# Jonetz/TreeDetection

Measured on AMD Instinct MI355X. Metric: tiles/sec (1000x1000 RGB+nDSM) predict_tiles model stage, higher is better.
Workload: dtype f32

## Files before the change

include/treedet.h:

```cpp
#ifndef TREEDET_H
#define TREEDET_H

#include <stddef.h>
#include <stdint.h>

#ifdef __cplusplus
extern "C" {
#endif

typedef int td_status;
typedef struct td_engine td_engine;

enum {
    TD_OK = 0,
    TD_ERR_INVALID = -1,
    TD_ERR_HIP = -2,
    TD_ERR_WEIGHTS = -3,
    TD_ERR_CAPACITY = -4,
    TD_ERR_STATE = -5,
    TD_ERR_UNSUPPORTED = -6
};

enum { TD_PRECISION_FP32 = 0, TD_PRECISION_FP16 = 1 };
enum { TD_INPUT_F32_CHW = 0,
       TD_INPUT_U8_HWC = 1 };

typedef struct td_model_desc {
    int32_t num_classes;
    int32_t precision;
    int32_t pre_nms_topk;
    int32_t post_nms_topk;
    int32_t detections_per_image;
    float rpn_nms_thresh;
    float score_thresh;
    float nms_thresh;
    float mask_thresh;
} td_model_desc;

typedef struct td_tensor_desc {
    const char* name;
    const float* data;
    int32_t ndim;
    int64_t shape[4];
} td_tensor_desc;

#define TD_MASK_SIDE 28

typedef struct td_detections {
    float* boxes;
    float* scores;
    int32_t* classes;
    int32_t* count;
    float* mask_probs;
    int32_t* mask_region;
    int64_t* mask_offset;
    uint32_t* mask_bits;
    int64_t mask_words_per_image;
} td_detections;

void td_model_desc_default(td_model_desc* desc);
td_status td_engine_create(const td_model_desc* desc, int device, td_engine** out);
td_status td_engine_load_weights(td_engine* e, const td_tensor_desc* tensors, size_t n);
td_status td_engine_reserve(td_engine* e, int max_batch, int max_hp, int max_wp);
td_status td_engine_forward(td_engine* e, const void* images, int input_format, const int32_t* hw_valid,
                            const int32_t* hw_out, int B, int Hp, int Wp, void* stream, td_detections* out);
#define TD_PHASE_STEM 6
td_status td_engine_forward_phase(td_engine* e, int phase, const void* images, int input_format, const int32_t* hw_valid,
                                  const int32_t* hw_out, int B, int Hp, int Wp, void* stream, td_detections* out);
td_status td_engine_tensor(td_engine* e, const char* name, void** dev_ptr, int64_t dims[4], int* elem_size);
td_status td_engine_read_tensor(td_engine* e, const char* name, void* dst_dev, int64_t bytes, void* stream);
#define TD_PROF_CATEGORIES 9
td_status td_engine_profile_enable(td_engine* e, int enable);
td_status td_engine_profile_read(td_engine* e, double* ms, int64_t* launches, double* flops, double* bytes, int reset);
#define TD_PROF_CLASSES 7
#define TD_CLS_WINO_GEMM 0
#define TD_CLS_WINO_XFORM 1
#define TD_CLS_CONV1X1 2
#define TD_CLS_CONV3X3 3
#define TD_CLS_FC 4
#define TD_CLS_MASK_HEAD 5
#define TD_CLS_TAIL 6
#define TD_PEAK_F32_MFMA_TFLOPS 157.3
#define TD_PEAK_F16_MFMA_TFLOPS 2500.0
#define TD_HBM_ACHIEVABLE_TBS 6.3
td_status td_engine_profile_classes(td_engine* e, double* ms, int64_t* launches, double* exec_flops, double* bytes, double* tmin_ms, int reset);
const char* td_last_error(void);
void td_engine_destroy(td_engine* e);

td_status td_resize_tile_u8(const uint8_t* src, int h, int w, int c, uint8_t* dst, int out_h, int out_w,
                            int dst_pitch_px, void* tmp_dev , void* stream);
td_status td_resize_batch_u8(const uint8_t* const* src_tiles, int n, int h, int w, int c, uint8_t* dst, int out_h,
                             int out_w, int dst_pitch_px, int64_t dst_image_stride_bytes, void* tmp_dev, void* stream);
td_status td_resize_bilinear_f64(const double* src, int c, int h, int w, float* dst, int out_h, int out_w, int dst_pitch_px,
                                 int64_t dst_plane_stride, void* stream);
td_status td_windows_u16_to_input(const uint16_t* raster, int height, int width, int c, const int32_t* windows, int n, int32_t* band1_max,
                                  float* dst, int out_h, int out_w, int dst_pitch_px, int64_t dst_plane_stride, int64_t dst_image_stride,
                                  void* stream);
void td_resize_shape(int h, int w, int short_edge, int max_size, int* out_h, int* out_w);

td_status td_bottleneck_tail_nhwc(const void* x, const void* w2, const float* scale2, const float* bias2, const void* w3,
                                  const float* scale3, const float* bias3, const void* shortcut, void* y, int B, int H, int W,
                                  int mid, int cout, int precision, void* stream);
td_status td_conv2d_nhwc(const void* x, const void* w, const float* scale, const float* bias,
                         const void* residual, int res_shift, void* y, int B, int H, int W, int Cin,
                         int Cout, int KH, int KW, int stride, int pad, int relu, int precision,
                         void* stream);
td_status td_conv2d_head_nhwc(const void* x, const void* w, const float* bias, const void* head_w, const float* head_b,
                              float* head_y, int B, int H, int W, int Cin, int KH, int KW, int pad, int head_n, int precision,
                              void* stream);
td_status td_conv2d_winograd_nhwc(const float* x, const float* w, const float* scale, const float* bias, float* y, int B,
                                  int H, int W, int Cin, int Cout, int relu, void* stream);
td_status td_conv2d_winograd_head_nhwc(const float* x, const float* w, const float* bias, const float* head_w, const float* head_b,
                                       float* head_y, int B, int H, int W, int Cin, int head_n, void* stream);
td_status td_nms(const float* boxes, const float* scores, int n, float iou_thresh, int32_t* keep_idx,
                 int32_t* keep_count, void* stream);
td_status td_roi_align(const void* feat, int H, int W, int C, const float* rois, int R, float spatial_scale,
                       int pooled, void* out, int precision, void* stream);
td_status td_paste_masks(const float* mask_probs, const float* boxes, int n, int out_h, int out_w,
                         float thresh, int32_t* mask_region, int64_t* mask_offset, uint32_t* mask_bits,
                         int64_t mask_words_cap, void* stream);

td_status td_paste_masks_batch(const float* mask_probs, const float* boxes, const int32_t* counts, const int32_t* out_hw,
                               int batch, int dets_per_image, float thresh, int32_t* mask_region, int64_t* mask_offset,
                               uint32_t* mask_bits, int64_t mask_words_per_image, void* stream);

#define TD_CONTOUR_MAX 256
td_status td_trace_contours_dev(const int32_t* mask_region, const int64_t* mask_offset, const uint32_t* mask_bits,
                                int64_t mask_words_per_image, const int32_t* counts, int batch, int dets_per_image,
                                int16_t* points, int points_cap, int32_t* image_points, int32_t* det_info,
                                int32_t* contour_info, void* stream);

int td_find_contours(const uint8_t* img, int h, int w, int32_t* points, int max_points, int32_t* starts,
                     int max_contours);
int td_tile_polygons_json(const int32_t* mask_region, const int64_t* mask_offset, const uint32_t* mask_bits,
                          int64_t mask_words, const float* scores, const int32_t* classes, int n,
                          const double* transform, const char* image_id, char* buf, int64_t cap, int64_t* needed);

int td_tile_prediction_file(int device, const int32_t* mask_region, const int64_t* mask_offset, const uint32_t* mask_bits_dev,
                            uint32_t* rows_host, int64_t mask_words, const float* scores, const int32_t* classes, int n,
                            const double* transform, const char* image_id, const char* path, int64_t* bytes_written);

int td_batch_prediction_files(int device, int n_tiles, int dets_per_image, const int32_t* mask_region, const int64_t* mask_offset,
                              const uint32_t* mask_bits_dev, uint32_t* rows_host, int64_t bits_stride_words, const float* scores,
                              const int32_t* classes, const int32_t* counts, const double* transforms, const char* image_id,
                              const char* const* paths, int threads, int32_t* status, int64_t* bytes_written);

int64_t td_tiff_lzw_decode(const uint8_t* src, int64_t n, uint8_t* dst, int64_t cap);
int64_t td_tiff_packbits_decode(const uint8_t* src, int64_t n, uint8_t* dst, int64_t cap);
int64_t td_tiff_lzw_encode(const uint8_t* src, int64_t n, uint8_t* dst, int64_t cap);
td_status td_tiff_lzw_decode_dev(const uint8_t* comp, const int64_t* block_off, const int64_t* block_nbytes, int nblocks,
                                 uint8_t* blocks_out, int64_t block_cap, int64_t* decoded, int32_t* status, void* stream);
td_status td_tiff_inflate_dev(const uint8_t* comp, const int64_t* block_off, const int64_t* block_nbytes, int nblocks,
                              uint8_t* blocks_out, int64_t block_cap, int64_t* decoded, int32_t* status, void* stream);
td_status td_tiff_inflate_verified_dev(const uint8_t* comp, const int64_t* block_off, const int64_t* block_nbytes, int nblocks,
                                       uint8_t* blocks_out, int64_t block_cap, int64_t* decoded, int32_t* status, int64_t* end_off,
                                       void* stream);
td_status td_tiff_adler32_blocks_dev(const uint8_t* blocks, int64_t block_cap, const int64_t* decoded, const uint8_t* comp,
                                     const int64_t* block_off, const int64_t* block_nbytes, const int64_t* end_off, int nblocks,
                                     int32_t* status, void* stream);
td_status td_adler32_dev(const uint8_t* data_dev, int64_t n, uint32_t* out_dev, void* stream);
int64_t td_tiff_inflate(const uint8_t* src, int64_t n, uint8_t* dst, int64_t cap);
int64_t td_tiff_inflate_verified(const uint8_t* src, int64_t n, uint8_t* dst, int64_t cap);
td_status td_tiff_blocks_to_image_dev(const uint8_t* blocks, int64_t block_cap, int block_w, int block_h, int blocks_across,
                                      int blocks_down, int spp, int predictor, uint8_t* image, int width, int height, void* stream);
td_status td_tiff_blocks_to_image_u16_dev(const uint8_t* blocks, int64_t block_cap, int block_w, int block_h, int blocks_across,
                                          int blocks_down, int spp, int predictor, uint16_t* image, int width, int height, void* stream);
td_status td_tiff_blocks_to_image_f32_dev(const uint8_t* blocks, int64_t block_cap, int block_w, int block_h, int blocks_across,
                                          int blocks_down, int spp, int predictor, float* image, int width, int height, void* stream);
#define TD_JPEG_TABSET_BYTES 8928
td_status td_tiff_jpeg_plan(const uint8_t* tables, int64_t tables_len, const uint8_t* data, const int64_t* block_off,
                            const int64_t* block_nbytes, int nblocks, int photometric, int bands, int block_w, const int32_t* block_rows,
                            int64_t* block_info, int64_t* segs, int64_t seg_cap, void* tabsets, int64_t tabset_cap, int64_t* totals);
td_status td_tiff_jpeg_decode_dev(const uint8_t* comp, const int64_t* block_info, int nblocks, const int64_t* segs, int nseg,
                                  const void* tabsets, int16_t* coef, uint8_t* planes, int64_t coef_count, int32_t* status, uint8_t* image,
                                  int width, int height, int bands, int block_w, int block_h, int blocks_across, void* stream);
int64_t td_jpeg_decode(const uint8_t* src, int64_t n, uint8_t* dst, int64_t cap, int32_t* shape);
int64_t td_read_window(int fd, int64_t file_off, int64_t row_stride, int64_t row_bytes, int64_t rows, uint8_t* dst);
int64_t td_read_windows(int fd, int n, const int64_t* file_off, int64_t row_stride, const int64_t* row_bytes, const int64_t* rows,
                        uint8_t* dst, const int64_t* dst_off, int threads);
int td_tiff_unpredict(void* data, int64_t rows, int64_t cols, int samples, int bytes_per_sample);
int td_tiff_unpredict_float(void* data, int64_t rows, int64_t cols, int samples, int bytes_per_sample);

int td_tile_polygons_json_dev(const int16_t* points, int64_t points_cap, const int32_t* det_info, const int32_t* contour_info,
                              const int32_t* mask_region, const int64_t* mask_offset, const uint32_t* mask_bits,
                              int64_t mask_words, const float* scores, const int32_t* classes, int n,
                              const double* transform, const char* image_id, char* buf, int64_t cap, int64_t* needed);

int td_simplify_ring(const double* xy, int n, double tolerance, double* out_xy, int out_cap);

int td_ring_is_valid(const double* xy, int n);
int td_stitch_tile_json(const char* json, int64_t len, const double* box, double tolerance, int32_t srs_id,
                        uint8_t* blobs, int64_t blob_cap, int64_t* blob_offsets, double* scores, int max_features,
                        int64_t* needed_bytes, int* needed_features);

int td_stitch_tile_files(const char* paths, const int64_t* path_offsets, int n_files, const double* boxes, double tolerance,
                         const int32_t* srs_ids, int threads, uint8_t* blobs, int64_t blob_cap, int64_t* blob_offsets,
                         double* scores, int max_features, int32_t* file_status, int64_t* needed_bytes, int* needed_features);

int td_region_relate(const double* ring_xy, const int64_t* ring_start, const int32_t* ring_poly, int n_rings,
                     const double* query_xy, const int64_t* query_start, int n_queries, uint8_t* flags);

td_status td_crown_stats(const float* raster, int rows, int cols, const double* transform, const int32_t* window,
                         const float* circles, int n, int mode, float radius_scale, float* out, void* stream);

#ifdef __cplusplus
}
#endif
#endif
```

treedetection_amd/_lib.py:

```python
from __future__ import annotations

import ctypes as C
import os
import threading
from typing import Optional

_HERE = os.path.dirname(os.path.abspath(__file__))
LIB_PATH = os.path.join(_HERE, "libtreedet_hip.so")

_lib: Optional[C.CDLL] = None
ERR_INVALID = -1
ERR_CAPACITY = -4
ERR_STATE = -5
ERR_UNSUPPORTED = -6
JPEG_TABSET_BYTES = 8928


class TdError(RuntimeError):
    """A libtreedet_hip call returned a negative status (message from td_last_error)."""


class ModelDesc(C.Structure):
    _fields_ = [("num_classes", C.c_int32), ("precision", C.c_int32), ("pre_nms_topk", C.c_int32),
                ("post_nms_topk", C.c_int32), ("detections_per_image", C.c_int32),
                ("rpn_nms_thresh", C.c_float), ("score_thresh", C.c_float), ("nms_thresh", C.c_float),
                ("mask_thresh", C.c_float)]


class TensorDesc(C.Structure):
    _fields_ = [("name", C.c_char_p), ("data", C.c_void_p), ("ndim", C.c_int32), ("shape", C.c_int64 * 4)]


class Detections(C.Structure):
    _fields_ = [("boxes", C.c_void_p), ("scores", C.c_void_p), ("classes", C.c_void_p), ("count", C.c_void_p),
                ("mask_probs", C.c_void_p), ("mask_region", C.c_void_p), ("mask_offset", C.c_void_p),
                ("mask_bits", C.c_void_p), ("mask_words_per_image", C.c_int64)]


SIGNATURES = {
    "td_model_desc_default": (None, [C.POINTER(ModelDesc)]),
    "td_engine_create": (C.c_int, [C.POINTER(ModelDesc), C.c_int, C.POINTER(C.c_void_p)]),
    "td_engine_load_weights": (C.c_int, [C.c_void_p, C.POINTER(TensorDesc), C.c_size_t]),
    "td_engine_reserve": (C.c_int, [C.c_void_p, C.c_int, C.c_int, C.c_int]),
    "td_engine_forward": (C.c_int, [C.c_void_p, C.c_void_p, C.c_int, C.POINTER(C.c_int32), C.POINTER(C.c_int32),
                                    C.c_int, C.c_int, C.c_int, C.c_void_p, C.POINTER(Detections)]),
    "td_engine_forward_phase": (C.c_int, [C.c_void_p, C.c_int, C.c_void_p, C.c_int, C.POINTER(C.c_int32), C.POINTER(C.c_int32),
                                          C.c_int, C.c_int, C.c_int, C.c_void_p, C.POINTER(Detections)]),
    "td_engine_tensor": (C.c_int, [C.c_void_p, C.c_char_p, C.POINTER(C.c_void_p), C.POINTER(C.c_int64),
                                   C.POINTER(C.c_int)]),
    "td_engine_read_tensor": (C.c_int, [C.c_void_p, C.c_char_p, C.c_void_p, C.c_int64, C.c_void_p]),
    "td_engine_profile_enable": (C.c_int, [C.c_void_p, C.c_int]),
    "td_engine_profile_read": (C.c_int, [C.c_void_p, C.POINTER(C.c_double), C.POINTER(C.c_int64), C.POINTER(C.c_double),
                                         C.POINTER(C.c_double), C.c_int]),
    "td_engine_profile_classes": (C.c_int, [C.c_void_p, C.POINTER(C.c_double), C.POINTER(C.c_int64), C.POINTER(C.c_double),
                                            C.POINTER(C.c_double), C.POINTER(C.c_double), C.c_int]),
    "td_last_error": (C.c_char_p, []),
    "td_engine_destroy": (None, [C.c_void_p]),
    "td_resize_tile_u8": (C.c_int, [C.c_void_p, C.c_int, C.c_int, C.c_int, C.c_void_p, C.c_int, C.c_int, C.c_int,
                                    C.c_void_p, C.c_void_p]),
    "td_resize_batch_u8": (C.c_int, [C.POINTER(C.c_void_p), C.c_int, C.c_int, C.c_int, C.c_int, C.c_void_p, C.c_int, C.c_int,
                                     C.c_int, C.c_int64, C.c_void_p, C.c_void_p]),
    "td_bottleneck_tail_nhwc": (C.c_int, [C.c_void_p] * 9 + [C.c_int] * 6 + [C.c_void_p]),
    "td_resize_bilinear_f64": (C.c_int, [C.c_void_p, C.c_int, C.c_int, C.c_int, C.c_void_p, C.c_int, C.c_int, C.c_int, C.c_int64, C.c_void_p]),
    "td_windows_u16_to_input": (C.c_int, [C.c_void_p, C.c_int, C.c_int, C.c_int, C.c_void_p, C.c_int, C.c_void_p, C.c_void_p, C.c_int, C.c_int,
                                          C.c_int, C.c_int64, C.c_int64, C.c_void_p]),
    "td_resize_shape": (None, [C.c_int, C.c_int, C.c_int, C.c_int, C.POINTER(C.c_int), C.POINTER(C.c_int)]),
    "td_conv2d_nhwc": (C.c_int, [C.c_void_p, C.c_void_p, C.c_void_p, C.c_void_p, C.c_void_p, C.c_int, C.c_void_p]
                       + [C.c_int] * 11 + [C.c_void_p]),
    "td_conv2d_head_nhwc": (C.c_int, [C.c_void_p] * 6 + [C.c_int] * 9 + [C.c_void_p]),
    "td_conv2d_winograd_head_nhwc": (C.c_int, [C.c_void_p] * 6 + [C.c_int] * 5 + [C.c_void_p]),
    "td_conv2d_winograd_nhwc": (C.c_int, [C.c_void_p] * 5 + [C.c_int] * 6 + [C.c_void_p]),
    "td_nms": (C.c_int, [C.c_void_p, C.c_void_p, C.c_int, C.c_float, C.c_void_p, C.c_void_p, C.c_void_p]),
    "td_roi_align": (C.c_int, [C.c_void_p, C.c_int, C.c_int, C.c_int, C.c_void_p, C.c_int, C.c_float, C.c_int,
                               C.c_void_p, C.c_int, C.c_void_p]),
    "td_paste_masks": (C.c_int, [C.c_void_p, C.c_void_p, C.c_int, C.c_int, C.c_int, C.c_float, C.c_void_p,
                                 C.c_void_p, C.c_void_p, C.c_int64, C.c_void_p]),
    "td_paste_masks_batch": (C.c_int, [C.c_void_p, C.c_void_p, C.c_void_p, C.POINTER(C.c_int32), C.c_int, C.c_int, C.c_float,
                                       C.c_void_p, C.c_void_p, C.c_void_p, C.c_int64, C.c_void_p]),
    "td_crown_stats": (C.c_int, [C.c_void_p, C.c_int, C.c_int, C.POINTER(C.c_double), C.POINTER(C.c_int32), C.c_void_p, C.c_int,
                                 C.c_int, C.c_float, C.c_void_p, C.c_void_p]),
    "td_trace_contours_dev": (C.c_int, [C.c_void_p, C.c_void_p, C.c_void_p, C.c_int64, C.c_void_p, C.c_int, C.c_int, C.c_void_p,
                                        C.c_int, C.c_void_p, C.c_void_p, C.c_void_p, C.c_void_p]),
    "td_find_contours": (C.c_int, [C.c_void_p, C.c_int, C.c_int, C.c_void_p, C.c_int, C.c_void_p, C.c_int]),
    "td_batch_prediction_files": (C.c_int, [C.c_int, C.c_int, C.c_int, C.c_void_p, C.c_void_p, C.c_void_p, C.c_void_p, C.c_int64, C.c_void_p,
                                          C.c_void_p, C.c_void_p, C.c_void_p, C.c_char_p, C.POINTER(C.c_char_p), C.c_int, C.c_void_p, C.c_void_p]),
    "td_tiff_lzw_decode": (C.c_int64, [C.c_void_p, C.c_int64, C.c_void_p, C.c_int64]),
    "td_tiff_packbits_decode": (C.c_int64, [C.c_void_p, C.c_int64, C.c_void_p, C.c_int64]),
    "td_tiff_lzw_encode": (C.c_int64, [C.c_void_p, C.c_int64, C.c_void_p, C.c_int64]),
    "td_tiff_inflate": (C.c_int64, [C.c_void_p, C.c_int64, C.c_void_p, C.c_int64]),
    "td_tiff_inflate_dev": (C.c_int, [C.c_void_p, C.c_void_p, C.c_void_p, C.c_int, C.c_void_p, C.c_int64, C.c_void_p, C.c_void_p, C.c_void_p]),
    "td_tiff_inflate_verified": (C.c_int64, [C.c_void_p, C.c_int64, C.c_void_p, C.c_int64]),
    "td_tiff_inflate_verified_dev": (C.c_int, [C.c_void_p, C.c_void_p, C.c_void_p, C.c_int, C.c_void_p, C.c_int64, C.c_void_p, C.c_void_p, C.c_void_p,
                                               C.c_void_p]),
    "td_tiff_adler32_blocks_dev": (C.c_int, [C.c_void_p, C.c_int64, C.c_void_p, C.c_void_p, C.c_void_p, C.c_void_p, C.c_void_p, C.c_int, C.c_void_p,
                                             C.c_void_p]),
    "td_adler32_dev": (C.c_int, [C.c_void_p, C.c_int64, C.c_void_p, C.c_void_p]),
    "td_tiff_lzw_decode_dev": (C.c_int, [C.c_void_p, C.c_void_p, C.c_void_p, C.c_int, C.c_void_p, C.c_int64, C.c_void_p, C.c_void_p, C.c_void_p]),
    "td_tiff_blocks_to_image_dev": (C.c_int, [C.c_void_p, C.c_int64, C.c_int, C.c_int, C.c_int, C.c_int, C.c_int, C.c_int, C.c_void_p, C.c_int, C.c_int, C.c_void_p]),
    "td_tiff_blocks_to_image_u16_dev": (C.c_int, [C.c_void_p, C.c_int64, C.c_int, C.c_int, C.c_int, C.c_int, C.c_int, C.c_int, C.c_void_p, C.c_int,
                                                  C.c_int, C.c_void_p]),
    "td_tiff_blocks_to_image_f32_dev": (C.c_int, [C.c_void_p, C.c_int64, C.c_int, C.c_int, C.c_int, C.c_int, C.c_int, C.c_int, C.c_void_p, C.c_int,
                                                  C.c_int, C.c_void_p]),
    "td_tiff_jpeg_plan": (C.c_int, [C.c_void_p, C.c_int64, C.c_void_p, C.c_void_p, C.c_void_p, C.c_int, C.c_int, C.c_int, C.c_int, C.c_void_p,
                                    C.c_void_p, C.c_void_p, C.c_int64, C.c_void_p, C.c_int64, C.c_void_p]),
    "td_tiff_jpeg_decode_dev": (C.c_int, [C.c_void_p, C.c_void_p, C.c_int, C.c_void_p, C.c_int, C.c_void_p, C.c_void_p, C.c_void_p, C.c_int64,
                                          C.c_void_p, C.c_void_p] + [C.c_int] * 6 + [C.c_void_p]),
    "td_jpeg_decode": (C.c_int64, [C.c_void_p, C.c_int64, C.c_void_p, C.c_int64, C.c_void_p]),
    "td_read_windows": (C.c_int64, [C.c_int, C.c_int, C.c_void_p, C.c_int64, C.c_void_p, C.c_void_p, C.c_void_p, C.c_void_p, C.c_int]),
    "td_tiff_unpredict": (C.c_int, [C.c_void_p, C.c_int64, C.c_int64, C.c_int, C.c_int]),
    "td_tiff_unpredict_float": (C.c_int, [C.c_void_p, C.c_int64, C.c_int64, C.c_int, C.c_int]),
    "td_region_relate": (C.c_int, [C.c_void_p, C.c_void_p, C.c_void_p, C.c_int, C.c_void_p, C.c_void_p, C.c_int, C.c_void_p]),
    "td_simplify_ring": (C.c_int, [C.c_void_p, C.c_int, C.c_double, C.c_void_p, C.c_int]),
    "td_ring_is_valid": (C.c_int, [C.c_void_p, C.c_int]),
    "td_stitch_tile_json": (C.c_int, [C.c_char_p, C.c_int64, C.POINTER(C.c_double), C.c_double, C.c_int32, C.c_void_p,
                                      C.c_int64, C.c_void_p, C.c_void_p, C.c_int, C.POINTER(C.c_int64), C.POINTER(C.c_int)]),
    "td_stitch_tile_files": (C.c_int, [C.c_char_p, C.c_void_p, C.c_int, C.c_void_p, C.c_double, C.c_void_p, C.c_int, C.c_void_p, C.c_int64,
                                       C.c_void_p, C.c_void_p, C.c_int, C.c_void_p, C.POINTER(C.c_int64), C.POINTER(C.c_int)]),
    "td_tile_polygons_json_dev": (C.c_int, [C.c_void_p, C.c_int64, C.c_void_p, C.c_void_p, C.c_void_p, C.c_void_p, C.c_void_p, C.c_int64,
                                            C.c_void_p, C.c_void_p, C.c_int, C.POINTER(C.c_double), C.c_char_p, C.c_void_p, C.c_int64,
                                            C.POINTER(C.c_int64)]),
    "td_read_window": (C.c_int64, [C.c_int, C.c_int64, C.c_int64, C.c_int64, C.c_int64, C.c_void_p]),
    "td_tile_prediction_file": (C.c_int, [C.c_int, C.c_void_p, C.c_void_p, C.c_void_p, C.c_void_p, C.c_int64, C.c_void_p, C.c_void_p,
                                          C.c_int, C.POINTER(C.c_double), C.c_char_p, C.c_char_p, C.POINTER(C.c_int64)]),
    "td_tile_polygons_json": (C.c_int, [C.c_void_p, C.c_void_p, C.c_void_p, C.c_int64, C.c_void_p, C.c_void_p, C.c_int,
                                        C.POINTER(C.c_double), C.c_char_p, C.c_void_p, C.c_int64, C.POINTER(C.c_int64)]),
}


def load() -> C.CDLL:
    global _lib
    if _lib is not None:
        return _lib
    host_only = os.environ.get("TD_HOST_LIB")
    if host_only:
        lib = C.CDLL(host_only, mode=C.RTLD_GLOBAL)
        for name, (res, args) in SIGNATURES.items():
            fn = getattr(lib, name, None)
            if fn is not None:
                fn.restype = res
                fn.argtypes = args
        _lib = lib
        return lib
    if not os.path.exists(LIB_PATH):
        raise TdError(f"{LIB_PATH} not found — build it first: python -c 'import __graft_entry__ as g; g.build()' "
                      f"(or make -C treedetection_amd/csrc). There is no CPU fallback.")
    import torch

    lib = C.CDLL(LIB_PATH, mode=C.RTLD_GLOBAL)
    for name, (res, args) in SIGNATURES.items():
        fn = getattr(lib, name)
        fn.restype = res
        fn.argtypes = args
    _lib = lib
    return lib


def check(status: int, what: str = "") -> None:
    if status < 0:
        msg = load().td_last_error().decode("utf-8", "replace")
        raise TdError(f"{what or 'libtreedet_hip'} failed ({status}): {msg}")


def stream_ptr() -> int:
    import torch

    return int(torch.cuda.current_stream().cuda_stream)


_low_priority_streams: dict = {}
_low_priority_lock = threading.Lock()


def low_priority_stream(device_index: int):
    import torch

    with _low_priority_lock:
        if device_index in _low_priority_streams:
            return _low_priority_streams[device_index]
        lib = load()
        least, greatest, handle = C.c_int(0), C.c_int(0), C.c_void_p()
        with torch.cuda.device(device_index):
            torch.cuda.current_stream()
            err = lib.hipDeviceGetStreamPriorityRange(C.byref(least), C.byref(greatest))
            if err == 0:
                err = lib.hipStreamCreateWithPriority(C.byref(handle), C.c_uint(1), C.c_int(least.value))
            if err != 0 or not handle.value:
                raise TdError(f"hipStreamCreateWithPriority(priority {least.value}) failed: hipError {err}")
            stream = torch.cuda.ExternalStream(handle.value, device=device_index)
        _low_priority_streams[device_index] = stream
        return stream
```

treedetection_amd/csrc/api.cpp:

```cpp
#include "common.h"
#include "detect.h"
#include <cstdarg>
#include <cstdio>
#include <cmath>
#include <cstdlib>
#include <vector>


namespace {
td_status scratch(void** p, size_t bytes) {
    TD_HIP_CHECK(hipMalloc(p, bytes ? bytes : 16));
    return TD_OK;
}
}

extern "C" {

void td_model_desc_default(td_model_desc* d) {
    d->num_classes = 1;
    d->precision = TD_PRECISION_FP32;
    d->pre_nms_topk = 1000;
    d->post_nms_topk = 1000;
    d->detections_per_image = 100;
    d->rpn_nms_thresh = 0.7f;
    d->score_thresh = 0.3f;
    d->nms_thresh = 0.5f;
    d->mask_thresh = 0.5f;
}

static td_status conv2d_api(ConvArgs& a, int precision, void* stream);

td_status td_conv2d_nhwc(const void* x, const void* w, const float* scale, const float* bias,
                         const void* residual, int res_shift, void* y, int B, int H, int W, int Cin,
                         int Cout, int KH, int KW, int stride, int pad, int relu, int precision,
                         void* stream) {
    TD_REQUIRE(x && w && y, "td_conv2d_nhwc: null pointer");
    TD_REQUIRE(stride >= 1 && KH >= 1 && KW >= 1 && B >= 1, "td_conv2d_nhwc: bad geometry");
    ConvArgs a{};
    a.x = x; a.w = w; a.scale = scale; a.bias = bias; a.res = residual; a.y = y;
    a.B = B; a.H = H; a.W = W; a.Cin = Cin; a.Cout = Cout; a.KH = KH; a.KW = KW;
    a.stride = stride; a.pad = pad;
    a.Ho = (H + 2 * pad - KH) / stride + 1;
    a.Wo = (W + 2 * pad - KW) / stride + 1;
    a.res_shift = res_shift; a.relu = relu; a.out_mode = 0;
    a.M = B * a.Ho * a.Wo; a.m_dyn = nullptr; a.m_mul = 1;
    a.out_f32 = (precision & 0x10000) && (precision & 0xff) == TD_PRECISION_FP16 ? 1 : 0;
    a.tile_cfg = ((precision >> 8) & 0xff) - 1;
    a.tile_strict = (precision & 0x20000) ? 1 : 0;
    return conv2d_api(a, precision, stream);
}

td_status td_conv2d_head_nhwc(const void* x, const void* w, const float* bias, const void* head_w, const float* head_b,
                              float* head_y, int B, int H, int W, int Cin, int KH, int KW, int pad, int head_n, int precision,
                              void* stream) {
    TD_REQUIRE(x && w && head_w && head_y, "td_conv2d_head_nhwc: null pointer");
    TD_REQUIRE((precision & 0xff) == TD_PRECISION_FP16, "td_conv2d_head_nhwc: float16 tensors only");
    TD_REQUIRE(KH >= 1 && KW >= 1 && B >= 1 && head_n >= 1 && head_n <= 32, "td_conv2d_head_nhwc: bad geometry");
    ConvArgs a{};
    a.x = x; a.w = w; a.bias = bias;
    a.B = B; a.H = H; a.W = W; a.Cin = Cin; a.Cout = 256; a.KH = KH; a.KW = KW;
    a.stride = 1; a.pad = pad;
    a.Ho = H + 2 * pad - KH + 1;
    a.Wo = W + 2 * pad - KW + 1;
    a.relu = 1; a.M = B * a.Ho * a.Wo; a.m_mul = 1;
    a.tile_cfg = ((precision >> 8) & 0xff) - 1;
    TD_REQUIRE(conv_head_capable(a.tile_cfg, TD_PRECISION_FP16), "td_conv2d_head_nhwc: tile id %d does not own 256 output channels per block", a.tile_cfg);
    a.head_w = head_w; a.head_b = head_b; a.head_y = head_y; a.head_n = head_n;
    a.y = head_y;
    return conv2d_api(a, precision, stream);
}

static td_status conv2d_api(ConvArgs& a, int precision, void* stream) {
    hipStream_t s = static_cast<hipStream_t>(stream);
    ConvArgs with_frag = a;
    with_frag.w_frag = a.w;
    if (!conv_tile(a.tile_cfg) || !conv_tile(a.tile_cfg)->frag || conv_tile_refusal(a.tile_cfg, with_frag, precision & 0xff))
        return conv2d_launch(a, precision & 0xff, s);
    const int es = (precision & 0xff) == TD_PRECISION_FP16 ? 2 : 4;
    const size_t n = (size_t)a.Cout * a.KH * a.KW * a.Cin;
    std::vector<unsigned char> bits(n * es), packed;
    TD_HIP_CHECK(hipStreamSynchronize(s));
    TD_HIP_CHECK(hipMemcpy(bits.data(), a.w, n * es, hipMemcpyDeviceToHost));
    conv_bd_pack(bits.data(), es, a.Cout, a.KH, a.KW, a.Cin, packed);
    void* wf = nullptr;
    td_status st = scratch(&wf, packed.size());
    if (st < 0) return st;
    hipError_t herr = hipMemcpy(wf, packed.data(), packed.size(), hipMemcpyHostToDevice);
    a.w_frag = wf;
    if (herr == hipSuccess) st = conv2d_launch(a, precision & 0xff, s);
    hipError_t herr2 = hipStreamSynchronize(s);
    (void)hipFree(wf);
    if (st < 0) return st;
    TD_HIP_CHECK(herr);
    TD_HIP_CHECK(herr2);
    return TD_OK;
}

static td_status wino_api(const float* x, const float* w, const float* scale, const float* bias, float* y, int B, int H, int W, int Cin,
                          int Cout, int relu, void* stream, const float* head_w, const float* head_b, float* head_y, int head_n);

td_status td_conv2d_winograd_nhwc(const float* x, const float* w, const float* scale, const float* bias, float* y, int B, int H,
                                  int W, int Cin, int Cout, int relu, void* stream) {
    TD_REQUIRE(y, "td_conv2d_winograd_nhwc: bad arguments");
    return wino_api(x, w, scale, bias, y, B, H, W, Cin, Cout, relu, stream, nullptr, nullptr, nullptr, 0);
}

td_status td_conv2d_winograd_head_nhwc(const float* x, const float* w, const float* bias, const float* head_w, const float* head_b,
                                       float* head_y, int B, int H, int W, int Cin, int head_n, void* stream) {
    TD_REQUIRE(head_w && head_y && head_n >= 1 && head_n <= 32, "td_conv2d_winograd_head_nhwc: bad arguments");
    return wino_api(x, w, nullptr, bias, nullptr, B, H, W, Cin, 256, 1, stream, head_w, head_b, head_y, head_n);
}

static td_status wino_api(const float* x, const float* w, const float* scale, const float* bias, float* y, int B, int H, int W, int Cin,
                          int Cout, int relu, void* stream, const float* head_w, const float* head_b, float* head_y, int head_n) {
    TD_REQUIRE(x && w && B >= 1 && H >= 1 && W >= 1, "td_conv2d_winograd_nhwc: bad arguments");
    TD_REQUIRE(Cin % 32 == 0 && Cout % 4 == 0, "td_conv2d_winograd_nhwc: Cin must be a multiple of 32, Cout of 4");
    hipStream_t s = static_cast<hipStream_t>(stream);
    const char* tenv = getenv("TD_WINO_TILE");
    const bool f43 = head_w || (tenv && atoi(tenv) == 4);
    const int P = f43 ? 36 : 16;
    const size_t T = f43 ? (size_t)B * ((H + 3) / 4) * ((W + 3) / 4) : (size_t)B * ((H + 1) / 2) * ((W + 1) / 2);
    std::vector<float> wh((size_t)Cout * 9 * Cin), uh((size_t)P * Cout * Cin);
    TD_HIP_CHECK(hipMemcpy(wh.data(), w, wh.size() * sizeof(float), hipMemcpyDeviceToHost));
    if (f43) wino43_filter_transform(wh.data(), Cout, Cin, uh.data());
    else wino_filter_transform(wh.data(), Cout, Cin, uh.data());
    void *U = nullptr, *V = nullptr, *Mb = nullptr;
    td_status st;
    if ((st = scratch(&U, uh.size() * 4)) < 0 || (st = scratch(&V, P * T * Cin * 4)) < 0 || (st = scratch(&Mb, P * T * Cout * 4)) < 0) {
        (void)hipFree(U); (void)hipFree(V); (void)hipFree(Mb);
        return st;
    }
    TD_HIP_CHECK(hipMemcpy(U, uh.data(), uh.size() * 4, hipMemcpyHostToDevice));
    const char* folde = getenv("TD_WINO_FOLD");
    const bool fold = f43 && !head_w && folde && atoi(folde) != 0;
    if (fold) TD_REQUIRE(wino43_fused_ok(B, H, W, Cin, Cout), "td_conv2d_winograd_nhwc: TD_WINO_FOLD needs Cin %% 128 == 0, Cout %% 64 == 0");
    const char* fenv = getenv("TD_WINO_FUSED");
    const bool fused = !f43 && (!fenv || atoi(fenv) != 0);
    ConvArgs a{};
    a.w = U; a.y = Mb;
    a.Cin = Cin; a.Cout = Cout; a.KH = a.KW = 1; a.stride = 1; a.pad = 0;
    a.M = (int)T; a.m_mul = 1; a.tile_cfg = -1;
    a.w_bs = (long long)Cout * Cin; a.y_bs = (long long)T * Cout;
    if (fused) {
        a.x = x; a.B = B; a.H = H; a.W = W;
        st = wino_gemm_launch(a, s);
    } else {
        st = f43 ? wino43_input_launch(x, B, H, W, Cin, static_cast<float*>(V), nullptr, s)
                 : wino_input_launch(x, B, H, W, Cin, static_cast<float*>(V), nullptr, 1, 0, (int)T, s);
        if (st == TD_OK && fold) {
            st = wino43_fused_launch(static_cast<float*>(V), static_cast<float*>(U), B, H, W, Cin, Cout, scale, bias, relu, y, nullptr, s);
        } else if (st == TD_OK) {
            a.x = V; a.B = 1; a.H = 1; a.W = (int)T; a.Ho = 1; a.Wo = (int)T;
            a.batch_count = P; a.x_bs = (long long)T * Cin;
            st = conv2d_launch(a, TD_PRECISION_FP32, s);
        }
    }
    if (fold) {
    } else if (st == TD_OK && head_w)
        st = wino43_output_head_launch(static_cast<float*>(Mb), B, H, W, Cout, scale, bias, relu, head_w, head_b, head_y, head_n, s);
    else if (st == TD_OK)
        st = f43 ? wino43_output_launch(static_cast<float*>(Mb), B, H, W, Cout, scale, bias, relu, y, nullptr, s)
                 : wino_output_launch(static_cast<float*>(Mb), B, H, W, Cout, scale, bias, relu, y, nullptr, 1, 0, (int)T, s);
    hipError_t herr = hipStreamSynchronize(s);
    (void)hipFree(U); (void)hipFree(V); (void)hipFree(Mb);
    if (st < 0) return st;
    TD_HIP_CHECK(herr);
    return TD_OK;
}

td_status td_resize_tile_u8(const uint8_t* src, int h, int w, int c, uint8_t* dst, int out_h, int out_w,
                            int dst_pitch_px, void* tmp_dev, void* stream) {
    return resize_tile_u8_launch(src, h, w, c, dst, out_h, out_w, dst_pitch_px, tmp_dev, static_cast<hipStream_t>(stream));
}

td_status td_resize_batch_u8(const uint8_t* const* src_tiles, int n, int h, int w, int c, uint8_t* dst, int out_h,
                             int out_w, int dst_pitch_px, int64_t dst_image_stride_bytes, void* tmp_dev, void* stream) {
    return resize_batch_u8_launch(src_tiles, n, h, w, c, dst, out_h, out_w, dst_pitch_px, (size_t)dst_image_stride_bytes,
                                  tmp_dev, static_cast<hipStream_t>(stream));
}

td_status td_bottleneck_tail_nhwc(const void* x, const void* w2, const float* scale2, const float* bias2, const void* w3,
                                  const float* scale3, const float* bias3, const void* shortcut, void* y, int B, int H, int W,
                                  int mid, int cout, int precision, void* stream) {
    TD_REQUIRE(x && w2 && w3 && shortcut && y && B > 0 && H > 0 && W > 0, "td_bottleneck_tail_nhwc: null argument or empty tensor");
    TailArgs a{};
    a.x = x; a.w2 = w2; a.scale2 = scale2; a.bias2 = bias2; a.w3 = w3; a.scale3 = scale3; a.bias3 = bias3; a.res = shortcut; a.y = y;
    a.B = B; a.H = H; a.W = W; a.MID = mid; a.COUT = cout; a.M = B * H * W;
    return bottleneck_tail_launch(a, precision, static_cast<hipStream_t>(stream));
}

td_status td_resize_bilinear_f64(const double* src, int c, int h, int w, float* dst, int out_h, int out_w, int dst_pitch_px,
                                 int64_t dst_plane_stride, void* stream) {
    return resize_bilinear_f64_launch(src, c, h, w, dst, out_h, out_w, dst_pitch_px, (long long)dst_plane_stride, static_cast<hipStream_t>(stream));
}

td_status td_windows_u16_to_input(const uint16_t* raster, int height, int width, int c, const int32_t* windows, int n, int32_t* band1_max,
                                  float* dst, int out_h, int out_w, int dst_pitch_px, int64_t dst_plane_stride, int64_t dst_image_stride,
                                  void* stream) {
    return windows_u16_to_input_launch(raster, height, width, c, windows, n, band1_max, dst, out_h, out_w, dst_pitch_px,
                                       (long long)dst_plane_stride, (long long)dst_image_stride, static_cast<hipStream_t>(stream));
}

void td_resize_shape(int h, int w, int short_edge, int max_size, int* out_h, int* out_w) {
    const double scale = (double)short_edge / (double)(h < w ? h : w);
    double newh, neww;
    if (h < w) { newh = short_edge; neww = scale * w; }
    else { newh = scale * h; neww = short_edge; }
    const double mx = newh > neww ? newh : neww;
    if (mx > max_size) {
        const double s2 = (double)max_size / mx;
        newh *= s2;
        neww *= s2;
    }
    *out_h = (int)(newh + 0.5);
    *out_w = (int)(neww + 0.5);
}

td_status td_nms(const float* boxes, const float* scores, int n, float iou_thresh, int32_t* keep_idx,
                 int32_t* keep_count, void* stream) {
    TD_REQUIRE(boxes && scores && keep_idx && keep_count, "td_nms: null pointer");
    TD_REQUIRE(n >= 0 && n <= 32768, "td_nms: n=%d must be in [0, 32768]", n);
    hipStream_t s = static_cast<hipStream_t>(stream);
    if (n == 0) {
        TD_HIP_CHECK(hipMemsetAsync(keep_count, 0, sizeof(int32_t), s));
        return TD_OK;
    }
    void *sb = nullptr, *ss = nullptr, *si = nullptr, *sc = nullptr, *mk = nullptr, *kp = nullptr;
    td_status st;
    if ((st = scratch(&sb, sizeof(float) * 4 * n)) < 0) return st;
    if ((st = scratch(&ss, sizeof(float) * n)) < 0) return st;
    if ((st = scratch(&si, sizeof(int) * n)) < 0) return st;
    if ((st = scratch(&sc, sizeof(int))) < 0) return st;
    if ((st = scratch(&mk, sizeof(unsigned long long) * n * td_cdiv(n, 64))) < 0) return st;
    if ((st = scratch(&kp, sizeof(int) * n)) < 0) return st;
    if (n > 1024) {
        st = nms_big_launch(boxes, scores, n, iou_thresh, (float*)sb, (float*)ss, (int*)si, (int*)sc, (unsigned long long*)mk, (int*)kp, keep_count, s);
    } else {
        st = sort_boxes_launch(boxes, scores, nullptr, nullptr, 1, n, (float*)sb, (float*)ss, (int*)si, (int*)sc, s);
        if (st >= 0) st = nms_launch((float*)sb, (int*)sc, nullptr, 1, n, iou_thresh, (unsigned long long*)mk, (int*)kp, keep_count, n, s);
    }
    if (st >= 0) st = gather_keep_launch((int*)si, (int*)kp, keep_count, n, keep_idx, s);
    hipError_t herr = hipStreamSynchronize(s);
    (void)hipFree(sb); (void)hipFree(ss); (void)hipFree(si); (void)hipFree(sc); (void)hipFree(mk); (void)hipFree(kp);
    if (st < 0) return st;
    TD_HIP_CHECK(herr);
    return TD_OK;
}

td_status td_roi_align(const void* feat, int H, int W, int C, const float* rois, int R, float spatial_scale,
                       int pooled, void* out, int precision, void* stream) {
    TD_REQUIRE(feat && rois && out, "td_roi_align: null pointer");
    TD_REQUIRE(H >= 1 && W >= 1 && pooled >= 1 && R >= 0, "td_roi_align: bad geometry");
    if (R == 0) return TD_OK;
    return roi_align_single_launch(feat, H, W, C, rois, R, spatial_scale, pooled, out, precision, static_cast<hipStream_t>(stream));
}

td_status td_paste_masks(const float* mask_probs, const float* boxes, int n, int out_h, int out_w, float thresh,
                         int32_t* mask_region, int64_t* mask_offset, uint32_t* mask_bits, int64_t mask_words_cap,
                         void* stream) {
    TD_REQUIRE(mask_probs && boxes && mask_region && mask_offset && mask_bits, "td_paste_masks: null pointer");
    TD_REQUIRE(n >= 0 && n <= 1024 && out_h >= 1 && out_w >= 1, "td_paste_masks: bad shape");
    if (n == 0) return TD_OK;
    hipStream_t s = static_cast<hipStream_t>(stream);
    void* cnt = nullptr;
    td_status st = scratch(&cnt, sizeof(int));
    if (st < 0) return st;
    TD_HIP_CHECK(hipMemcpy(cnt, &n, sizeof(int), hipMemcpyHostToDevice));
    ImgSizes outsz{};
    outsz.h[0] = out_h;
    outsz.w[0] = out_w;
    st = paste_masks_launch(mask_probs, boxes, (int*)cnt, outsz, 1, n, thresh, mask_region,
                            reinterpret_cast<long long*>(mask_offset), mask_bits, mask_words_cap, s);
    hipError_t herr = hipStreamSynchronize(s);
    (void)hipFree(cnt);
    if (st < 0) return st;
    TD_HIP_CHECK(herr);
    return TD_OK;
}

td_status td_paste_masks_batch(const float* mask_probs, const float* boxes, const int32_t* counts, const int32_t* out_hw,
                               int batch, int dets_per_image, float thresh, int32_t* mask_region, int64_t* mask_offset,
                               uint32_t* mask_bits, int64_t mask_words_per_image, void* stream) {
    TD_REQUIRE(mask_probs && boxes && counts && out_hw && mask_region && mask_offset && mask_bits,
               "td_paste_masks_batch: null pointer");
    TD_REQUIRE(batch >= 1 && batch <= TD_MAX_BATCH && dets_per_image >= 1 && dets_per_image <= 1024,
               "td_paste_masks_batch: batch %d (max %d) / detections per image %d (max 1024)", batch, TD_MAX_BATCH, dets_per_image);
    ImgSizes outsz{};
    for (int i = 0; i < batch; ++i) {
        TD_REQUIRE(out_hw[2 * i] >= 1 && out_hw[2 * i + 1] >= 1, "td_paste_masks_batch: bad output size of image %d", i);
        outsz.h[i] = out_hw[2 * i];
        outsz.w[i] = out_hw[2 * i + 1];
        const int64_t need = (int64_t)dets_per_image * ((outsz.w[i] + 2 + 31) / 32) * outsz.h[i];
        TD_REQUIRE(mask_words_per_image >= need, "td_paste_masks_batch: image %d needs %lld mask words, capacity %lld", i,
                   (long long)need, (long long)mask_words_per_image);
    }
    return paste_masks_launch(mask_probs, boxes, counts, outsz, batch, dets_per_image, thresh, mask_region,
                              reinterpret_cast<long long*>(mask_offset), mask_bits, mask_words_per_image,
                              static_cast<hipStream_t>(stream));
}

}
```

treedetection_amd/csrc/common.h:

```cpp
#pragma once
#include <hip/hip_runtime.h>
#include <hip/hip_fp16.h>
#include <cstdint>
#include <cstddef>
#include "../../include/treedet.h"
#include <string>
#include <vector>

void td_set_error(const char* fmt, ...);

int td_polygons_json_text(const int32_t* mask_region, const int64_t* mask_offset, const uint32_t* mask_bits, int64_t mask_words,
                          const float* scores, const int32_t* classes, int n, const double* transform, const char* image_id,
                          std::string& out, const char* who);

#define TD_HIP_CHECK(expr)                                                                         \
    do {                                                                                           \
        hipError_t _e = (expr);                                                                    \
        if (_e != hipSuccess) {                                                                    \
            td_set_error("%s failed: %s (%s:%d)", #expr, hipGetErrorString(_e), __FILE__, __LINE__); \
            return TD_ERR_HIP;                                                                     \
        }                                                                                          \
    } while (0)

#define TD_REQUIRE(cond, ...)            \
    do {                                 \
        if (!(cond)) {                   \
            td_set_error(__VA_ARGS__);   \
            return TD_ERR_INVALID;       \
        }                                \
    } while (0)

#define TD_KERNEL_CHECK() TD_HIP_CHECK(hipGetLastError())

td_status td_decode_ticket(hipStream_t s, int** ticket, int* cus);

static inline int td_cdiv(int a, int b) { return (a + b - 1) / b; }

struct ConvArgs {
    const void* x;
    const void* w;
    const float* scale;
    const float* bias;
    const void* res;
    void* y;
    int B, H, W, Cin, Cout, KH, KW, stride, pad, Ho, Wo;
    int res_shift;
    int relu;
    int out_mode;
    int M;
    const int* m_dyn;
    int m_mul;
    int m_off;
    int out_f32;
    int batch_count;
    long long x_bs, w_bs, y_bs;
    const void* w_frag;
    int tile_cfg;
    int tile_strict;
    const void* head_w;
    const float* head_b;
    float* head_y;
    int head_n;
    int nlev;
    struct Level {
        const void* x;
        const void* w;
        const float* bias;
        void* y;
        float* head_y;
        int H, W, M, tile0;
    } lev[5];
    int ntiles;
};
enum ConvFamily : unsigned char { TILE_IGEMM, TILE_PP8, TILE_PLANE, TILE_BD, TILE_BS, TILE_RETIRED };
enum : unsigned char { TILE_F32 = 1 << TD_PRECISION_FP32, TILE_F16 = 1 << TD_PRECISION_FP16, TILE_ANY = TILE_F32 | TILE_F16 };
struct ConvTile {
    ConvFamily family;
    unsigned char variant;
    unsigned char prec;
    bool head;
    bool frag;
    signed char tune_rank;
    unsigned char max_ksteps;
    short min_cout, max_cout;
};
inline constexpr ConvTile TD_CONV_TILES[] = {
    {TILE_IGEMM,   0, TILE_ANY, false, false,  5, 0,   0,  0},
    {TILE_IGEMM,   0, TILE_ANY, false, false, 10, 0,   0,  0},
    {TILE_IGEMM,   0, TILE_ANY, false, false, 11, 0,   0,  0},
    {TILE_IGEMM,   0, TILE_ANY, false, false, 16, 0,   0,  0},
    {TILE_IGEMM,   0, TILE_ANY, false, false, -1, 0,   0,  0},
    {TILE_IGEMM,   0, TILE_ANY, false, false, -1, 0,   0,  0},
    {TILE_IGEMM,   0, TILE_ANY, false, false, -1, 0,   0,  0},
    {TILE_IGEMM,   0, TILE_ANY, false, false, -1, 0,   0,  0},
    {TILE_IGEMM,   0, TILE_ANY, false, false, -1, 0,   0,  0},
    {TILE_IGEMM,   0, TILE_ANY, true,  false, -1, 0,   0,  0},
    {TILE_IGEMM,   0, TILE_ANY, true,  false,  1, 0,   0,  0},
    {TILE_IGEMM,   0, TILE_ANY, false, false, -1, 0,   0,  0},
    {TILE_IGEMM,   0, TILE_ANY, true,  false, -1, 0,   0,  0},
    {TILE_IGEMM,   0, TILE_ANY, true,  false, -1, 0,   0,  0},
    {TILE_IGEMM,   0, TILE_ANY, false, false, -1, 4,   0,  0},
    {TILE_IGEMM,   0, TILE_ANY, false, false,  6, 4,   0,  0},
    {TILE_IGEMM,   0, TILE_ANY, false, false,  4, 4,   0,  0},
    {TILE_PP8,     0, TILE_F16, true,  false,  2, 0, 128,  0},
    {TILE_PLANE,   0, TILE_F32, false, false, 18, 0,   0,  0},
    {TILE_PLANE,   0, TILE_F32, false, false, 19, 0,   0,  0},
    {TILE_PLANE,   0, TILE_F32, false, false, 20, 0,   0,  0},
    {TILE_RETIRED, 0, 0,        false, false, -1, 0,   0,  0},
    {TILE_RETIRED, 0, 0,        false, false, -1, 0,   0,  0},
    {TILE_BD,      0, TILE_ANY, true,  true,   8, 0,   0,  0},
    {TILE_BD,      1, TILE_ANY, false, true,  12, 0,   0,  0},
    {TILE_BD,      2, TILE_ANY, false, true,  13, 0,   0,  0},
    {TILE_BD,      3, TILE_ANY, false, true,  14, 0,   0,  0},
    {TILE_BD,      4, TILE_ANY, true,  true,   9, 0,   0,  0},
    {TILE_RETIRED, 0, 0,        false, false, -1, 0,   0,  0},
    {TILE_BD,      5, TILE_ANY, true,  true,   3, 0,   0,  0},
    {TILE_BD,      6, TILE_ANY, false, true,   7, 0,   0,  0},
    {TILE_IGEMM,   0, TILE_ANY, false, false, 15, 0,   0, 32},
    {TILE_IGEMM,   0, TILE_ANY, false, false, 17, 0,   0, 32},
    {TILE_BS,      0, TILE_ANY, false, true,   0, 4, 128,  0},
};
static inline const ConvTile* conv_tile(int id) { return id >= 0 && id < (int)(sizeof TD_CONV_TILES / sizeof *TD_CONV_TILES) ? &TD_CONV_TILES[id] : nullptr; }
static inline bool conv_head_capable(int id, int precision) { return precision == TD_PRECISION_FP16 && conv_tile(id) && conv_tile(id)->head; }
const char* conv_tile_refusal(int id, const ConvArgs& a, int precision);
td_status conv2d_launch(const ConvArgs& a, int precision, hipStream_t stream);
td_status conv_pp8_grouped_launch(ConvArgs a, hipStream_t stream);
void conv_bd_pack(const void* w_ohwi, int elem_bytes, int cout, int kh, int kw, int cin, std::vector<unsigned char>& out);
bool conv_bd_ok(const ConvArgs& a, int precision);
td_status conv_bd_launch(const ConvArgs& a, int precision, int variant, hipStream_t stream);
bool conv_bs_ok(const ConvArgs& a, int precision);
td_status conv_bs_launch(const ConvArgs& a, int precision, hipStream_t stream);
td_status wino_gemm_launch(const ConvArgs& a, hipStream_t stream);

struct TailArgs {
    const void* x;
    const void* w2;
    const float* scale2;
    const float* bias2;
    const void* w3;
    const float* scale3;
    const float* bias3;
    const void* res;
    void* y;
    int B, H, W, MID, COUT, M;
};
bool bottleneck_tail_ok(int precision, int mid, int cout);
td_status bottleneck_tail_launch(const TailArgs& a, int precision, hipStream_t stream);

td_status wino_input_launch(const float* x, int B, int H, int W, int C, float* V, const int* m_dyn, int m_mul, long long t0, int Ts,
                            hipStream_t s);
td_status wino_output_launch(const float* Mb, int B, int H, int W, int N, const float* scale, const float* bias, int relu,
                             float* y, const int* m_dyn, int m_mul, long long t0, int Ts, hipStream_t s);
void wino_filter_transform(const float* w_ohwi, int N, int C, float* U);
td_status wino43_input_launch(const float* x, int B, int H, int W, int C, float* V, const int* m_dyn, hipStream_t s);
bool wino43_fused_ok(int B, int H, int W, int C, int N);
td_status wino43_fused_launch(const float* V, const float* U, int B, int H, int W, int C, int N, const float* scale, const float* bias,
                              int relu, float* y, const int* m_dyn, hipStream_t s);
td_status wino43_output_launch(const float* Mb, int B, int H, int W, int N, const float* scale, const float* bias, int relu,
                               float* y, const int* m_dyn, hipStream_t s);
td_status wino43_output_head_launch(const float* Mb, int B, int H, int W, int N, const float* scale, const float* bias, int relu,
                                    const float* head_w, const float* head_b, float* head_y, int head_n, hipStream_t s);
void wino43_filter_transform(const float* w_ohwi, int N, int C, float* U);

struct ImgSizes {
    int h[64];
    int w[64];
};
#define TD_MAX_BATCH 64
td_status stem_launch(const void* images, int input_format, const ImgSizes& valid, int B, int Hp, int Wp,
                      const float* w_kc , const float* scale, const float* bias, void* y,
                      int cout, int precision, hipStream_t stream, const void* w16 = nullptr, const float* bias16 = nullptr);
void stem_mfma_prepare(const float* w_kc, const float* scale, const float* bias, int cout, std::vector<unsigned short>& w16_bits,
                       std::vector<float>& bias16);
td_status maxpool3x3s2_launch(const void* x, void* y, int B, int H, int W, int C, int precision, hipStream_t stream);
td_status subsample2_launch(const void* x, void* y, int B, int H, int W, int C, int precision, hipStream_t stream);
td_status resize_batch_u8_launch(const uint8_t* const* srcs, int n, int h, int w, int c, uint8_t* dst, int out_h,
                                 int out_w, int dst_pitch_px, size_t dst_img_bytes, void* tmp, hipStream_t stream);
td_status resize_bilinear_f64_launch(const double* src, int c, int h, int w, float* dst, int out_h, int out_w, int dst_pitch,
                                     long long dst_plane, hipStream_t stream);
td_status windows_u16_to_input_launch(const uint16_t* raster, int H, int W, int C, const int32_t* windows, int n, int* band1_max, float* dst,
                                      int out_h, int out_w, int dst_pitch, long long dst_plane, long long dst_image, hipStream_t stream);
td_status resize_tile_u8_launch(const uint8_t* src, int h, int w, int c, uint8_t* dst, int out_h, int out_w,
                                int dst_pitch_px, void* tmp, hipStream_t stream);
```

treedetection_amd/csrc/engine.cpp:

```cpp
#include "common.h"
#include "detect.h"

#include <cmath>
#include <cstdio>
#include <cstdlib>
#include <cstring>
#include <algorithm>
#include <functional>
#include <map>
#include <optional>
#include <string>
#include <tuple>
#include <vector>

namespace {

struct HostTensor {
    const float* data = nullptr;
    std::vector<int64_t> shape;
    int64_t numel() const {
        int64_t n = 1;
        for (auto s : shape) n *= s;
        return n;
    }
};

struct ConvLayer {
    int cout = 0, cin = 0, kh = 1, kw = 1;
    void* w = nullptr;
    float* scale = nullptr;
    float* bias = nullptr;
    bool out_f32 = false;
    void* w_frag = nullptr;
    float* wino_u = nullptr;
    float* wino_u43 = nullptr;
};

struct Block {
    ConvLayer c1, c2, c3, sc;
    bool has_sc = false;
    int stride = 1;
};

struct NamedTensor {
    void* p = nullptr;
    int64_t dims[4] = {0, 0, 0, 0};
    int elem = 4;
};

}

struct td_engine {
    td_model_desc desc{};
    int device = 0;
    bool loaded = false;
    std::vector<void*> weight_allocs;
    std::vector<void*> ws_allocs;

    float* stem_w = nullptr;
    float* stem_scale = nullptr;
    float* stem_bias = nullptr;
    unsigned short* stem_w16 = nullptr;
    float* stem_bias16 = nullptr;
    int stem_c = 64;
    std::vector<Block> stages[4];
    ConvLayer lateral[4], fpn_out[4];
    ConvLayer rpn_conv, rpn_head;
    ConvLayer fc1, fc2, pred;
    ConvLayer mask_fcn[4], deconv;
    float* mask_pred_w = nullptr;
    float mask_pred_b = 0.f;
    int fpn_c = 256, fc_dim = 1024;

    int rB = 0, rHp = 0, rWp = 0;
    void *stem_out = nullptr, *pool_out = nullptr;
    void *t1[4] = {}, *t2[4] = {}, *scb[4] = {}, *res[4] = {}, *xtmp[4] = {};
    void *inner[4] = {}, *pfeat[5] = {};
    void* rpn_t = nullptr;
    float* rpn_headbuf[5] = {};
    uint32_t* key_ws = nullptr;
    float *cand_boxes = nullptr, *cand_scores = nullptr;
    int *cand_valid = nullptr, *cand_idx = nullptr;
    unsigned long long* nms_mask = nullptr;
    int *rpn_keep = nullptr, *rpn_keep_count = nullptr;
    float *props = nullptr, *prop_scores = nullptr;
    int* prop_count = nullptr;
    void *pooled7 = nullptr, *fc1_out = nullptr, *fc2_out = nullptr;
    float* pred_out = nullptr;
    float *dboxes = nullptr, *dscores = nullptr;
    int* dflags = nullptr;
    float *sboxes = nullptr, *sscores = nullptr;
    int *sidx = nullptr, *scount = nullptr, *det_keep = nullptr, *det_keep_count = nullptr;
    float* det_boxes_net = nullptr;
    void *pooled14 = nullptr, *mbuf0 = nullptr, *mbuf1 = nullptr, *deconv_out = nullptr;
    float *mask_logits = nullptr, *mask_probs_compact = nullptr;
    int* total_rows = nullptr;
    float *o_boxes = nullptr, *o_scores = nullptr, *o_mask_probs = nullptr;
    int *o_classes = nullptr, *o_count = nullptr;

    std::map<std::string, NamedTensor> named;

    bool autotune = true;
    int backbone_subbatch = 0;
    std::map<std::tuple<int, int, int, int, int>, int> tuned;
    bool winograd = true;
    float *wino_v = nullptr, *wino_m = nullptr;
    size_t wino_elems = 0;
    bool group_levels = true;
    bool fuse_head = true;
    bool fuse_tail = true;
    bool fuse_tail_fp16 = false;
    bool wino_fused = true;
    int wino_slab = 0;
    int wino_minc = 128;
    int wino43_min = 12;
    int wino_fold = 39;
    std::string tune_cache;
    void* tune_evict = nullptr;
    size_t tune_evict_bytes = 0;

    struct FwdCtx {
        const void* images = nullptr;
        int input_format = 0, B = 0, Hp = 0, Wp = 0;
        ImgSizes valid{}, outsz{};
        td_detections out{};
        bool valid_ctx = false;
    } ctx;
    hipEvent_t phase_ev[7] = {};
    bool phase_ev_recorded[7] = {};
    hipEvent_t prev5_ev = nullptr;
    bool prev5_recorded = false;
    bool stem_done = false;

    bool prof = false;
    bool prof_group_open = false;
    struct ProfRec { hipEvent_t a, b; int cat; };
    std::vector<ProfRec> prof_recs;
    std::vector<hipEvent_t> prof_free;
    double prof_ms[TD_PROF_CATEGORIES] = {};
    int64_t prof_launches[TD_PROF_CATEGORIES] = {};
    double prof_flops[TD_PROF_CATEGORIES] = {};
    double prof_bytes[TD_PROF_CATEGORIES] = {};
    bool prof_detail = false;
    double cls_ms[TD_PROF_CLASSES] = {};
    int64_t cls_launches[TD_PROF_CLASSES] = {};
    double cls_flops[TD_PROF_CLASSES] = {};
    double cls_bytes[TD_PROF_CLASSES] = {};
    double cls_tmin_ms[TD_PROF_CLASSES] = {};
    struct ClsRec { hipEvent_t a, b; int cls; };
    std::vector<ClsRec> cls_recs;
};

namespace {

td_status dev_alloc(std::vector<void*>& pool, void** p, size_t bytes) {
    if (bytes == 0) bytes = 16;
    TD_HIP_CHECK(hipMalloc(p, bytes));
    pool.push_back(*p);
    return TD_OK;
}

template <typename T>
td_status upload(td_engine* e, const std::vector<T>& h, T** d) {
    void* p = nullptr;
    td_status st = dev_alloc(e->weight_allocs, &p, h.size() * sizeof(T));
    if (st < 0) return st;
    TD_HIP_CHECK(hipMemcpy(p, h.data(), h.size() * sizeof(T), hipMemcpyHostToDevice));
    *d = static_cast<T*>(p);
    return TD_OK;
}

td_status upload_w(td_engine* e, const std::vector<float>& h, void** d) {
    if (e->desc.precision == TD_PRECISION_FP16) {
        std::vector<_Float16> hh(h.size());
        for (size_t i = 0; i < h.size(); ++i) hh[i] = (_Float16)h[i];
        _Float16* p = nullptr;
        td_status st = upload(e, hh, &p);
        *d = p;
        return st;
    }
    float* p = nullptr;
    td_status st = upload(e, h, &p);
    *d = p;
    return st;
}

td_status upload_frag(td_engine* e, const std::vector<float>& h, ConvLayer& L) {
    L.w_frag = nullptr;
    static const bool off = getenv("TD_BDIRECT") && atoi(getenv("TD_BDIRECT")) == 0;
    const bool f16 = e->desc.precision == TD_PRECISION_FP16;
    const int ke = f16 ? 64 : 32;
    if (off || L.cin % ke != 0 || L.kh * L.kw > 32 || (size_t)L.cout * L.kh * L.kw * L.cin != h.size()) return TD_OK;
    std::vector<unsigned char> packed;
    if (f16) {
        std::vector<unsigned short> bits(h.size());
        for (size_t i = 0; i < h.size(); ++i) bits[i] = __builtin_bit_cast(unsigned short, (_Float16)h[i]);
        conv_bd_pack(bits.data(), 2, L.cout, L.kh, L.kw, L.cin, packed);
    } else {
        conv_bd_pack(h.data(), 4, L.cout, L.kh, L.kw, L.cin, packed);
    }
    unsigned char* d = nullptr;
    td_status st = upload(e, packed, &d);
    L.w_frag = d;
    return st;
}

using TensorMap = std::map<std::string, HostTensor>;

td_status need(const TensorMap& tm, const std::string& name, int ndim, const HostTensor** out) {
    auto it = tm.find(name);
    if (it == tm.end()) {
        td_set_error("load_weights: tensor '%s' missing", name.c_str());
        return TD_ERR_WEIGHTS;
    }
    if ((int)it->second.shape.size() != ndim) {
        td_set_error("load_weights: tensor '%s' has %d dims, expected %d", name.c_str(), (int)it->second.shape.size(), ndim);
        return TD_ERR_WEIGHTS;
    }
    *out = &it->second;
    return TD_OK;
}

std::vector<float> pack_ohwi(const HostTensor& t) {
    const int co = (int)t.shape[0], ci = (int)t.shape[1], kh = (int)t.shape[2], kw = (int)t.shape[3];
    std::vector<float> out((size_t)co * ci * kh * kw);
    for (int o = 0; o < co; ++o)
        for (int c = 0; c < ci; ++c)
            for (int y = 0; y < kh; ++y)
                for (int x = 0; x < kw; ++x)
                    out[(((size_t)o * kh + y) * kw + x) * ci + c] = t.data[(((size_t)o * ci + c) * kh + y) * kw + x];
    return out;
}

td_status bn_fold(const TensorMap& tm, const std::string& p, int c, std::vector<float>& scale, std::vector<float>& bias) {
    const HostTensor *g, *b, *m, *v;
    td_status st;
    if ((st = need(tm, p + ".norm.weight", 1, &g)) < 0) return st;
    if ((st = need(tm, p + ".norm.bias", 1, &b)) < 0) return st;
    if ((st = need(tm, p + ".norm.running_mean", 1, &m)) < 0) return st;
    if ((st = need(tm, p + ".norm.running_var", 1, &v)) < 0) return st;
    if (g->shape[0] != c || b->shape[0] != c || m->shape[0] != c || v->shape[0] != c) {
        td_set_error("load_weights: norm tensors of '%s' do not have %d channels", p.c_str(), c);
        return TD_ERR_WEIGHTS;
    }
    scale.resize(c);
    bias.resize(c);
    for (int i = 0; i < c; ++i) {
        const float r = 1.0f / std::sqrt(v->data[i] + 1e-5f);
        const float s = g->data[i] * r;
        const float ms = m->data[i] * s;
        scale[i] = s;
        bias[i] = b->data[i] - ms;
    }
    return TD_OK;
}

int wino_slab_tiles(const td_engine* e, const ConvLayer& L) {
    (void)L;
    return e->wino_slab > 0 ? e->wino_slab : (1 << 30);
}

// ... 11 lines not shown
}

td_status load_conv_bn(td_engine* e, const TensorMap& tm, const std::string& p, ConvLayer& L) {
    const HostTensor* w;
    td_status st = need(tm, p + ".weight", 4, &w);
    if (st < 0) return st;
    L.cout = (int)w->shape[0];
    L.cin = (int)w->shape[1];
    L.kh = (int)w->shape[2];
    L.kw = (int)w->shape[3];
    const std::vector<float> packed = pack_ohwi(*w);
    if ((st = upload_w(e, packed, &L.w)) < 0) return st;
    if ((st = upload_frag(e, packed, L)) < 0) return st;
    if ((st = upload_wino(e, packed, L)) < 0) return st;
    std::vector<float> s, b;
    if ((st = bn_fold(tm, p, L.cout, s, b)) < 0) return st;
    if ((st = upload(e, s, &L.scale)) < 0) return st;
    return upload(e, b, &L.bias);
}

td_status load_conv_bias(td_engine* e, const TensorMap& tm, const std::string& p, ConvLayer& L) {
    const HostTensor *w, *b;
    td_status st = need(tm, p + ".weight", 4, &w);
    if (st < 0) return st;
    if ((st = need(tm, p + ".bias", 1, &b)) < 0) return st;
    L.cout = (int)w->shape[0];
    L.cin = (int)w->shape[1];
    L.kh = (int)w->shape[2];
    L.kw = (int)w->shape[3];
    if (b->shape[0] != L.cout) {
        td_set_error("load_weights: bias of '%s' has wrong length", p.c_str());
        return TD_ERR_WEIGHTS;
    }
    const std::vector<float> packed = pack_ohwi(*w);
    if ((st = upload_w(e, packed, &L.w)) < 0) return st;
    if ((st = upload_frag(e, packed, L)) < 0) return st;
    if ((st = upload_wino(e, packed, L)) < 0) return st;
    L.scale = nullptr;
    return upload(e, std::vector<float>(b->data, b->data + L.cout), &L.bias);
}

void set_named(td_engine* e, const char* name, void* p, int64_t d0, int64_t d1 = 0, int64_t d2 = 0, int64_t d3 = 0,
               int elem = 4) {
    NamedTensor t;
    t.p = p;
    t.dims[0] = d0; t.dims[1] = d1; t.dims[2] = d2; t.dims[3] = d3;
    t.elem = elem;
    e->named[name] = t;
}

hipEvent_t prof_event(td_engine* e) {
    hipEvent_t ev = nullptr;
    if (!e->prof_free.empty()) {
        ev = e->prof_free.back();
        e->prof_free.pop_back();
    } else {
        (void)hipEventCreate(&ev);
    }
    return ev;
}

struct ProfScope {
    td_engine* e;
    hipStream_t s;
    hipEvent_t a = nullptr;
    int cat;
    bool group;
    ProfScope(td_engine* e_, hipStream_t s_, int cat_, double flops = 0.0, double bytes = 0.0, bool group_ = false)
        : e(e_), s(s_), cat(cat_), group(group_) {
        if (!e->prof) return;
        if (!group) {
            e->prof_flops[cat] += flops;
            e->prof_bytes[cat] += bytes;
            e->prof_launches[cat] += 1;
        }
        if (e->prof_group_open) return;
        a = prof_event(e);
        (void)hipEventRecord(a, s);
        if (group) e->prof_group_open = true;
    }
    ~ProfScope() {
        if (!a) return;
        hipEvent_t b = prof_event(e);
        (void)hipEventRecord(b, s);
        e->prof_recs.push_back({a, b, cat});
        if (group) e->prof_group_open = false;
    }
};

struct ClassScope {
    td_engine* e;
    hipStream_t s;
    hipEvent_t a = nullptr;
    int cls;
    ClassScope(td_engine* e_, hipStream_t s_, int cls_, double exec_flops, double bytes) : e(e_), s(s_), cls(cls_) {
        if (!e->prof) return;
        const double peak = (e->desc.precision == TD_PRECISION_FP16 ? TD_PEAK_F16_MFMA_TFLOPS : TD_PEAK_F32_MFMA_TFLOPS) * 1e12;
        e->cls_launches[cls] += 1;
        e->cls_flops[cls] += exec_flops;
        e->cls_bytes[cls] += bytes;
        e->cls_tmin_ms[cls] += 1e3 * std::max(exec_flops / peak, bytes / (TD_HBM_ACHIEVABLE_TBS * 1e12));
        if (!e->prof_detail) return;
        a = prof_event(e);
        (void)hipEventRecord(a, s);
    }
    ~ClassScope() {
        if (!a) return;
        hipEvent_t b = prof_event(e);
        (void)hipEventRecord(b, s);
        e->cls_recs.push_back({a, b, cls});
    }
};

void load_tune_cache(td_engine* e) {
    if (e->tune_cache.empty()) return;
    if (FILE* f = fopen(e->tune_cache.c_str(), "r")) {
        int pr, a0, a1, a2, a3, a4, cfg;
        while (fscanf(f, "%d %d %d %d %d %d %d", &pr, &a0, &a1, &a2, &a3, &a4, &cfg) == 7) {
            if (pr == e->desc.precision && conv_tile(cfg)) e->tuned[std::make_tuple(a0, a1, a2, a3, a4)] = cfg;
        }
        fclose(f);
    }
}

void free_pool(std::vector<void*>& pool) {
    for (void* p : pool) (void)hipFree(p);
    pool.clear();
}

}

extern "C" {

td_status td_engine_create(const td_model_desc* desc, int device, td_engine** out) {
    TD_REQUIRE(out, "td_engine_create: out is NULL");
    td_model_desc d;
    if (desc) d = *desc; else td_model_desc_default(&d);
    TD_REQUIRE(d.num_classes == 1, "td_engine_create: num_classes=%d (the reference configures exactly 1, config.py:35)", d.num_classes);
    TD_REQUIRE(d.precision == TD_PRECISION_FP32 || d.precision == TD_PRECISION_FP16, "td_engine_create: bad precision %d", d.precision);
    TD_REQUIRE(d.pre_nms_topk >= 1 && d.pre_nms_topk <= RPN_CAND, "td_engine_create: pre_nms_topk must be in [1,%d]", RPN_CAND);
    TD_REQUIRE(d.post_nms_topk >= 1 && d.post_nms_topk <= 1024, "td_engine_create: post_nms_topk must be in [1,1024]");
    TD_REQUIRE(d.detections_per_image >= 1 && d.detections_per_image <= 1024, "td_engine_create: detections_per_image must be in [1,1024]");
    int ndev = 0;
    TD_HIP_CHECK(hipGetDeviceCount(&ndev));
    TD_REQUIRE(device >= 0 && device < ndev, "td_engine_create: device %d of %d", device, ndev);
    TD_HIP_CHECK(hipSetDevice(device));
    td_engine* e = new td_engine();
    if (const char* sbenv = getenv("TD_BACKBONE_SUBBATCH")) e->backbone_subbatch = atoi(sbenv);
    if (const char* tc = getenv("TD_TUNE_CACHE")) e->tune_cache = tc;
    if (const char* wg = getenv("TD_WINOGRAD")) e->winograd = atoi(wg) != 0;
    if (const char* ws = getenv("TD_WINO_SLAB")) e->wino_slab = atoi(ws);
    if (const char* wf = getenv("TD_WINO_FUSED")) e->wino_fused = atoi(wf) != 0;
    if (const char* fh = getenv("TD_FUSE_HEAD")) e->fuse_head = atoi(fh) != 0;
    if (const char* gl = getenv("TD_GROUP_LEVELS")) e->group_levels = atoi(gl) != 0;
    if (const char* ft = getenv("TD_FUSE_TAIL")) { e->fuse_tail = atoi(ft) != 0; e->fuse_tail_fp16 = atoi(ft) == 2; }
    if (const char* w4 = getenv("TD_WINO43_MIN")) e->wino43_min = atoi(w4);
    if (const char* wf2 = getenv("TD_WINO_FOLD")) e->wino_fold = atoi(wf2);
    if (const char* wc = getenv("TD_WINO_MINC")) e->wino_minc = atoi(wc);
    e->desc = d;
    load_tune_cache(e);
    e->device = device;
    *out = e;
    return TD_OK;
}

void td_engine_destroy(td_engine* e) {
    if (!e) return;
    (void)hipSetDevice(e->device);
    free_pool(e->weight_allocs);
    free_pool(e->ws_allocs);
    if (e->tune_evict) (void)hipFree(e->tune_evict);
    for (auto& r : e->prof_recs) { (void)hipEventDestroy(r.a); (void)hipEventDestroy(r.b); }
    for (auto& r : e->cls_recs) { (void)hipEventDestroy(r.a); (void)hipEventDestroy(r.b); }
    for (auto ev : e->prof_free) (void)hipEventDestroy(ev);
    for (auto ev : e->phase_ev) if (ev) (void)hipEventDestroy(ev);
    if (e->prev5_ev) (void)hipEventDestroy(e->prev5_ev);
    delete e;
}

td_status td_engine_load_weights(td_engine* e, const td_tensor_desc* tensors, size_t n) {
    TD_REQUIRE(e && tensors, "td_engine_load_weights: null argument");
    TD_HIP_CHECK(hipSetDevice(e->device));
    TensorMap tm;
    for (size_t i = 0; i < n; ++i) {
        TD_REQUIRE(tensors[i].name && tensors[i].data && tensors[i].ndim >= 1 && tensors[i].ndim <= 4,
                   "td_engine_load_weights: bad tensor descriptor %zu", i);
        HostTensor t;
        t.data = tensors[i].data;
        t.shape.assign(tensors[i].shape, tensors[i].shape + tensors[i].ndim);
        tm[tensors[i].name] = t;
    }
    free_pool(e->weight_allocs);
    e->loaded = false;
    td_status st;
    {
        const HostTensor* w;
        if ((st = need(tm, "backbone.bottom_up.stem.conv1.weight", 4, &w)) < 0) return st;
        if (w->shape[1] != 3 || w->shape[2] != 7 || w->shape[3] != 7) {
            td_set_error("load_weights: stem conv must be [C,3,7,7] (RGB+nDSM tiles still feed 3 channels, prediction.py:166)");
            return TD_ERR_WEIGHTS;
        }
        e->stem_c = (int)w->shape[0];
        std::vector<float> p((size_t)147 * e->stem_c);
        for (int co = 0; co < e->stem_c; ++co)
            for (int c = 0; c < 3; ++c)
                for (int ky = 0; ky < 7; ++ky)
                    for (int kx = 0; kx < 7; ++kx)
                        p[(size_t)((ky * 7 + kx) * 3 + c) * e->stem_c + co] = w->data[(((size_t)co * 3 + c) * 7 + ky) * 7 + kx];
        if ((st = upload(e, p, &e->stem_w)) < 0) return st;
        std::vector<float> s, b;
        if ((st = bn_fold(tm, "backbone.bottom_up.stem.conv1", e->stem_c, s, b)) < 0) return st;
        if ((st = upload(e, s, &e->stem_scale)) < 0) return st;
        if ((st = upload(e, b, &e->stem_bias)) < 0) return st;
        const char* mfma_stem = getenv("TD_STEM_MFMA");
        if (e->desc.precision == TD_PRECISION_FP16 && e->stem_c == 64 && !(mfma_stem && atoi(mfma_stem) == 0)) {
            std::vector<unsigned short> w16;
            std::vector<float> b16;
            stem_mfma_prepare(p.data(), s.data(), b.data(), e->stem_c, w16, b16);
            if ((st = upload(e, w16, &e->stem_w16)) < 0) return st;
            if ((st = upload(e, b16, &e->stem_bias16)) < 0) return st;
        }
    }
    for (int si = 0; si < 4; ++si) {
        e->stages[si].clear();
        for (int bi = 0;; ++bi) {
            const std::string p = "backbone.bottom_up.res" + std::to_string(si + 2) + "." + std::to_string(bi);
            if (tm.find(p + ".conv1.weight") == tm.end()) break;
            Block blk;
            blk.stride = (bi == 0 && si > 0) ? 2 : 1;
            if ((st = load_conv_bn(e, tm, p + ".conv1", blk.c1)) < 0) return st;
            if ((st = load_conv_bn(e, tm, p + ".conv2", blk.c2)) < 0) return st;
            if ((st = load_conv_bn(e, tm, p + ".conv3", blk.c3)) < 0) return st;
            blk.has_sc = tm.find(p + ".shortcut.weight") != tm.end();
            if (blk.has_sc && (st = load_conv_bn(e, tm, p + ".shortcut", blk.sc)) < 0) return st;
            e->stages[si].push_back(blk);
        }
        if (e->stages[si].empty()) {
            td_set_error("load_weights: no blocks found for res%d", si + 2);
            return TD_ERR_WEIGHTS;
        }
    }
    for (int l = 0; l < 4; ++l) {
        if ((st = load_conv_bias(e, tm, "backbone.fpn_lateral" + std::to_string(l + 2), e->lateral[l])) < 0) return st;
        if ((st = load_conv_bias(e, tm, "backbone.fpn_output" + std::to_string(l + 2), e->fpn_out[l])) < 0) return st;
    }
    e->fpn_c = e->lateral[0].cout;
    if ((st = load_conv_bias(e, tm, "proposal_generator.rpn_head.conv", e->rpn_conv)) < 0) return st;
    {
        const HostTensor *wo, *bo, *wd, *bd;
        if ((st = need(tm, "proposal_generator.rpn_head.objectness_logits.weight", 4, &wo)) < 0) return st;
        if ((st = need(tm, "proposal_generator.rpn_head.objectness_logits.bias", 1, &bo)) < 0) return st;
        if ((st = need(tm, "proposal_generator.rpn_head.anchor_deltas.weight", 4, &wd)) < 0) return st;
        if ((st = need(tm, "proposal_generator.rpn_head.anchor_deltas.bias", 1, &bd)) < 0) return st;
        if (wo->shape[0] != RPN_A || wd->shape[0] != 4 * RPN_A || wo->shape[1] != e->fpn_c || wd->shape[1] != e->fpn_c) {
            td_set_error("load_weights: RPN head must have %d anchors per position", RPN_A);
            return TD_ERR_WEIGHTS;
        }
        const int c = e->fpn_c;
        std::vector<float> w((size_t)RPN_HEAD_C * c), b(RPN_HEAD_C);
        std::memcpy(w.data(), wo->data, sizeof(float) * RPN_A * c);
        std::memcpy(w.data() + (size_t)RPN_A * c, wd->data, sizeof(float) * 4 * RPN_A * c);
        std::memcpy(b.data(), bo->data, sizeof(float) * RPN_A);
        std::memcpy(b.data() + RPN_A, bd->data, sizeof(float) * 4 * RPN_A);
        e->rpn_head.cout = RPN_HEAD_C; e->rpn_head.cin = c; e->rpn_head.kh = e->rpn_head.kw = 1;
        e->rpn_head.out_f32 = true;
        if ((st = upload_w(e, w, &e->rpn_head.w)) < 0) return st;
        if ((st = upload_frag(e, w, e->rpn_head)) < 0) return st;
        if ((st = upload(e, b, &e->rpn_head.bias)) < 0) return st;
    }
    {
        const HostTensor *w, *b;
        if ((st = need(tm, "roi_heads.box_head.fc1.weight", 2, &w)) < 0) return st;
        if ((st = need(tm, "roi_heads.box_head.fc1.bias", 1, &b)) < 0) return st;
        const int c = e->fpn_c, o = (int)w->shape[0];
        if (w->shape[1] != (int64_t)c * 49) {
            td_set_error("load_weights: fc1 expects %d inputs", c * 49);
            return TD_ERR_WEIGHTS;
        }
        std::vector<float> p((size_t)o * c * 49);
        for (int r = 0; r < o; ++r)
            for (int ch = 0; ch < c; ++ch)
                for (int q = 0; q < 49; ++q) p[(size_t)r * c * 49 + (size_t)q * c + ch] = w->data[(size_t)r * c * 49 + (size_t)ch * 49 + q];
        e->fc1.cout = o; e->fc1.cin = c * 49; e->fc1.kh = e->fc1.kw = 1;
        e->fc_dim = o;
        if ((st = upload_w(e, p, &e->fc1.w)) < 0) return st;
        if ((st = upload_frag(e, p, e->fc1)) < 0) return st;
        if ((st = upload(e, std::vector<float>(b->data, b->data + o), &e->fc1.bias)) < 0) return st;
    }
    {
        const HostTensor *w, *b;
        if ((st = need(tm, "roi_heads.box_head.fc2.weight", 2, &w)) < 0) return st;
        if ((st = need(tm, "roi_heads.box_head.fc2.bias", 1, &b)) < 0) return st;
        e->fc2.cout = (int)w->shape[0]; e->fc2.cin = (int)w->shape[1]; e->fc2.kh = e->fc2.kw = 1;
        const std::vector<float> w2v(w->data, w->data + w->numel());
        if ((st = upload_w(e, w2v, &e->fc2.w)) < 0) return st;
        if ((st = upload_frag(e, w2v, e->fc2)) < 0) return st;
        if ((st = upload(e, std::vector<float>(b->data, b->data + e->fc2.cout), &e->fc2.bias)) < 0) return st;
    }
    {
        const HostTensor *wc, *bc, *wr, *br;
        if ((st = need(tm, "roi_heads.box_predictor.cls_score.weight", 2, &wc)) < 0) return st;
        if ((st = need(tm, "roi_heads.box_predictor.cls_score.bias", 1, &bc)) < 0) return st;
        if ((st = need(tm, "roi_heads.box_predictor.bbox_pred.weight", 2, &wr)) < 0) return st;
        if ((st = need(tm, "roi_heads.box_predictor.bbox_pred.bias", 1, &br)) < 0) return st;
        if (wc->shape[0] != 2 || wr->shape[0] != 4) {
            td_set_error("load_weights: box predictor must be 1 class (+background), got cls %lld / reg %lld rows",
                         (long long)wc->shape[0], (long long)wr->shape[0]);
            return TD_ERR_WEIGHTS;
        }
        const int k = (int)wc->shape[1];
        std::vector<float> w((size_t)6 * k), b(6);
        std::memcpy(w.data(), wc->data, sizeof(float) * 2 * k);
        std::memcpy(w.data() + (size_t)2 * k, wr->data, sizeof(float) * 4 * k);
        std::memcpy(b.data(), bc->data, sizeof(float) * 2);
        std::memcpy(b.data() + 2, br->data, sizeof(float) * 4);
        e->pred.cout = 6; e->pred.cin = k; e->pred.kh = e->pred.kw = 1;
        e->pred.out_f32 = true;
        if ((st = upload_w(e, w, &e->pred.w)) < 0) return st;
        if ((st = upload_frag(e, w, e->pred)) < 0) return st;
        if ((st = upload(e, b, &e->pred.bias)) < 0) return st;
    }
    for (int i = 0; i < 4; ++i)
        if ((st = load_conv_bias(e, tm, "roi_heads.mask_head.mask_fcn" + std::to_string(i + 1), e->mask_fcn[i])) < 0) return st;
    {
        const HostTensor *w, *b;
        if ((st = need(tm, "roi_heads.mask_head.deconv.weight", 4, &w)) < 0) return st;
        if ((st = need(tm, "roi_heads.mask_head.deconv.bias", 1, &b)) < 0) return st;
        const int ci = (int)w->shape[0], co = (int)w->shape[1];
        if (w->shape[2] != 2 || w->shape[3] != 2) {
            td_set_error("load_weights: mask deconv must be 2x2");
            return TD_ERR_WEIGHTS;
        }
        std::vector<float> p((size_t)4 * co * ci);
        for (int i = 0; i < ci; ++i)
            for (int o = 0; o < co; ++o)
                for (int q = 0; q < 4; ++q) p[((size_t)q * co + o) * ci + i] = w->data[((size_t)i * co + o) * 4 + q];
        e->deconv.cout = 4 * co; e->deconv.cin = ci; e->deconv.kh = e->deconv.kw = 1;
        if ((st = upload_w(e, p, &e->deconv.w)) < 0) return st;
        if ((st = upload(e, std::vector<float>(b->data, b->data + co), &e->deconv.bias)) < 0) return st;
    }
    {
        const HostTensor *w, *b;
        if ((st = need(tm, "roi_heads.mask_head.predictor.weight", 4, &w)) < 0) return st;
        if ((st = need(tm, "roi_heads.mask_head.predictor.bias", 1, &b)) < 0) return st;
        if (w->shape[0] != 1) {
            td_set_error("load_weights: mask predictor must have 1 output channel");
            return TD_ERR_WEIGHTS;
        }
        if ((st = upload(e, std::vector<float>(w->data, w->data + w->shape[1]), &e->mask_pred_w)) < 0) return st;
        e->mask_pred_b = b->data[0];
    }
    e->loaded = true;
    return TD_OK;
}

td_status td_engine_reserve(td_engine* e, int B, int Hp, int Wp) {
    TD_REQUIRE(e, "td_engine_reserve: null engine");
    TD_REQUIRE(e->loaded, "td_engine_reserve: load weights first");
    TD_REQUIRE(B >= 1 && B <= TD_MAX_BATCH, "td_engine_reserve: batch %d not in [1,%d]", B, TD_MAX_BATCH);
    TD_REQUIRE(Hp >= 64 && Wp >= 64 && Hp % 32 == 0 && Wp % 32 == 0, "td_engine_reserve: padded size %dx%d must be multiples of 32 (>= 64)", Hp, Wp);
    if (B <= e->rB && Hp <= e->rHp && Wp <= e->rWp) return TD_OK;
    B = B > e->rB ? B : e->rB;
    Hp = Hp > e->rHp ? Hp : e->rHp;
    Wp = Wp > e->rWp ? Wp : e->rWp;
    TD_HIP_CHECK(hipSetDevice(e->device));
    free_pool(e->ws_allocs);
    e->rB = e->rHp = e->rWp = 0;
    auto A = [&](auto** p, size_t elems) -> td_status {
        void* q = nullptr;
        td_status st = dev_alloc(e->ws_allocs, &q, elems * sizeof(**p));
        *p = static_cast<std::remove_reference_t<decltype(*p)>>(q);
        return st;
    };
    const size_t es = e->desc.precision == TD_PRECISION_FP16 ? 2 : 4;
    auto AA = [&](void** p, size_t elems) -> td_status { return dev_alloc(e->ws_allocs, p, elems * es); };
    td_status st;
    const size_t b = B;
    const int H2 = Hp / 4, W2 = Wp / 4;
    if ((st = AA(&e->stem_out, b * (Hp / 2) * (Wp / 2) * e->stem_c)) < 0) return st;
    if ((st = AA(&e->pool_out, b * H2 * W2 * e->stem_c)) < 0) return st;
    int hs[5], wsz[5];
    for (int l = 0; l < 4; ++l) {
        hs[l] = Hp >> (l + 2);
        wsz[l] = Wp >> (l + 2);
    }
    hs[4] = (hs[3] - 1) / 2 + 1;
    wsz[4] = (wsz[3] - 1) / 2 + 1;
    for (int s = 0; s < 4; ++s) {
        const size_t px = b * hs[s] * wsz[s];
        const int mid = e->stages[s][0].c1.cout, co = e->stages[s][0].c3.cout;
        if ((st = AA(&e->t1[s], px * mid)) < 0) return st;
        if ((st = AA(&e->t2[s], px * mid)) < 0) return st;
        if ((st = AA(&e->scb[s], px * co)) < 0) return st;
        if ((st = AA(&e->res[s], px * co)) < 0) return st;
        if ((st = AA(&e->xtmp[s], px * co)) < 0) return st;
        if ((st = AA(&e->inner[s], px * e->fpn_c)) < 0) return st;
    }
    size_t total_anchors = 0;
    for (int l = 0; l < 5; ++l) {
        const size_t px = b * hs[l] * wsz[l];
        if ((st = AA(&e->pfeat[l], px * e->fpn_c)) < 0) return st;
        if ((st = A(&e->rpn_headbuf[l], px * RPN_HEAD_C)) < 0) return st;
        total_anchors += (size_t)hs[l] * wsz[l] * RPN_A;
    }
    if ((st = AA(&e->rpn_t, b * hs[0] * wsz[0] * e->fpn_c)) < 0) return st;
    if ((st = A(&e->key_ws, rpn_topk_ws_elems((int)b, (int)total_anchors))) < 0) return st;
    const size_t nc = b * RPN_LEVELS * RPN_CAND;
    if ((st = A(&e->cand_boxes, nc * 4)) < 0) return st;
    if ((st = A(&e->cand_scores, nc)) < 0) return st;
    if ((st = A(&e->cand_valid, nc)) < 0) return st;
    if ((st = A(&e->cand_idx, nc)) < 0) return st;
    if ((st = A(&e->nms_mask, nc * (RPN_CAND / 64))) < 0) return st;
    if ((st = A(&e->rpn_keep, nc)) < 0) return st;
    if ((st = A(&e->rpn_keep_count, b * RPN_LEVELS)) < 0) return st;
    const int P = e->desc.post_nms_topk, D = e->desc.detections_per_image;
    if ((st = A(&e->props, b * P * 4)) < 0) return st;
    if ((st = A(&e->prop_scores, b * P)) < 0) return st;
    if ((st = A(&e->prop_count, b)) < 0) return st;
    if ((st = AA(&e->pooled7, b * P * 49 * e->fpn_c)) < 0) return st;
    if ((st = AA(&e->fc1_out, b * P * e->fc_dim)) < 0) return st;
    if ((st = AA(&e->fc2_out, b * P * e->fc_dim)) < 0) return st;
    if ((st = A(&e->pred_out, b * P * 6)) < 0) return st;
    if ((st = A(&e->dboxes, b * P * 4)) < 0) return st;
    if ((st = A(&e->dscores, b * P)) < 0) return st;
    if ((st = A(&e->dflags, b * P)) < 0) return st;
    if ((st = A(&e->sboxes, b * P * 4)) < 0) return st;
    if ((st = A(&e->sscores, b * P)) < 0) return st;
    if ((st = A(&e->sidx, b * P)) < 0) return st;
    if ((st = A(&e->scount, b)) < 0) return st;
    if ((st = A(&e->det_keep, b * D)) < 0) return st;
    if ((st = A(&e->det_keep_count, b)) < 0) return st;
    if ((st = A(&e->det_boxes_net, b * D * 4)) < 0) return st;
    const size_t mrows = b * D;
    if ((st = AA(&e->pooled14, mrows * 196 * e->fpn_c)) < 0) return st;
    if ((st = AA(&e->mbuf0, mrows * 196 * e->fpn_c)) < 0) return st;
    if ((st = AA(&e->mbuf1, mrows * 196 * e->fpn_c)) < 0) return st;
    if ((st = AA(&e->deconv_out, mrows * 784 * (e->deconv.cout / 4))) < 0) return st;
    if ((st = A(&e->mask_logits, mrows * 784)) < 0) return st;
    if ((st = A(&e->mask_probs_compact, mrows * 784)) < 0) return st;
    if ((st = A(&e->total_rows, 4)) < 0) return st;
    if ((st = A(&e->o_boxes, b * D * 4)) < 0) return st;
    if ((st = A(&e->o_scores, b * D)) < 0) return st;
    if ((st = A(&e->o_classes, b * D)) < 0) return st;
    if ((st = A(&e->o_count, b)) < 0) return st;
    if ((st = A(&e->o_mask_probs, mrows * 784)) < 0) return st;
    e->wino_v = e->wino_m = nullptr;
    e->wino_elems = 0;
    if (e->desc.precision == TD_PRECISION_FP32 && e->winograd) {
        auto tiles = [](int h, int w) { return (size_t)((h + 1) / 2) * ((w + 1) / 2); };
        size_t need = 0;
        for (int l = 0; l < 5; ++l) need = std::max(need, b * tiles(hs[l], wsz[l]) * (size_t)e->fpn_c);
        for (int s = 0; s < 4; ++s) need = std::max(need, b * tiles(hs[s], wsz[s]) * (size_t)e->stages[s][0].c2.cout);
        need = std::max(need, mrows * tiles(14, 14) * (size_t)e->fpn_c);
        e->wino_elems = 16 * need;
        if ((st = A(&e->wino_v, e->wino_elems)) < 0) return st;
        if ((st = A(&e->wino_m, e->wino_elems)) < 0) return st;
    }
    e->rB = B;
    e->rHp = Hp;
    e->rWp = Wp;
    return TD_OK;
}

}

namespace {

td_status time_launch(td_engine* e, hipStream_t s, hipEvent_t ea, hipEvent_t eb, const std::function<td_status()>& launch, float* ms_out) {
    td_status st = launch();
    if (st < 0) return st;
    static const bool evict = !(getenv("TD_TUNE_EVICT") && atoi(getenv("TD_TUNE_EVICT")) == 0);
    if (evict && !e->tune_evict) {
        e->tune_evict_bytes = (size_t)64 << 20;
        if (hipMalloc(&e->tune_evict, e->tune_evict_bytes) != hipSuccess) {
            (void)hipGetLastError();
            e->tune_evict = nullptr;
            e->tune_evict_bytes = 0;
        }
    }
    const bool cold = evict && e->tune_evict;
    float ms = 1e30f;
    for (int round = 0, reps = cold ? 1 : 2; round < (cold ? 5 : 2); ++round, reps = cold ? 1 : 8) {
        if (cold) TD_HIP_CHECK(hipMemsetAsync(e->tune_evict, round, e->tune_evict_bytes, s));
        TD_HIP_CHECK(hipEventRecord(ea, s));
        for (int rep = 0; rep < reps; ++rep)
            if ((st = launch()) < 0) return st;
        TD_HIP_CHECK(hipEventRecord(eb, s));
        TD_HIP_CHECK(hipEventSynchronize(eb));
        float t = 0.f;
        TD_HIP_CHECK(hipEventElapsedTime(&t, ea, eb));
        t /= (float)reps;
        if (t < ms) ms = t;
        if (!cold && ms > 0.1f) break;
    }
    *ms_out = ms;
    return TD_OK;
}

td_status tuned_cfg(td_engine* e, const std::tuple<int, int, int, int, int>& key, int prec, const ConvArgs& a, hipStream_t s,
                    const std::function<td_status(int)>& launch_cfg, int* cfg_out) {
    const int ksteps = a.KH * a.KW * a.Cin / (prec == TD_PRECISION_FP16 ? 64 : 32);
    auto candidate = [&](int id) {
        const ConvTile* t = conv_tile(id);
        return t && (!t->max_ksteps || ksteps <= t->max_ksteps) && a.Cout >= t->min_cout && (!t->max_cout || a.Cout <= t->max_cout) &&
               !conv_tile_refusal(id, a, prec);
    };
    static const int forced = getenv("TD_FORCE_CFG") ? atoi(getenv("TD_FORCE_CFG")) : -1;
    if (candidate(forced)) {
        *cfg_out = forced;
        return TD_OK;
    }
    auto it = e->tuned.find(key);
    if (it == e->tuned.end()) {
        load_tune_cache(e);
        it = e->tuned.find(key);
    }
    if (it != e->tuned.end()) {
        *cfg_out = it->second;
        return TD_OK;
    }
    std::vector<int> order;
    for (const ConvTile& t : TD_CONV_TILES)
        if (t.tune_rank >= 0 && candidate((int)(&t - TD_CONV_TILES))) order.push_back((int)(&t - TD_CONV_TILES));
    std::sort(order.begin(), order.end(), [](int x, int y) { return TD_CONV_TILES[x].tune_rank < TD_CONV_TILES[y].tune_rank; });
    float best = 1e30f;
    int best_cfg = -1;
    hipEvent_t ea, eb;
    TD_HIP_CHECK(hipEventCreate(&ea));
    TD_HIP_CHECK(hipEventCreate(&eb));
    td_status st = TD_OK;
    for (int c : order) {
        float ms = 1e30f;
        if ((st = time_launch(e, s, ea, eb, [&]() { return launch_cfg(c); }, &ms)) < 0) break;
        static const float hyst = 1.f - 0.01f * (getenv("TD_TUNE_HYST") ? (float)atof(getenv("TD_TUNE_HYST")) : 2.f);
        if (best_cfg < 0 || ms < best * hyst) { best = ms; best_cfg = c; }
    }
    (void)hipEventDestroy(ea);
    (void)hipEventDestroy(eb);
    if (st < 0) return st;
    e->tuned.emplace(key, best_cfg);
    if (FILE* f = e->tune_cache.empty() ? nullptr : fopen(e->tune_cache.c_str(), "a")) {
        fprintf(f, "%d %d %d %d %d %d %d\n", prec, std::get<0>(key), std::get<1>(key), std::get<2>(key), std::get<3>(key), std::get<4>(key), best_cfg);
        fclose(f);
    }
    *cfg_out = best_cfg;
    return TD_OK;
}

ConvArgs wino_plane_args(const td_engine* e, const ConvLayer& L, const void* x, int B, int H, int W, int n, long long t0,
                         const int* m_dyn, int m_mul) {
    ConvArgs a{};
    a.w = L.wino_u; a.y = e->wino_m;
    a.Cin = L.cin; a.Cout = L.cout; a.KH = a.KW = 1; a.stride = 1; a.pad = 0;
    a.M = n; a.m_dyn = m_dyn; a.m_mul = m_dyn ? m_mul / 4 : 1;
    a.m_off = (int)t0;
    a.w_bs = (long long)L.cout * L.cin; a.y_bs = (long long)n * L.cout;
    if (e->wino_fused) { a.x = x; a.B = B; a.H = H; a.W = W; }
    else { a.x = e->wino_v; a.B = 1; a.H = 1; a.W = n; a.Ho = 1; a.Wo = n; a.batch_count = 16; a.x_bs = (long long)n * L.cin; }
    return a;
}

ConvArgs wino43_plane_args(const td_engine* e, const ConvLayer& L, int B, int H, int W, const int* m_dyn) {
    const int tiles_img = ((H + 3) / 4) * ((W + 3) / 4);
    const long long T = (long long)B * tiles_img;
    ConvArgs a{};
    a.x = e->wino_v; a.w = L.wino_u43; a.y = e->wino_m;
    a.Cin = L.cin; a.Cout = L.cout; a.KH = a.KW = 1; a.stride = 1; a.pad = 0;
    a.B = 1; a.H = 1; a.W = (int)T; a.Ho = 1; a.Wo = (int)T;
    a.M = (int)T; a.m_dyn = m_dyn; a.m_mul = m_dyn ? tiles_img : 1;
    a.batch_count = 36; a.x_bs = T * L.cin; a.w_bs = (long long)L.cout * L.cin; a.y_bs = T * L.cout;
    return a;
}

td_status forward_impl(td_engine* e, unsigned phase_mask, hipStream_t s) {
    const td_engine::FwdCtx& c = e->ctx;
    const void* images = c.images;
    const int input_format = c.input_format, B = c.B, Hp = c.Hp, Wp = c.Wp;
    const ImgSizes& valid = c.valid;
    const ImgSizes& outsz = c.outsz;
    const td_detections* out = &c.out;
    const int prec = e->desc.precision;
    auto PH = [&](int k) { return (phase_mask >> k) & 1u; };
    if (PH(0)) e->named.clear();
    td_status st;
    auto run_wino = [&](const ConvLayer& L, const void* x_, int B_, int H_, int W_, bool relu, void* y_, hipStream_t s_,
                        const int* m_dyn, int m_mul, int gemm_cfg) -> td_status {
        const long long T = (long long)B_ * ((H_ + 1) / 2) * ((W_ + 1) / 2);
        const int Ts = wino_slab_tiles(e, L);
        for (long long t0 = 0; t0 < T; t0 += Ts) {
            const int n = (int)std::min<long long>(Ts, T - t0);
            td_status st2;
            ConvArgs a = wino_plane_args(e, L, x_, B_, H_, W_, n, t0, m_dyn, m_mul);
            const double xb = 4.0 * B_ * H_ * W_ * L.cin, yb = 4.0 * B_ * H_ * W_ * L.cout, ub = 4.0 * 16 * L.cout * L.cin;
            const double vb = 4.0 * 16 * n * L.cin, mb = 4.0 * 16 * n * L.cout, pf = 2.0 * 16 * n * (double)L.cin * L.cout;
            const bool dyn = m_dyn != nullptr;
            if (e->wino_fused) {
                ClassScope cs(e, s_, dyn ? TD_CLS_MASK_HEAD : TD_CLS_WINO_GEMM, dyn ? 0.0 : pf, dyn ? 0.0 : xb + ub + mb);
                if ((st2 = wino_gemm_launch(a, s_)) < 0) return st2;
            } else {
                { ClassScope cs(e, s_, dyn ? TD_CLS_MASK_HEAD : TD_CLS_WINO_XFORM, 0.0, dyn ? 0.0 : xb + vb);
                if ((st2 = wino_input_launch(static_cast<const float*>(x_), B_, H_, W_, L.cin, e->wino_v, m_dyn, m_mul, t0, n, s_)) < 0) return st2; }
                a.tile_cfg = gemm_cfg;
                ClassScope cs(e, s_, dyn ? TD_CLS_MASK_HEAD : TD_CLS_WINO_GEMM, dyn ? 0.0 : pf, dyn ? 0.0 : vb + ub + mb);
                if ((st2 = conv2d_launch(a, TD_PRECISION_FP32, s_)) < 0) return st2;
            }
            ClassScope cs(e, s_, dyn ? TD_CLS_MASK_HEAD : TD_CLS_WINO_XFORM, 0.0, dyn ? 0.0 : mb + yb);
            if ((st2 = wino_output_launch(e->wino_m, B_, H_, W_, L.cout, L.scale, L.bias, relu ? 1 : 0, static_cast<float*>(y_), m_dyn,
                                          m_mul, t0, n, s_)) < 0) return st2;
        }
        return TD_OK;
    };
    auto run_wino43 = [&](const ConvLayer& L, const void* x_, int B_, int H_, int W_, bool relu, void* y_, hipStream_t s_,
                          const int* m_dyn, int gemm_cfg, const ConvLayer* head = nullptr, float* head_y = nullptr, bool fold = false) -> td_status {
        const int tiles_img = ((H_ + 3) / 4) * ((W_ + 3) / 4);
        const long long T = (long long)B_ * tiles_img;
        td_status st2;
        const bool dyn = m_dyn != nullptr;
        const double xb = 4.0 * B_ * H_ * W_ * L.cin, yb = 4.0 * B_ * H_ * W_ * L.cout, ub = 4.0 * 36 * L.cout * L.cin;
        const double vb = 4.0 * 36 * T * L.cin, mb = 4.0 * 36 * T * L.cout, pf = 2.0 * 36 * T * (double)L.cin * L.cout;
        if (fold) {
            const unsigned long long per_img = 36ull * tiles_img * (unsigned long long)std::max(L.cin, L.cout) * 4ull;
            const int gmax = (int)std::max<unsigned long long>(1ull, std::min<unsigned long long>((0xfffffff0ull - (2u << 20)) / per_img,
                                                                                                 (0xfffffff0ull - (2u << 20)) / (16ull * tiles_img * L.cout * 4ull)));
            for (int b0 = 0; b0 < B_; b0 += gmax) {
                const int Bg = dyn ? B_ : std::min(gmax, B_ - b0);
                const float* xg = static_cast<const float*>(x_) + (size_t)b0 * H_ * W_ * L.cin;
                float* yg = static_cast<float*>(y_) + (size_t)b0 * H_ * W_ * L.cout;
                const double share = (double)Bg / B_;
                { ClassScope cs(e, s_, dyn ? TD_CLS_MASK_HEAD : TD_CLS_WINO_XFORM, 0.0, dyn ? 0.0 : (xb + vb) * share);
                if ((st2 = wino43_input_launch(xg, Bg, H_, W_, L.cin, e->wino_v, m_dyn, s_)) < 0) return st2; }
                ClassScope cs(e, s_, dyn ? TD_CLS_MASK_HEAD : TD_CLS_WINO_GEMM, dyn ? 0.0 : pf * share, dyn ? 0.0 : (vb + yb) * share + ub);
                if ((st2 = wino43_fused_launch(e->wino_v, static_cast<const float*>(L.wino_u43), Bg, H_, W_, L.cin, L.cout, L.scale, L.bias, relu ? 1 : 0,
                                               yg, m_dyn, s_)) < 0) return st2;
                if (dyn) break;
            }
            return TD_OK;
        }
        { ClassScope cs(e, s_, dyn ? TD_CLS_MASK_HEAD : TD_CLS_WINO_XFORM, 0.0, dyn ? 0.0 : xb + vb);
        if ((st2 = wino43_input_launch(static_cast<const float*>(x_), B_, H_, W_, L.cin, e->wino_v, m_dyn, s_)) < 0) return st2; }
        ConvArgs a = wino43_plane_args(e, L, B_, H_, W_, m_dyn);
        a.tile_cfg = gemm_cfg;
        { ClassScope cs(e, s_, dyn ? TD_CLS_MASK_HEAD : TD_CLS_WINO_GEMM, dyn ? 0.0 : pf, dyn ? 0.0 : vb + ub + mb);
        if ((st2 = conv2d_launch(a, TD_PRECISION_FP32, s_)) < 0) return st2; }
        if (head) {
            const double hflops = 2.0 * B_ * H_ * W_ * (double)head->cout * L.cout, hb = 4.0 * B_ * H_ * W_ * head->cout + 4.0 * head->cout * L.cout;
            if (e->prof) {
                e->prof_flops[0] += hflops;
                e->prof_flops[8] += hflops;
                e->prof_launches[0] += 1;
                e->prof_bytes[0] += hb + yb;
            }
            ClassScope cs(e, s_, TD_CLS_WINO_XFORM, hflops, mb + hb);
            return wino43_output_head_launch(e->wino_m, B_, H_, W_, L.cout, L.scale, L.bias, relu ? 1 : 0, static_cast<const float*>(head->w),
                                             head->bias, head_y, head->cout, s_);
        }
        ClassScope cs(e, s_, dyn ? TD_CLS_MASK_HEAD : TD_CLS_WINO_XFORM, 0.0, dyn ? 0.0 : mb + yb);
        return wino43_output_launch(e->wino_m, B_, H_, W_, L.cout, L.scale, L.bias, relu ? 1 : 0, static_cast<float*>(y_), m_dyn, s_);
    };
    auto run_conv = [&](const ConvLayer& L, const void* x_, int B_, int H_, int W_, int stride, int pad, bool relu,
                        void* y_, const void* res_, int res_shift, hipStream_t s_, int prec_,
                        const int* m_dyn = nullptr, int m_mul = 1, int out_mode = 0,
                        const ConvLayer* head = nullptr, float* head_y = nullptr, bool* head_fused = nullptr) -> td_status {
        const int Ho = (H_ + 2 * pad - L.kh) / stride + 1, Wo = (W_ + 2 * pad - L.kw) / stride + 1;
        const double M = (double)B_ * Ho * Wo, K = (double)L.kh * L.kw * L.cin;
        const double flops = 2.0 * M * L.cout * K;
        const double es = prec_ == TD_PRECISION_FP16 ? 2.0 : 4.0;
        const double bytes = es * ((double)B_ * H_ * W_ * L.cin / (stride * stride) + M * L.cout * (res_ ? 2.0 : 1.0) + L.cout * K);
        int cfg = -1, wino_cfg = -1;
        bool use_wino = false, use_43 = false, use_fold = false;
        td_status st2;
        ConvArgs ca{};
        ca.x = x_; ca.w = L.w; ca.w_frag = L.w_frag; ca.scale = L.scale; ca.bias = L.bias; ca.res = res_; ca.y = y_;
        ca.B = B_; ca.H = H_; ca.W = W_; ca.Cin = L.cin; ca.Cout = L.cout; ca.KH = L.kh; ca.KW = L.kw;
        ca.stride = stride; ca.pad = pad; ca.Ho = Ho; ca.Wo = Wo;
        ca.res_shift = res_shift; ca.relu = relu ? 1 : 0; ca.out_mode = out_mode;
        ca.M = B_ * Ho * Wo; ca.m_dyn = m_dyn; ca.m_mul = m_mul; ca.tile_cfg = -1; ca.out_f32 = L.out_f32 ? 1 : 0;
        if (e->autotune) {
            const auto key = std::make_tuple(L.cout, L.cin, L.kh * 16 + L.kw, B_ * Ho * Wo, stride * 4 + out_mode * 2 + (res_ ? 1 : 0));
            auto direct = [&](int c) { ConvArgs a = ca; a.tile_cfg = c; return conv2d_launch(a, prec_, s_); };
            const bool wino_ok = prec_ == TD_PRECISION_FP32 && L.wino_u && e->wino_v && stride == 1 && pad == 1 && !res_ && out_mode == 0 &&
                                 (!m_dyn || ((H_ | W_) & 1) == 0) &&
                                 (size_t)16 * std::min<long long>((long long)B_ * ((H_ + 1) / 2) * ((W_ + 1) / 2), wino_slab_tiles(e, L)) *
                                         (size_t)std::max(L.cin, L.cout) <= e->wino_elems;
            if (wino_ok) {
                const int T = (int)std::min<long long>((long long)B_ * ((H_ + 1) / 2) * ((W_ + 1) / 2), wino_slab_tiles(e, L));
                const auto wkey = std::make_tuple(L.cout, L.cin, 1 * 16 + 1, T, 4 + 32);
                auto wino = [&](int c) { return run_wino(L, x_, B_, H_, W_, relu, y_, s_, m_dyn, m_mul, c); };
                use_wino = L.cin >= e->wino_minc && L.cout >= e->wino_minc;
                const long long T43 = (long long)B_ * ((H_ + 3) / 4) * ((W_ + 3) / 4);
                use_43 = use_wino && L.wino_u43 && e->wino43_min > 0 && H_ >= e->wino43_min && W_ >= e->wino43_min &&
                         (size_t)36 * T43 * (size_t)std::max(L.cin, L.cout) <= e->wino_elems && T43 * std::max(L.cin, L.cout) < (1ll << 31);
                const int hw_ = H_ * W_, wf_ = e->wino_fold;
                use_fold = use_43 && wf_ > 0 && wino43_fused_ok(m_dyn ? B_ : 1, H_, W_, L.cin, L.cout) &&
                           (((wf_ & 1) && !m_dyn && (!head || (wf_ & 32)) && ((L.cin == 256 && hw_ >= 160 * 160) || (L.cin == 128 && hw_ >= 80 * 80))) ||
                            ((wf_ & 2) && m_dyn && !head) || ((wf_ & 4) && !m_dyn && !head && L.cin == 256 && hw_ >= 80 * 80) ||
                            ((wf_ & 8) && !m_dyn && !head && hw_ >= 40 * 40) || ((wf_ & 16) && !m_dyn && !head));
                if (use_43 && !use_fold) {
                    const auto key43 = std::make_tuple(L.cout, L.cin, 1 * 16 + 1, (int)T43, 4 + 64);
                    auto w43 = [&](int c) { return run_wino43(L, x_, B_, H_, W_, relu, y_, s_, m_dyn, c); };
                    if ((st2 = tuned_cfg(e, key43, prec_, wino43_plane_args(e, L, B_, H_, W_, m_dyn), s_, w43, &wino_cfg)) < 0) return st2;
                }
                if (use_wino && !use_43 && !e->wino_fused &&
                    (st2 = tuned_cfg(e, wkey, prec_, wino_plane_args(e, L, x_, B_, H_, W_, T, 0, m_dyn, m_mul), s_, wino, &wino_cfg)) < 0) return st2;
            }
            if (!use_wino && (st2 = tuned_cfg(e, key, prec_, ca, s_, direct, &cfg)) < 0) return st2;
        }
        ProfScope ps(e, s_, m_dyn ? 7 : 0, m_dyn ? 0.0 : flops, m_dyn ? 0.0 : bytes);
        if (e->prof && !m_dyn) {
            const double padded = use_43 ? (double)(((H_ + 3) / 4) * 4) * (((W_ + 3) / 4) * 4) / ((double)H_ * W_) : 1.0;
            e->prof_flops[8] += use_43 ? flops * padded * 0.25 : (use_wino ? flops * 4.0 / 9.0 : flops);
            e->prof_launches[8] += use_wino ? 1 : 0;
        }
        if (use_43) {
            const bool fuse43 = head && !use_fold && e->fuse_head && !m_dyn && relu && L.cout == 256 && head->cin == 256 && head->kh == 1 && head->kw == 1 &&
                                head->cout <= 32 && !head->scale;
            if (head_fused) *head_fused = fuse43;
            return run_wino43(L, x_, B_, H_, W_, relu, y_, s_, m_dyn, wino_cfg, fuse43 ? head : nullptr, fuse43 ? head_y : nullptr, use_fold);
        }
        if (use_wino) return run_wino(L, x_, B_, H_, W_, relu, y_, s_, m_dyn, m_mul, wino_cfg);
        const int cls = m_dyn ? TD_CLS_MASK_HEAD : (H_ == 1 && W_ == 1 ? TD_CLS_FC : (L.kh == 1 && L.kw == 1 ? TD_CLS_CONV1X1 : TD_CLS_CONV3X3));
        const bool fuse_head = head && e->fuse_head && !m_dyn && out_mode == 0 && !res_ && relu && L.cout == 256 && head->cin == 256 &&
                               head->kh == 1 && head->kw == 1 && head->cout <= 32 && head->out_f32 && !head->scale && conv_head_capable(cfg, prec_);
        if (head_fused) *head_fused = fuse_head;
        ca.tile_cfg = cfg;
        if (fuse_head) {
            const double hflops = 2.0 * M * head->cout * L.cout, hbytes = 4.0 * M * head->cout + es * head->cout * L.cout;
            const double bytes_f = bytes - es * M * L.cout + hbytes;
            if (e->prof) {
                e->prof_flops[0] += hflops;
                e->prof_flops[8] += hflops;
                e->prof_launches[0] += 1;
                e->prof_bytes[0] += hbytes + es * M * L.cout;
            }
            ca.head_w = head->w; ca.head_b = head->bias; ca.head_y = head_y; ca.head_n = head->cout;
            ClassScope cs(e, s_, cls, flops + hflops, bytes_f);
            return conv2d_launch(ca, prec_, s_);
        }
        ClassScope cs(e, s_, cls, m_dyn ? 0.0 : flops, m_dyn ? 0.0 : bytes);
        return conv2d_launch(ca, prec_, s_);
    };
    auto groupable = [&](const ConvLayer& L) {
        return L.kh == 3 && L.kw == 3 && L.cout == 256 && L.cin % 64 == 0 && !L.scale && L.bias && !L.out_f32;
    };
    auto run_grouped = [&](const ConvLayer* const* Ls, const void* const* xs, void* const* ys, float* const* head_ys, int nl, const int* Hs,
                           const int* Ws, bool relu, const ConvLayer* head, hipStream_t s_) -> td_status {
        ConvArgs a{};
        a.B = B; a.Cin = Ls[0]->cin; a.Cout = 256; a.KH = a.KW = 3; a.stride = 1; a.pad = 1; a.relu = relu ? 1 : 0; a.m_mul = 1; a.nlev = nl;
        a.tile_cfg = 17;
        double flops = 0.0, bytes = 0.0, unfused_bytes = 0.0;
        for (int l = 0; l < nl; ++l) {
            a.lev[l].x = xs[l]; a.lev[l].w = Ls[l]->w; a.lev[l].bias = Ls[l]->bias;
            a.lev[l].y = ys ? ys[l] : nullptr; a.lev[l].head_y = head_ys ? head_ys[l] : nullptr;
            a.lev[l].H = Hs[l]; a.lev[l].W = Ws[l];
            const double M = (double)B * Hs[l] * Ws[l], K = 9.0 * a.Cin;
            flops += 2.0 * M * 256 * K + (head ? 2.0 * M * head->cout * 256 : 0.0);
            bytes += 2.0 * (M * a.Cin + (head ? 0.0 : M * 256) + 256 * K) + (head ? 4.0 * M * head->cout + 2.0 * head->cout * 256 : 0.0);
            unfused_bytes += head ? 2.0 * 2.0 * M * 256 : 0.0;
        }
        if (head) { a.head_w = head->w; a.head_b = head->bias; a.head_n = head->cout; }
        ProfScope ps(e, s_, 0, flops, bytes + unfused_bytes);
        if (e->prof) {
            e->prof_flops[8] += flops;
            e->prof_launches[0] += nl * (head ? 2 : 1) - 1;
        }
        ClassScope cs(e, s_, TD_CLS_CONV3X3, flops, bytes);
        return conv_pp8_grouped_launch(a, s_);
    };
    auto run_tail = [&](const Block& blk, const void* t1_, int B_, int H_, int W_, void* y_, const void* shortcut_, hipStream_t s_) -> td_status {
        TailArgs a{};
        a.x = t1_; a.w2 = blk.c2.w; a.scale2 = blk.c2.scale; a.bias2 = blk.c2.bias;
        a.w3 = blk.c3.w; a.scale3 = blk.c3.scale; a.bias3 = blk.c3.bias; a.res = shortcut_; a.y = y_;
        a.B = B_; a.H = H_; a.W = W_; a.MID = blk.c2.cout; a.COUT = blk.c3.cout; a.M = B_ * H_ * W_;
        const double M = (double)a.M, mid = a.MID, co = a.COUT, es = prec == TD_PRECISION_FP16 ? 2.0 : 4.0;
        const double flops = 2.0 * M * mid * (9.0 * mid) + 2.0 * M * co * mid;
        const double bytes = es * (M * mid + 2.0 * M * co + 9.0 * mid * mid + co * mid);
        ProfScope ps(e, s_, 0, flops, bytes);
        if (e->prof) {
            e->prof_flops[8] += flops;
            e->prof_launches[0] += 1;
            e->prof_bytes[0] += es * 2.0 * M * mid;
        }
        ClassScope cs(e, s_, TD_CLS_TAIL, flops, bytes);
        return bottleneck_tail_launch(a, prec, s_);
    };
    int hs[5], wsz[5];
    for (int l = 0; l < 4; ++l) {
        hs[l] = Hp >> (l + 2);
        wsz[l] = Wp >> (l + 2);
    }
    hs[4] = (hs[3] - 1) / 2 + 1;
    wsz[4] = (wsz[3] - 1) / 2 + 1;
    const size_t esz = prec == TD_PRECISION_FP16 ? 2 : 4;
    auto off = [&](void* p, size_t elems) -> void* { return static_cast<char*>(p) + elems * esz; };
    int sb = e->backbone_subbatch > 0 ? e->backbone_subbatch : B;
    if (sb > B) sb = B;
    const bool do_stem = PH(6) || (PH(0) && !e->stem_done);
    std::optional<ProfScope> trunk_group;
    for (int b0 = 0; (PH(0) || PH(6)) && b0 < B; b0 += sb) {
        const int nb_img = (B - b0) < sb ? (B - b0) : sb;
        ImgSizes vsub{};
        for (int i = 0; i < nb_img; ++i) {
            vsub.h[i] = valid.h[b0 + i];
            vsub.w[i] = valid.w[b0 + i];
        }
        const size_t in_img = input_format == TD_INPUT_U8_HWC ? (size_t)Hp * Wp * 3 : (size_t)Hp * Wp * 3 * 4;
        const void* img_sub = static_cast<const char*>(images) + (size_t)b0 * in_img;
        void* stem_sub = off(e->stem_out, (size_t)b0 * (Hp / 2) * (Wp / 2) * e->stem_c);
        void* pool_sub = off(e->pool_out, (size_t)b0 * hs[0] * wsz[0] * e->stem_c);
        if (do_stem) {
            { ProfScope ps(e, s, 1);
            if ((st = stem_launch(img_sub, input_format, vsub, nb_img, Hp, Wp, e->stem_w, e->stem_scale, e->stem_bias, stem_sub,
                                  e->stem_c, prec, s, e->stem_w16, e->stem_bias16)) < 0) return st; }
            { ProfScope ps(e, s, 2);
            if ((st = maxpool3x3s2_launch(stem_sub, pool_sub, nb_img, Hp / 2, Wp / 2, e->stem_c, prec, s)) < 0) return st; }
        }
        if (!PH(0)) continue;
        if (!trunk_group && sb >= B) trunk_group.emplace(e, s, 0, 0.0, 0.0, true);
        const void* x = pool_sub;
        int xh = hs[0], xw = wsz[0];
        ProfScope backbone_group(e, s, 0, 0.0, 0.0, true);
        for (int si = 0; si < 4; ++si) {
            const int nb = (int)e->stages[si].size();
            const int oh = hs[si], ow = wsz[si];
            const size_t px = (size_t)b0 * oh * ow;
            const int mid = e->stages[si][0].c1.cout, co = e->stages[si][0].c3.cout;
            void* t1 = off(e->t1[si], px * mid);
            void* t2 = off(e->t2[si], px * mid);
            void* scb = off(e->scb[si], px * co);
            void* resb = off(e->res[si], px * co);
            void* xtmp = off(e->xtmp[si], px * co);
            for (int bi = 0; bi < nb; ++bi) {
                const Block& blk = e->stages[si][bi];
                void* y = ((nb - 1 - bi) % 2 == 0) ? resb : xtmp;
                const void* shortcut = x;
                if (blk.has_sc) {
                    if ((st = run_conv(blk.sc, x, nb_img, xh, xw, blk.stride, 0, false, scb, nullptr, 0, s, prec)) < 0) return st;
                    shortcut = scb;
                }
                if ((st = run_conv(blk.c1, x, nb_img, xh, xw, blk.stride, 0, true, t1, nullptr, 0, s, prec)) < 0) return st;
                if (e->fuse_tail && (blk.c2.cout == 64 || e->fuse_tail_fp16) && blk.c2.kh == 3 && blk.c2.kw == 3 &&
                    blk.c2.cin == blk.c2.cout && blk.c3.cin == blk.c2.cout && bottleneck_tail_ok(prec, blk.c2.cout, blk.c3.cout)) {
                    if ((st = run_tail(blk, t1, nb_img, oh, ow, y, shortcut, s)) < 0) return st;
                } else {
                    if ((st = run_conv(blk.c2, t1, nb_img, oh, ow, 1, 1, true, t2, nullptr, 0, s, prec)) < 0) return st;
                    if ((st = run_conv(blk.c3, t2, nb_img, oh, ow, 1, 0, true, y, shortcut, 0, s, prec)) < 0) return st;
                }
                x = y;
                xh = oh;
                xw = ow;
            }
        }
    }
    if (PH(0)) {
    set_named(e, "stem", e->stem_out, B, Hp / 2, Wp / 2, e->stem_c, (int)esz);
    set_named(e, "pool", e->pool_out, B, Hp / 4, Wp / 4, e->stem_c, (int)esz);
    for (int si = 0; si < 4; ++si) {
        const std::string nm = "res" + std::to_string(si + 2);
        set_named(e, nm.c_str(), e->res[si], B, hs[si], wsz[si], e->stages[si][0].c3.cout, (int)esz);
    }
    {
    ProfScope fpn_group(e, s, 0, 0.0, 0.0, true);
    const bool group_fpn = prec == TD_PRECISION_FP16 && e->group_levels && groupable(e->fpn_out[0]) && groupable(e->fpn_out[1]) &&
                           groupable(e->fpn_out[2]) && groupable(e->fpn_out[3]);
    for (int l = 3; l >= 0; --l) {
        const void* td_res = l == 3 ? nullptr : e->inner[l + 1];
        if ((st = run_conv(e->lateral[l], e->res[l], B, hs[l], wsz[l], 1, 0, false, e->inner[l], td_res, td_res ? 1 : 0, s, prec)) < 0) return st;
        if (!group_fpn && (st = run_conv(e->fpn_out[l], e->inner[l], B, hs[l], wsz[l], 1, 1, false, e->pfeat[l], nullptr, 0, s, prec)) < 0) return st;
    }
    if (group_fpn) {
        const ConvLayer* Ls[4] = {&e->fpn_out[0], &e->fpn_out[1], &e->fpn_out[2], &e->fpn_out[3]};
        const void* xs[4] = {e->inner[0], e->inner[1], e->inner[2], e->inner[3]};
        void* ys[4] = {e->pfeat[0], e->pfeat[1], e->pfeat[2], e->pfeat[3]};
        if ((st = run_grouped(Ls, xs, ys, nullptr, 4, hs, wsz, false, nullptr, s)) < 0) return st;
    }
    }
    { ProfScope ps(e, s, 2);
    if ((st = subsample2_launch(e->pfeat[3], e->pfeat[4], B, hs[3], wsz[3], e->fpn_c, prec, s)) < 0) return st; }
    for (int l = 0; l < 5; ++l) {
        const std::string nm = "p" + std::to_string(l + 2);
        set_named(e, nm.c_str(), e->pfeat[l], B, hs[l], wsz[l], e->fpn_c, (e->desc.precision == TD_PRECISION_FP16 ? 2 : 4));
    }
    {
        ProfScope rpn_group(e, s, 0, 0.0, 0.0, true);
        const bool group_rpn = prec == TD_PRECISION_FP16 && e->group_levels && e->fuse_head && groupable(e->rpn_conv) && e->rpn_head.cin == 256 &&
                               e->rpn_head.kh == 1 && e->rpn_head.kw == 1 && e->rpn_head.cout <= 32 && e->rpn_head.out_f32 && !e->rpn_head.scale;
        if (group_rpn) {
            const ConvLayer* Ls[5] = {&e->rpn_conv, &e->rpn_conv, &e->rpn_conv, &e->rpn_conv, &e->rpn_conv};
            const void* xs[5] = {e->pfeat[0], e->pfeat[1], e->pfeat[2], e->pfeat[3], e->pfeat[4]};
            float* hy[5] = {e->rpn_headbuf[0], e->rpn_headbuf[1], e->rpn_headbuf[2], e->rpn_headbuf[3], e->rpn_headbuf[4]};
            if ((st = run_grouped(Ls, xs, nullptr, hy, 5, hs, wsz, true, &e->rpn_head, s)) < 0) return st;
        }
        for (int l = 0; l < 5; ++l) {
            if (group_rpn) {
                const std::string nm = "rpn_head" + std::to_string(l + 2);
                set_named(e, nm.c_str(), e->rpn_headbuf[l], B, hs[l], wsz[l], RPN_HEAD_C);
                continue;
            }
            bool fused = false;
            if ((st = run_conv(e->rpn_conv, e->pfeat[l], B, hs[l], wsz[l], 1, 1, true, e->rpn_t, nullptr, 0, s, prec, nullptr, 1, 0,
                               &e->rpn_head, e->rpn_headbuf[l], &fused)) < 0) return st;
            if (!fused && (st = run_conv(e->rpn_head, e->rpn_t, B, hs[l], wsz[l], 1, 0, false, e->rpn_headbuf[l], nullptr, 0, s, prec)) < 0) return st;
            const std::string nm = "rpn_head" + std::to_string(l + 2);
            set_named(e, nm.c_str(), e->rpn_headbuf[l], B, hs[l], wsz[l], RPN_HEAD_C);
        }
    }
    trunk_group.reset();
    }
    RpnLevels lv{};
    {
        static const int sizes[5] = {32, 64, 128, 256, 512};
        static const double ratios[3] = {0.5, 1.0, 2.0};
        int off = 0;
        for (int l = 0; l < 5; ++l) {
            lv.head[l] = e->rpn_headbuf[l];
            lv.h[l] = hs[l];
            lv.w[l] = wsz[l];
            lv.stride[l] = 4 << l;
            lv.anchor_off[l] = off;
            off += hs[l] * wsz[l] * RPN_A;
            const double area = (double)sizes[l] * sizes[l];
            for (int a = 0; a < 3; ++a) {
                const double w = std::sqrt(area / ratios[a]);
                const double h = ratios[a] * w;
                lv.base[l][a][0] = (float)(-w / 2.0);
                lv.base[l][a][1] = (float)(-h / 2.0);
                lv.base[l][a][2] = (float)(w / 2.0);
                lv.base[l][a][3] = (float)(h / 2.0);
            }
        }
        lv.total_anchors = off;
    }
    const int P = e->desc.post_nms_topk, D = e->desc.detections_per_image;
    FeatLevels fl{};
    for (int l = 0; l < 4; ++l) {
        fl.feat[l] = e->pfeat[l];
        fl.h[l] = hs[l];
        fl.w[l] = wsz[l];
        fl.scale[l] = 1.0f / (float)(4 << l);
    }
    fl.C = e->fpn_c;
    float* o_boxes = out->boxes ? out->boxes : e->o_boxes;
    float* o_scores = out->scores ? out->scores : e->o_scores;
    int* o_classes = out->classes ? out->classes : e->o_classes;
    int* o_count = out->count ? out->count : e->o_count;
    float* o_probs = out->mask_probs ? out->mask_probs : e->o_mask_probs;
    const int mrows = B * D;
    if (PH(1)) {
    { ProfScope ps(e, s, 3);
    if ((st = rpn_topk_decode_launch(lv, valid, B, e->desc.pre_nms_topk, e->key_ws, e->cand_boxes, e->cand_scores,
                                     e->cand_valid, e->cand_idx, s)) < 0) return st; }
    set_named(e, "rpn_cand_boxes", e->cand_boxes, B, RPN_LEVELS, RPN_CAND, 4);
    set_named(e, "rpn_cand_scores", e->cand_scores, B, RPN_LEVELS, RPN_CAND);
    set_named(e, "rpn_cand_valid", e->cand_valid, B, RPN_LEVELS, RPN_CAND);
    set_named(e, "rpn_cand_idx", e->cand_idx, B, RPN_LEVELS, RPN_CAND);
    { ProfScope ps(e, s, 3);
    if ((st = nms_launch(e->cand_boxes, nullptr, e->cand_valid, B * RPN_LEVELS, RPN_CAND, e->desc.rpn_nms_thresh,
                         e->nms_mask, e->rpn_keep, e->rpn_keep_count, RPN_CAND, s)) < 0) return st; }
    set_named(e, "rpn_keep", e->rpn_keep, B, RPN_LEVELS, RPN_CAND);
    set_named(e, "rpn_keep_count", e->rpn_keep_count, B, RPN_LEVELS);
    { ProfScope ps(e, s, 3);
    if ((st = rpn_merge_launch(e->cand_boxes, e->cand_scores, e->rpn_keep, e->rpn_keep_count, B, P, e->props,
                               e->prop_scores, e->prop_count, P, s)) < 0) return st; }
    set_named(e, "proposals", e->props, B, P, 4);
    set_named(e, "proposal_scores", e->prop_scores, B, P);
    set_named(e, "proposal_count", e->prop_count, B);
    { ProfScope ps(e, s, 4);
    if ((st = roi_align_launch(fl, e->props, e->prop_count, B, P, 7, 0, e->pooled7, nullptr, prec, s)) < 0) return st; }
    set_named(e, "pooled7", e->pooled7, (int64_t)B * P, 7, 7, e->fpn_c, (e->desc.precision == TD_PRECISION_FP16 ? 2 : 4));
    }
    if (PH(2)) {
    {
    ProfScope box_group(e, s, 0, 0.0, 0.0, true);
    if ((st = run_conv(e->fc1, e->pooled7, B * P, 1, 1, 1, 0, true, e->fc1_out, nullptr, 0, s, prec)) < 0) return st;
    if ((st = run_conv(e->fc2, e->fc1_out, B * P, 1, 1, 1, 0, true, e->fc2_out, nullptr, 0, s, prec)) < 0) return st;
    if ((st = run_conv(e->pred, e->fc2_out, B * P, 1, 1, 1, 0, false, e->pred_out, nullptr, 0, s, prec)) < 0) return st;
    }
    set_named(e, "box_pred", e->pred_out, (int64_t)B * P, 6);
    }
    if (PH(3)) {
    { ProfScope ps(e, s, 5);
    if ((st = det_decode_launch(e->pred_out, 6, e->props, e->prop_count, valid, B, P, e->desc.score_thresh, e->dboxes,
                                e->dscores, e->dflags, s)) < 0) return st; }
    set_named(e, "det_all_boxes", e->dboxes, B, P, 4);
    set_named(e, "det_all_scores", e->dscores, B, P);
    set_named(e, "det_flags", e->dflags, B, P);
    { ProfScope ps(e, s, 5);
    if ((st = sort_boxes_launch(e->dboxes, e->dscores, e->dflags, e->prop_count, B, P, e->sboxes, e->sscores, e->sidx,
                                e->scount, s)) < 0) return st; }
    { ProfScope ps(e, s, 5);
    if ((st = nms_launch(e->sboxes, e->scount, nullptr, B, P, e->desc.nms_thresh, e->nms_mask, e->det_keep,
                         e->det_keep_count, D, s)) < 0) return st; }
    { ProfScope ps(e, s, 5);
    if ((st = det_finalize_launch(e->sboxes, e->sscores, e->det_keep, e->det_keep_count, valid, outsz, B, P, D,
                                  e->det_boxes_net, o_boxes, o_scores, o_classes, o_count, s)) < 0) return st; }
    set_named(e, "det_boxes_net", e->det_boxes_net, B, D, 4);
    { ProfScope ps(e, s, 4);
    if ((st = roi_align_launch(fl, e->det_boxes_net, o_count, B, D, 14, 1, e->pooled14, e->total_rows, prec, s)) < 0) return st; }
    set_named(e, "pooled14", e->pooled14, mrows, 14, 14, e->fpn_c, (e->desc.precision == TD_PRECISION_FP16 ? 2 : 4));
    }
    if (PH(4)) {
    const void* mx = e->pooled14;
    void* mbuf[2] = {e->mbuf0, e->mbuf1};
    {
    ProfScope mask_group(e, s, 7, 0.0, 0.0, true);
    for (int i = 0; i < 4; ++i) {
        if ((st = run_conv(e->mask_fcn[i], mx, mrows, 14, 14, 1, 1, true, mbuf[i & 1], nullptr, 0, s, prec, e->total_rows, 196)) < 0) return st;
        mx = mbuf[i & 1];
    }
    if ((st = run_conv(e->deconv, mx, mrows, 14, 14, 1, 0, true, e->deconv_out, nullptr, 0, s, prec, e->total_rows, 196, 1)) < 0) return st;
    }
    set_named(e, "mask_deconv", e->deconv_out, mrows, 28, 28, e->deconv.cout / 4, (e->desc.precision == TD_PRECISION_FP16 ? 2 : 4));
    }
    if (PH(5)) {
    { ProfScope ps(e, s, 6);
    if ((st = mask_predict_launch(e->deconv_out, e->mask_pred_w, e->mask_pred_b, e->deconv.cout / 4, mrows * 784,
                                  e->total_rows, 784, e->mask_logits, e->mask_probs_compact, prec, s)) < 0) return st; }
    set_named(e, "mask_logits", e->mask_logits, mrows, 28, 28);
    { ProfScope ps(e, s, 6);
    if ((st = mask_scatter_launch(e->mask_probs_compact, o_count, B, D, o_probs, s)) < 0) return st; }
    if (out->mask_bits) {
        { ProfScope ps(e, s, 6);
        if ((st = paste_masks_launch(o_probs, o_boxes, o_count, outsz, B, D, e->desc.mask_thresh, out->mask_region,
                                     reinterpret_cast<long long*>(out->mask_offset), out->mask_bits,
                                     out->mask_words_per_image, s)) < 0) return st; }
    }
    }
    return TD_OK;
}

td_status set_forward_ctx(td_engine* e, const void* images, int input_format, const int32_t* hw_valid,
                          const int32_t* hw_out, int B, int Hp, int Wp, const td_detections* out) {
    TD_REQUIRE(e && images && hw_valid && hw_out && out, "td_engine_forward: null argument");
    TD_REQUIRE(e->loaded, "td_engine_forward: load weights first");
    TD_REQUIRE(input_format == TD_INPUT_F32_CHW || input_format == TD_INPUT_U8_HWC, "td_engine_forward: bad input format %d", input_format);
    TD_REQUIRE(B >= 1 && Hp % 32 == 0 && Wp % 32 == 0 && Hp >= 64 && Wp >= 64, "td_engine_forward: bad batch geometry B=%d %dx%d", B, Hp, Wp);
    if (B > e->rB || Hp > e->rHp || Wp > e->rWp) {
        td_set_error("td_engine_forward: B=%d %dx%d exceeds the reserved B=%d %dx%d", B, Hp, Wp, e->rB, e->rHp, e->rWp);
        return TD_ERR_CAPACITY;
    }
    td_engine::FwdCtx& c = e->ctx;
    c.valid_ctx = false;
    for (int i = 0; i < B; ++i) {
        c.valid.h[i] = hw_valid[2 * i];
        c.valid.w[i] = hw_valid[2 * i + 1];
        c.outsz.h[i] = hw_out[2 * i];
        c.outsz.w[i] = hw_out[2 * i + 1];
// ... 163 lines not shown
```

treedetection_amd/csrc/wino_fused.hip:

```cpp
#include "common.h"
#include "conv_tiles.h"
#include <utility>

namespace {

struct WinoFusedArgs {
    const float* V;
    const float* U;
    const float* scale;
    const float* bias;
    float* y;
    const int* m_dyn;
    int B, H, W, C, N, relu;
    long long T;
};

constexpr int WF_BN = 64;

__constant__ float WF_AT[4][6] = {{1.f, 1.f, 1.f, 1.f, 1.f, 0.f}, {0.f, 1.f, -1.f, 2.f, -2.f, 0.f}, {0.f, 1.f, 1.f, 4.f, 4.f, 0.f}, {0.f, 1.f, -1.f, 8.f, -8.f, 1.f}};

template <class F, int... I>
__device__ __forceinline__ void wf_static_for_impl(F&& f, std::integer_sequence<int, I...>) {
    (f(std::integral_constant<int, I>{}), ...);
}
template <int N, class F>
__device__ __forceinline__ void wf_static_for(F&& f) {
    wf_static_for_impl(f, std::make_integer_sequence<int, N>{});
}

template <int NS, int KREP, int NWT, int VAR>
__global__ __launch_bounds__(NWT * 128, 2) void wino43_fused_kernel(const WinoFusedArgs a) {
    constexpr int AHEAD = NS - 1;
    constexpr int WF_BT = 16 * NWT, THREADS = 128 * NWT;
    constexpr int DROWS = THREADS / 8;
    constexpr int NU = WF_BN / DROWS;
    constexpr int NDMA = 1 + NU;
    constexpr int WF_STAGE = (WF_BT + WF_BN) * CHUNK_BYTES;
    static_assert((NWT == 2 || NWT == 4) && (NS == 4 || NS == 8) && KREP >= 1 && NS * WF_STAGE <= 160 * 1024 && DROWS == WF_BT, "geometry");
    __shared__ __attribute__((aligned(16))) char lds[NS * WF_STAGE];

    const int TH = (a.H + 3) >> 2, TW = (a.W + 3) >> 2;
    long long live = a.T;
    if (a.m_dyn) {
        const long long n = (long long)*a.m_dyn * TH * TW;
        live = n < live ? n : live;
    }
    const int tb_n = (int)((live + WF_BT - 1) / WF_BT), nb_n = a.N / WF_BN;
    const int nblk = tb_n * nb_n;
    if ((int)blockIdx.x >= nblk) return;
    const int pid = xcd_remap(blockIdx.x, nblk);
    const int tb = pid / nb_n, nb = pid - tb * nb_n;
    const long long t0 = (long long)tb * WF_BT;
    const int n0 = nb * WF_BN;

    const int tid = threadIdx.x, lane = tid & 63;
    const int wave = __builtin_amdgcn_readfirstlane(tid >> 6);
    const int wt = wave & (NWT - 1), wc = wave / NWT;
    constexpr int KC = NS * KREP;

    constexpr unsigned OOB = 0xfffffff0u;
    const unsigned row_bytes = (unsigned)a.C * 4u;
    const unsigned planeV = (unsigned)((unsigned long long)a.T * row_bytes), planeU = (unsigned)a.N * row_bytes;
    const __amdgpu_buffer_rsrc_t vrsrc = __builtin_amdgcn_make_buffer_rsrc(const_cast<float*>(a.V), 0, (int)(36u * planeV), 0x00020000);
    const __amdgpu_buffer_rsrc_t ursrc = __builtin_amdgcn_make_buffer_rsrc(const_cast<float*>(a.U), 0, (int)(36u * planeU), 0x00020000);
    const int ld_c = tid & 7, ld_r = tid >> 3;
    const unsigned src_piece = (unsigned)(ld_c ^ ((ld_r >> 1) & 7)) * 16u;
    const bool v_ok = t0 + ld_r < live;
    const unsigned v_off = (unsigned)(t0 + ld_r) * row_bytes + src_piece;
    const unsigned u_off = (unsigned)(n0 + ld_r) * row_bytes + src_piece;
    typedef __attribute__((address_space(3))) void lds_void;
    char* const dstV = lds + wave * 8 * CHUNK_BYTES;
    char* const dstU = lds + WF_BT * CHUNK_BYTES + wave * 8 * CHUNK_BYTES;
    int ld_kc = 0;
    unsigned ld_v = 0, ld_u = 0;
    auto issue = [&](auto st_c) __attribute__((always_inline)) {
        constexpr int ST = decltype(st_c)::value;
        __builtin_amdgcn_raw_ptr_buffer_load_lds(vrsrc, (lds_void*)(dstV + ST * WF_STAGE), 16, v_ok ? v_off + ld_v : OOB, 0, 0, 0);
        __builtin_amdgcn_raw_ptr_buffer_load_lds(ursrc, (lds_void*)(dstU + ST * WF_STAGE), 16, u_off + ld_u, 0, 0, 0);
        if constexpr (NU == 2)
            __builtin_amdgcn_raw_ptr_buffer_load_lds(ursrc, (lds_void*)(dstU + ST * WF_STAGE + DROWS * CHUNK_BYTES), 16, u_off + (unsigned)DROWS * row_bytes + ld_u, 0, 0, 0);
        ld_v += CHUNK_BYTES;
        ld_u += CHUNK_BYTES;
        if (++ld_kc == KC) {
            ld_kc = 0;
            ld_v += planeV - row_bytes;
            ld_u += planeU - row_bytes;
        }
    };

    const unsigned r16 = lane & 15, q = lane >> 4, swz = (r16 >> 1) & 7;
    const unsigned pc0 = ((0u + q) ^ swz) * 16u, pc1 = ((4u + q) ^ swz) * 16u;
    const unsigned fv = (unsigned)(wt * 16 + r16) * CHUNK_BYTES;
    const unsigned fu = (unsigned)(WF_BT + wc * 32 + r16) * CHUNK_BYTES;
    struct Frag { f32x4 u0, u1, v; };
    auto read_frag = [&](Frag& f, auto st_c, unsigned pc) __attribute__((always_inline)) {
        if constexpr (VAR & 32) {
            asm volatile("" : "+v"(f.u0), "+v"(f.u1), "+v"(f.v));
            return;
        }
        const char* sb = lds + decltype(st_c)::value * WF_STAGE;
        f.u0 = *reinterpret_cast<const f32x4*>(sb + fu + pc);
        f.u1 = *reinterpret_cast<const f32x4*>(sb + fu + 16 * CHUNK_BYTES + pc);
        f.v = *reinterpret_cast<const f32x4*>(sb + fv + pc);
    };
    f32x4 acc[2][2];
    auto mma = [&](const Frag& f, auto set_c, auto&& filler, auto slot0_c) __attribute__((always_inline)) {
        constexpr int SET = decltype(set_c)::value, SLOT0 = decltype(slot0_c)::value;
        if constexpr (VAR & 16) {
            asm volatile("" ::"v"(f.u0), "v"(f.u1), "v"(f.v));
            wf_static_for<4>([&](auto e_c) __attribute__((always_inline)) { filler(std::integral_constant<int, SLOT0 + decltype(e_c)::value>{}); });
            return;
        }
        wf_static_for<4>([&](auto e_c) __attribute__((always_inline)) {
            constexpr int e = decltype(e_c)::value;
            acc[SET][0] = __builtin_amdgcn_mfma_f32_16x16x4f32(f.u0[e], f.v[e], acc[SET][0], 0, 0, 0);
            acc[SET][1] = __builtin_amdgcn_mfma_f32_16x16x4f32(f.u1[e], f.v[e], acc[SET][1], 0, 0, 0);
            __builtin_amdgcn_sched_barrier(0);
            filler(std::integral_constant<int, SLOT0 + e>{});
            __builtin_amdgcn_sched_barrier(0);
        });
    };

    f32x4 Y[16][2], S[4][2];
#pragma unroll
    for (int i = 0; i < 16; ++i) Y[i][0] = Y[i][1] = f32x4{0.f, 0.f, 0.f, 0.f};
#pragma unroll
    for (int j = 0; j < 4; ++j) S[j][0] = S[j][1] = f32x4{0.f, 0.f, 0.f, 0.f};
    acc[0][0] = acc[0][1] = acc[1][0] = acc[1][1] = f32x4{0.f, 0.f, 0.f, 0.f};

    auto fold_s = [&](auto xc_c, auto set_c, auto sl_c) __attribute__((always_inline)) {
        constexpr int XC = decltype(xc_c)::value, SET = decltype(set_c)::value, sl = decltype(sl_c)::value, b = sl >> 2, e = sl & 3;
        const float m = acc[SET][b][e];
        acc[SET][b][e] = 0.f;
        if constexpr (XC <= 4) S[0][b][e] = __fadd_rn(S[0][b][e], m);
        if constexpr (XC == 1) {
            S[1][b][e] = __fadd_rn(S[1][b][e], m);
            S[2][b][e] = __fadd_rn(S[2][b][e], m);
            S[3][b][e] = __fadd_rn(S[3][b][e], m);
        } else if constexpr (XC == 2) {
            S[1][b][e] = __fsub_rn(S[1][b][e], m);
            S[2][b][e] = __fadd_rn(S[2][b][e], m);
            S[3][b][e] = __fsub_rn(S[3][b][e], m);
        } else if constexpr (XC == 3) {
            S[1][b][e] = __fmaf_rn(2.f, m, S[1][b][e]);
            S[2][b][e] = __fmaf_rn(4.f, m, S[2][b][e]);
            S[3][b][e] = __fmaf_rn(8.f, m, S[3][b][e]);
        } else if constexpr (XC == 4) {
            S[1][b][e] = __fmaf_rn(-2.f, m, S[1][b][e]);
            S[2][b][e] = __fmaf_rn(4.f, m, S[2][b][e]);
            S[3][b][e] = __fmaf_rn(-8.f, m, S[3][b][e]);
        } else if constexpr (XC == 5) {
            S[3][b][e] = __fadd_rn(S[3][b][e], m);
        }
    };
    float r0 = 0.f, r1 = 0.f, r2 = 0.f, r3 = 0.f;
    auto fold_y = [&](auto sl_c) __attribute__((always_inline)) {
        constexpr int sl = decltype(sl_c)::value, b = sl >> 2, e = sl & 3;
#pragma unroll
        for (int j = 0; j < 4; ++j) {
            const float v = S[j][b][e];
            S[j][b][e] = 0.f;
            Y[0 + j][b][e] = __fmaf_rn(r0, v, Y[0 + j][b][e]);
            Y[4 + j][b][e] = __fmaf_rn(r1, v, Y[4 + j][b][e]);
            Y[8 + j][b][e] = __fmaf_rn(r2, v, Y[8 + j][b][e]);
            Y[12 + j][b][e] = __fmaf_rn(r3, v, Y[12 + j][b][e]);
        }
    };

    wf_static_for<AHEAD>([&](auto i_c) __attribute__((always_inline)) { issue(i_c); });
    asm volatile("s_waitcnt vmcnt(%0)" ::"n"(NDMA * (AHEAD - 1)) : "memory");
    __builtin_amdgcn_s_barrier();
    Frag f0, f1;
    if constexpr (VAR & 32) {
        f0.u0 = f0.u1 = f0.v = f32x4{1.f, 2.f, 3.f, 4.f};
        f1 = f0;
    }
    read_frag(f0, std::integral_constant<int, 0>{}, pc0);

    auto ring_pass = [&](auto xc_c, auto fold_c) __attribute__((always_inline)) {
        constexpr int XC = decltype(xc_c)::value, SET = XC & 1, PXC = (XC + 5) % 6;
        constexpr bool FOLD = decltype(fold_c)::value;
        wf_static_for<NS>([&](auto st_c) __attribute__((always_inline)) {
            constexpr int ST = decltype(st_c)::value, NEXT = (ST + 1) % NS;
            auto filler = [&](auto slot_c) __attribute__((always_inline)) {
                if constexpr (FOLD && ST == 0) fold_s(std::integral_constant<int, PXC>{}, std::integral_constant<int, 1 - SET>{}, slot_c);
                if constexpr (FOLD && ST == 1 && PXC == 5) fold_y(slot_c);
            };
            if constexpr (!(VAR & 8)) issue(std::integral_constant<int, (ST + AHEAD) % NS>{});
            read_frag(f1, st_c, pc1);
            mma(f0, std::integral_constant<int, SET>{}, filler, std::integral_constant<int, 0>{});
            if constexpr (!(VAR & 8)) asm volatile("s_waitcnt vmcnt(%0)" ::"n"(NDMA * (AHEAD - 1)) : "memory");
            asm volatile("s_waitcnt lgkmcnt(0)" ::: "memory");
            __builtin_amdgcn_sched_barrier(0);
            if constexpr (!(VAR & 64)) __builtin_amdgcn_s_barrier();
            read_frag(f0, std::integral_constant<int, NEXT>{}, pc0);
            mma(f1, std::integral_constant<int, SET>{}, filler, std::integral_constant<int, 4>{});
        });
    };
    auto plane = [&](auto xc_c) __attribute__((always_inline)) {
        ring_pass(xc_c, std::true_type{});
        if constexpr (KREP > 1) {
#pragma unroll 1
            for (int rep = 1; rep < KREP; ++rep) ring_pass(xc_c, std::false_type{});
        }
    };
    for (int xr = 0; xr < 6; ++xr) {
        r0 = xr ? WF_AT[0][xr - 1] : 0.f; r1 = xr ? WF_AT[1][xr - 1] : 0.f; r2 = xr ? WF_AT[2][xr - 1] : 0.f; r3 = xr ? WF_AT[3][xr - 1] : 0.f;
        wf_static_for<6>(plane);
    }
    asm volatile("s_waitcnt vmcnt(0)" ::: "memory");
    wf_static_for<8>([&](auto sl_c) __attribute__((always_inline)) { fold_s(std::integral_constant<int, 5>{}, std::integral_constant<int, 1>{}, sl_c); });
    r0 = WF_AT[0][5]; r1 = WF_AT[1][5]; r2 = WF_AT[2][5]; r3 = WF_AT[3][5];
    wf_static_for<8>([&](auto sl_c) __attribute__((always_inline)) { fold_y(sl_c); });

    const long long t = t0 + wt * 16 + (int)r16;
    const bool tlive = t < live;
    const unsigned tt = tlive ? (unsigned)t : 0u;
    const unsigned tyx = tt % (unsigned)(TW * TH);
    const unsigned b = tt / (unsigned)(TW * TH);
    const unsigned ty = tyx / (unsigned)TW, tx = tyx - ty * (unsigned)TW;
    const __amdgpu_buffer_rsrc_t yrsrc = __builtin_amdgcn_make_buffer_rsrc(a.y, 0, (int)((unsigned)a.B * a.H * a.W * a.N * 4u), 0x00020000);
    f32x4 sc[2], bi[2];
#pragma unroll
    for (int blk = 0; blk < 2; ++blk) {
        const int n = n0 + wc * 32 + blk * 16 + 4 * (int)q;
        sc[blk] = a.scale ? *reinterpret_cast<const f32x4*>(a.scale + n) : f32x4{1.f, 1.f, 1.f, 1.f};
        bi[blk] = a.bias ? *reinterpret_cast<const f32x4*>(a.bias + n) : f32x4{0.f, 0.f, 0.f, 0.f};
    }
    const unsigned pix0 = (b * (unsigned)a.H + 4u * ty) * (unsigned)a.W + 4u * tx;
    const unsigned nbytes = (unsigned)a.N * 4u;
#pragma unroll
    for (int i = 0; i < 4; ++i) {
        const bool rok = tlive && (int)(4u * ty) + i < a.H;
#pragma unroll
        for (int j = 0; j < 4; ++j) {
            const bool ok = rok && (int)(4u * tx) + j < a.W;
            const unsigned pbase = (pix0 + (unsigned)(i * a.W + j)) * nbytes;
#pragma unroll
            for (int blk = 0; blk < 2; ++blk) {
                f32x4 v = Y[4 * i + j][blk];
#pragma unroll
                for (int e = 0; e < 4; ++e) {
                    float o = v[e];
                    if (a.scale) o = __fmul_rn(o, sc[blk][e]);
                    if (a.bias) o = __fadd_rn(o, bi[blk][e]);
                    if (a.relu) o = o > 0.f ? o : 0.f;
                    v[e] = o;
                }
                const unsigned off = ok ? pbase + (unsigned)(n0 + wc * 32 + blk * 16 + 4 * (int)q) * 4u : OOB;
                __builtin_amdgcn_raw_buffer_store_b128(__builtin_bit_cast(__attribute__((ext_vector_type(4))) unsigned, v), yrsrc, off, 0, 0);
            }
        }
    }
}

}

bool wino43_fused_ok(int B, int H, int W, int C, int N) {
    const long long T = (long long)B * ((H + 3) / 4) * ((W + 3) / 4);
    return (C == 128 || C == 256 || C == 512) && N >= WF_BN && N % WF_BN == 0 && 36ull * (unsigned long long)T * C * 4 < 0xfffffff0ull - (1u << 20) &&
           36ull * (unsigned long long)N * C * 4 < 0xfffffff0ull - (1u << 20) && (unsigned long long)B * H * W * N * 4 < 0xfffffff0ull - (1u << 20);
}

td_status wino43_fused_launch(const float* V, const float* U, int B, int H, int W, int C, int N, const float* scale, const float* bias,
                              int relu, float* y, const int* m_dyn, hipStream_t s) {
    TD_REQUIRE(V && U && y && B >= 1 && H >= 1 && W >= 1, "winograd F(4x4) fused contraction: bad arguments");
    TD_REQUIRE(wino43_fused_ok(B, H, W, C, N), "winograd F(4x4) fused contraction: needs C = 128, 256 or 512, N %% 64 == 0 and planes below 4 GB (C %d, N %d)", C, N);
    WinoFusedArgs a{};
    a.V = V; a.U = U; a.scale = scale; a.bias = bias; a.y = y; a.m_dyn = m_dyn;
    a.B = B; a.H = H; a.W = W; a.C = C; a.N = N; a.relu = relu;
    a.T = (long long)B * ((H + 3) / 4) * ((W + 3) / 4);
    static const int num_cu = [] {
        int dev = 0, n = 0;
        if (hipGetDevice(&dev) != hipSuccess || hipDeviceGetAttribute(&n, hipDeviceAttributeMultiprocessorCount, dev) != hipSuccess || n < 64) n = 256;
        return n;
    }();
    const long long blocks64 = ((a.T + 63) / 64) * (N / WF_BN);
    int nwt = (C == 512 || (blocks64 < num_cu && !m_dyn)) ? 2 : 4;
    if (const char* f = getenv("TD_WF_NWT")) {
        const int v = atoi(f);
        if ((v == 2 || v == 4) && !(v == 4 && C == 512)) nwt = v;
    }
    const long long blocks = ((a.T + 16 * nwt - 1) / (16 * nwt)) * (N / WF_BN);
    TD_REQUIRE(blocks < (1ll << 31), "winograd F(4x4) fused contraction: grid too large");
#define TD_WF_LAUNCH(NSV, KREPV, NWTV, VARV) hipLaunchKernelGGL((wino43_fused_kernel<NSV, KREPV, NWTV, VARV>), dim3((unsigned)blocks), dim3(128 * NWTV), 0, s, a)
#if defined(TD_WF_DIAG)
    const int var = getenv("TD_WF_VAR") ? atoi(getenv("TD_WF_VAR")) : 0;
    if (var && C == 256 && nwt == 4) {
        switch (var) {
            case 8: TD_WF_LAUNCH(8, 1, 4, 8); break;
            case 16: TD_WF_LAUNCH(8, 1, 4, 16); break;
            case 32: TD_WF_LAUNCH(8, 1, 4, 32); break;
            case 40: TD_WF_LAUNCH(8, 1, 4, 40); break;
            case 104: TD_WF_LAUNCH(8, 1, 4, 104); break;
            default: TD_WF_LAUNCH(8, 1, 4, 0); break;
        }
        TD_KERNEL_CHECK();
        return TD_OK;
    }
#endif
    if (nwt == 4) {
        if (C == 256) TD_WF_LAUNCH(8, 1, 4, 0);
        else TD_WF_LAUNCH(4, 1, 4, 0);
    } else {
        if (C == 512) TD_WF_LAUNCH(4, 4, 2, 0);
        else if (C == 256) TD_WF_LAUNCH(4, 2, 2, 0);
        else TD_WF_LAUNCH(4, 1, 2, 0);
    }
#undef TD_WF_LAUNCH
    TD_KERNEL_CHECK();
    return TD_OK;
}
```

treedetection_amd/csrc/winograd.hip:

```cpp
#include "common.h"

namespace {

__global__ __launch_bounds__(256) void wino_input_kernel(const float* __restrict__ x, int B, int H, int W, int C,
                                                         float* __restrict__ V, const int* __restrict__ m_dyn, int m_mul,
                                                         long long t0, int Ts) {
    const int TH = (H + 1) >> 1, TW = (W + 1) >> 1;
    int nimg = B;
    if (m_dyn) {
        const int n = (int)(((long long)*m_dyn * m_mul) / ((long long)H * W));
        nimg = n < B ? n : B;
    }
    const int c4n = C >> 2;
    const long long T = Ts;
    const long long idx = (long long)blockIdx.x * blockDim.x + threadIdx.x;
    const long long tl = idx / c4n;
    const int c = (int)(idx - tl * c4n) * 4;
    const long long t = t0 + tl;
    if (tl >= Ts || t >= (long long)nimg * TH * TW) return;
    const int tx = (int)(t % TW);
    const int ty = (int)((t / TW) % TH);
    const int b = (int)(t / ((long long)TW * TH));
    const int y0 = 2 * ty - 1, x0 = 2 * tx - 1;
    float4 d[4][4];
#pragma unroll
    for (int i = 0; i < 4; ++i) {
        const int yy = y0 + i;
#pragma unroll
        for (int j = 0; j < 4; ++j) {
            const int xx = x0 + j;
            if ((unsigned)yy < (unsigned)H && (unsigned)xx < (unsigned)W)
                d[i][j] = *reinterpret_cast<const float4*>(x + (((size_t)b * H + yy) * W + xx) * C + c);
            else
                d[i][j] = make_float4(0.f, 0.f, 0.f, 0.f);
        }
    }
#define TD_SUB(a, b) make_float4(__fsub_rn(a.x, b.x), __fsub_rn(a.y, b.y), __fsub_rn(a.z, b.z), __fsub_rn(a.w, b.w))
#define TD_ADD(a, b) make_float4(__fadd_rn(a.x, b.x), __fadd_rn(a.y, b.y), __fadd_rn(a.z, b.z), __fadd_rn(a.w, b.w))
    float4 r[4][4];
#pragma unroll
    for (int j = 0; j < 4; ++j) {
        r[0][j] = TD_SUB(d[0][j], d[2][j]);
        r[1][j] = TD_ADD(d[1][j], d[2][j]);
        r[2][j] = TD_SUB(d[2][j], d[1][j]);
        r[3][j] = TD_SUB(d[1][j], d[3][j]);
    }
#pragma unroll
    for (int i = 0; i < 4; ++i) {
        const float4 v0 = TD_SUB(r[i][0], r[i][2]);
        const float4 v1 = TD_ADD(r[i][1], r[i][2]);
        const float4 v2 = TD_SUB(r[i][2], r[i][1]);
        const float4 v3 = TD_SUB(r[i][1], r[i][3]);
        float* p = V + ((size_t)(4 * i) * T + tl) * C + c;
        *reinterpret_cast<float4*>(p) = v0;
        *reinterpret_cast<float4*>(p + (size_t)T * C) = v1;
        *reinterpret_cast<float4*>(p + (size_t)2 * T * C) = v2;
        *reinterpret_cast<float4*>(p + (size_t)3 * T * C) = v3;
    }
}

__global__ __launch_bounds__(256) void wino_output_kernel(const float* __restrict__ Mb, int B, int H, int W, int N,
                                                          const float* __restrict__ scale, const float* __restrict__ bias,
                                                          int relu, float* __restrict__ y, const int* __restrict__ m_dyn,
                                                          int m_mul, long long t0, int Ts) {
    const int TH = (H + 1) >> 1, TW = (W + 1) >> 1;
    int nimg = B;
    if (m_dyn) {
        const int n = (int)(((long long)*m_dyn * m_mul) / ((long long)H * W));
        nimg = n < B ? n : B;
    }
    const int c4n = N >> 2;
    const long long T = Ts;
    const long long idx = (long long)blockIdx.x * blockDim.x + threadIdx.x;
    const long long tl = idx / c4n;
    const int c = (int)(idx - tl * c4n) * 4;
    const long long t = t0 + tl;
    if (tl >= Ts || t >= (long long)nimg * TH * TW) return;
    const int tx = (int)(t % TW);
    const int ty = (int)((t / TW) % TH);
    const int b = (int)(t / ((long long)TW * TH));
    float4 m[4][4];
#pragma unroll
    for (int i = 0; i < 4; ++i)
#pragma unroll
        for (int j = 0; j < 4; ++j) m[i][j] = *reinterpret_cast<const float4*>(Mb + ((size_t)(4 * i + j) * T + tl) * N + c);
    float4 s[2][4];
#pragma unroll
    for (int j = 0; j < 4; ++j) {
        s[0][j] = TD_ADD(TD_ADD(m[0][j], m[1][j]), m[2][j]);
        s[1][j] = TD_SUB(TD_SUB(m[1][j], m[2][j]), m[3][j]);
    }
    float4 sc = make_float4(1.f, 1.f, 1.f, 1.f), bi = make_float4(0.f, 0.f, 0.f, 0.f);
    if (scale) sc = *reinterpret_cast<const float4*>(scale + c);
    if (bias) bi = *reinterpret_cast<const float4*>(bias + c);
#pragma unroll
    for (int i = 0; i < 2; ++i) {
        const int yy = 2 * ty + i;
        if (yy >= H) continue;
        const float4 o0 = TD_ADD(TD_ADD(s[i][0], s[i][1]), s[i][2]);
        const float4 o1 = TD_SUB(TD_SUB(s[i][1], s[i][2]), s[i][3]);
#pragma unroll
        for (int j = 0; j < 2; ++j) {
            const int xx = 2 * tx + j;
            if (xx >= W) continue;
            float4 v = j ? o1 : o0;
            if (scale) v = make_float4(__fmul_rn(v.x, sc.x), __fmul_rn(v.y, sc.y), __fmul_rn(v.z, sc.z), __fmul_rn(v.w, sc.w));
            if (bias) v = TD_ADD(v, bi);
            if (relu) v = make_float4(v.x > 0.f ? v.x : 0.f, v.y > 0.f ? v.y : 0.f, v.z > 0.f ? v.z : 0.f, v.w > 0.f ? v.w : 0.f);
            *reinterpret_cast<float4*>(y + (((size_t)b * H + yy) * W + xx) * N + c) = v;
        }
    }
#undef TD_SUB
#undef TD_ADD
}


#define TD_SUB(a, b) make_float4(__fsub_rn(a.x, b.x), __fsub_rn(a.y, b.y), __fsub_rn(a.z, b.z), __fsub_rn(a.w, b.w))
#define TD_ADD(a, b) make_float4(__fadd_rn(a.x, b.x), __fadd_rn(a.y, b.y), __fadd_rn(a.z, b.z), __fadd_rn(a.w, b.w))
#define TD_MUL(k, a) make_float4(__fmul_rn(k, a.x), __fmul_rn(k, a.y), __fmul_rn(k, a.z), __fmul_rn(k, a.w))

__device__ __forceinline__ void wino43_bt(const float4 (&d)[6], float4 (&t)[6]) {
    const float4 a = TD_SUB(d[4], TD_MUL(4.f, d[2]));
    const float4 b = TD_SUB(d[3], TD_MUL(4.f, d[1]));
    const float4 c = TD_SUB(d[4], d[2]);
    const float4 e = TD_MUL(2.f, TD_SUB(d[3], d[1]));
    t[0] = TD_ADD(TD_SUB(TD_MUL(4.f, d[0]), TD_MUL(5.f, d[2])), d[4]);
    t[1] = TD_ADD(a, b);
    t[2] = TD_SUB(a, b);
    t[3] = TD_ADD(c, e);
    t[4] = TD_SUB(c, e);
    t[5] = TD_ADD(TD_SUB(TD_MUL(4.f, d[1]), TD_MUL(5.f, d[3])), d[5]);
}

__global__ __launch_bounds__(256) void wino43_input_kernel(const float* __restrict__ x, int B, int H, int W, int C,
                                                           float* __restrict__ V, long long T, const int* __restrict__ m_dyn) {
    const int TH = (H + 3) >> 2, TW = (W + 3) >> 2;
    const int c4n = C >> 2;
    const unsigned idx = blockIdx.x * blockDim.x + threadIdx.x;
    const unsigned t = idx / (unsigned)c4n;
    const int c = (int)(idx - t * (unsigned)c4n) * 4;
    long long live = T;
    if (m_dyn) {
        const long long n = (long long)*m_dyn * TH * TW;
        live = n < T ? n : T;
    }
    if ((long long)t >= live) return;
    const unsigned tyx = t % (unsigned)(TW * TH);
    const int b = (int)(t / (unsigned)(TW * TH));
    const int ty = (int)(tyx / (unsigned)TW);
    const int tx = (int)(tyx - (unsigned)ty * (unsigned)TW);
    const int y0 = 4 * ty - 1, x0 = 4 * tx - 1;
    float4 d[6][6];
#pragma unroll
    for (int i = 0; i < 6; ++i) {
        const int yy = y0 + i;
#pragma unroll
        for (int j = 0; j < 6; ++j) {
            const int xx = x0 + j;
            if ((unsigned)yy < (unsigned)H && (unsigned)xx < (unsigned)W)
                d[i][j] = *reinterpret_cast<const float4*>(x + (((size_t)b * H + yy) * W + xx) * C + c);
            else
                d[i][j] = make_float4(0.f, 0.f, 0.f, 0.f);
        }
    }
#pragma unroll
    for (int j = 0; j < 6; ++j) {
        float4 col[6], r[6];
#pragma unroll
        for (int i = 0; i < 6; ++i) col[i] = d[i][j];
        wino43_bt(col, r);
#pragma unroll
        for (int i = 0; i < 6; ++i) d[i][j] = r[i];
    }
#pragma unroll
    for (int i = 0; i < 6; ++i) {
        float4 v[6];
        wino43_bt(d[i], v);
        float* p = V + ((size_t)(6 * i) * T + t) * C + c;
#pragma unroll
        for (int j = 0; j < 6; ++j) *reinterpret_cast<float4*>(p + (size_t)j * T * C) = v[j];
    }
}

__device__ __forceinline__ void wino43_at(const float4 (&m)[6], float4 (&s)[4]) {
    const float4 p12 = TD_ADD(m[1], m[2]), m12 = TD_SUB(m[1], m[2]);
    const float4 p34 = TD_ADD(m[3], m[4]), m34 = TD_SUB(m[3], m[4]);
    s[0] = TD_ADD(TD_ADD(m[0], p12), p34);
    s[1] = TD_ADD(m12, TD_MUL(2.f, m34));
    s[2] = TD_ADD(p12, TD_MUL(4.f, p34));
    s[3] = TD_ADD(TD_ADD(m12, TD_MUL(8.f, m34)), m[5]);
}

__global__ __launch_bounds__(256) void wino43_output_kernel(const float* __restrict__ Mb, int B, int H, int W, int N,
                                                            const float* __restrict__ scale, const float* __restrict__ bias,
                                                            int relu, float* __restrict__ y, long long T,
                                                            const int* __restrict__ m_dyn) {
    const int TH = (H + 3) >> 2, TW = (W + 3) >> 2;
    const int c4n = N >> 2;
    const unsigned idx = blockIdx.x * blockDim.x + threadIdx.x;
    const unsigned t = idx / (unsigned)c4n;
    const int c = (int)(idx - t * (unsigned)c4n) * 4;
    long long live = T;
    if (m_dyn) {
        const long long n = (long long)*m_dyn * TH * TW;
        live = n < T ? n : T;
    }
    if ((long long)t >= live) return;
    const unsigned tyx = t % (unsigned)(TW * TH);
    const int b = (int)(t / (unsigned)(TW * TH));
    const int ty = (int)(tyx / (unsigned)TW);
    const int tx = (int)(tyx - (unsigned)ty * (unsigned)TW);
    float4 s[4][6];
#pragma unroll
    for (int j = 0; j < 6; ++j) {
        float4 col[6], r[4];
#pragma unroll
        for (int i = 0; i < 6; ++i) col[i] = *reinterpret_cast<const float4*>(Mb + ((size_t)(6 * i + j) * T + t) * N + c);
        wino43_at(col, r);
#pragma unroll
        for (int i = 0; i < 4; ++i) s[i][j] = r[i];
    }
    float4 sc = make_float4(1.f, 1.f, 1.f, 1.f), bi = make_float4(0.f, 0.f, 0.f, 0.f);
    if (scale) sc = *reinterpret_cast<const float4*>(scale + c);
    if (bias) bi = *reinterpret_cast<const float4*>(bias + c);
#pragma unroll
    for (int i = 0; i < 4; ++i) {
        const int yy = 4 * ty + i;
        float4 o[4];
        wino43_at(s[i], o);
        if (yy >= H) continue;
#pragma unroll
        for (int j = 0; j < 4; ++j) {
            const int xx = 4 * tx + j;
            if (xx >= W) continue;
            float4 v = o[j];
            if (scale) v = make_float4(__fmul_rn(v.x, sc.x), __fmul_rn(v.y, sc.y), __fmul_rn(v.z, sc.z), __fmul_rn(v.w, sc.w));
            if (bias) v = TD_ADD(v, bi);
            if (relu) v = make_float4(v.x > 0.f ? v.x : 0.f, v.y > 0.f ? v.y : 0.f, v.z > 0.f ? v.z : 0.f, v.w > 0.f ? v.w : 0.f);
            *reinterpret_cast<float4*>(y + (((size_t)b * H + yy) * W + xx) * N + c) = v;
        }
    }
}
__global__ __launch_bounds__(256) void wino43_output_head_kernel(const float* __restrict__ Mb, int B, int H, int W,
                                                                 const float* __restrict__ scale, const float* __restrict__ bias,
                                                                 int relu, long long T, const float* __restrict__ head_w,
                                                                 const float* __restrict__ head_b, float* __restrict__ head_y, int hn) {
    constexpr int N = 256, NH = 128, RS = NH + 4;
    __shared__ __attribute__((aligned(16))) float tile[64 * RS];
    typedef float v4f __attribute__((ext_vector_type(4)));
    typedef float v16f __attribute__((ext_vector_type(16)));
    const int TH = (H + 3) >> 2, TW = (W + 3) >> 2;
    const int lt = threadIdx.x >> 6, c = (threadIdx.x & 63) * 4;
    const int wave = threadIdx.x >> 6, lane = threadIdx.x & 63;
    const long long t = (long long)blockIdx.x * 4 + lt;
    const bool live = t < T;
    float4 s[4][6];
    if (live) {
#pragma unroll
        for (int j = 0; j < 6; ++j) {
            float4 col[6], r[4];
#pragma unroll
            for (int i = 0; i < 6; ++i) col[i] = *reinterpret_cast<const float4*>(Mb + ((size_t)(6 * i + j) * T + t) * N + c);
            wino43_at(col, r);
#pragma unroll
            for (int i = 0; i < 4; ++i) s[i][j] = r[i];
        }
    }
    float4 sc = make_float4(1.f, 1.f, 1.f, 1.f), bi = make_float4(0.f, 0.f, 0.f, 0.f);
    if (scale) sc = *reinterpret_cast<const float4*>(scale + c);
    if (bias) bi = *reinterpret_cast<const float4*>(bias + c);
    float4 px[4][4];
#pragma unroll
    for (int i = 0; i < 4; ++i) {
        float4 o[4];
        if (live) wino43_at(s[i], o);
#pragma unroll
        for (int j = 0; j < 4; ++j) {
            float4 v = make_float4(0.f, 0.f, 0.f, 0.f);
            if (live) {
                v = o[j];
                if (scale) v = make_float4(__fmul_rn(v.x, sc.x), __fmul_rn(v.y, sc.y), __fmul_rn(v.z, sc.z), __fmul_rn(v.w, sc.w));
                if (bias) v = TD_ADD(v, bi);
                if (relu) v = make_float4(v.x > 0.f ? v.x : 0.f, v.y > 0.f ? v.y : 0.f, v.z > 0.f ? v.z : 0.f, v.w > 0.f ? v.w : 0.f);
            }
            px[i][j] = v;
        }
    }
    const int col = lane & 31, hi4 = (lane >> 5) * 4;
    const bool lcol = col < hn;
    v16f acc;
#pragma unroll
    for (int r = 0; r < 16; ++r) acc[r] = 0.f;
    const float* arow = &tile[((wave & 1) * 32 + col) * RS + hi4];
    const float* brow = head_w + (size_t)(lcol ? col : 0) * N + hi4;
#pragma unroll
    for (int half = 0; half < 2; ++half) {
        if (half) __syncthreads();
        if ((c >= NH) == (half == 1)) {
#pragma unroll
            for (int i = 0; i < 4; ++i)
#pragma unroll
                for (int j = 0; j < 4; ++j) *reinterpret_cast<float4*>(&tile[(lt * 16 + i * 4 + j) * RS + (c - half * NH)]) = px[i][j];
        }
        __syncthreads();
        if (wave < 2) {
#pragma unroll 2
            for (int ch = 0; ch < NH / 32; ++ch) {
#pragma unroll
                for (int kk = 0; kk < 4; ++kk) {
                    const v4f fa = *reinterpret_cast<const v4f*>(arow + ch * 32 + 8 * kk);
                    v4f fb = {0.f, 0.f, 0.f, 0.f};
                    if (lcol) fb = *reinterpret_cast<const v4f*>(brow + half * NH + ch * 32 + 8 * kk);
#pragma unroll
                    for (int e = 0; e < 4; ++e) acc = __builtin_amdgcn_mfma_f32_32x32x2f32(fa[e], fb[e], acc, 0, 0, 0);
                }
            }
        }
    }
    if (wave >= 2 || !lcol) return;
    const float hb = head_b ? head_b[col] : 0.f;
#pragma unroll
    for (int r = 0; r < 16; ++r) {
        const int row = wave * 32 + (r & 3) + 8 * (r >> 2) + 4 * (lane >> 5);
        const long long tt = (long long)blockIdx.x * 4 + (row >> 4);
        if (tt >= T) continue;
        const unsigned tyx = (unsigned)(tt % (unsigned)(TW * TH));
        const int b = (int)(tt / (unsigned)(TW * TH));
        const int ty = (int)(tyx / (unsigned)TW), tx = (int)(tyx - (unsigned)ty * (unsigned)TW);
        const int yy = 4 * ty + ((row >> 2) & 3), xx = 4 * tx + (row & 3);
        if (yy >= H || xx >= W) continue;
        head_y[(((size_t)b * H + yy) * W + xx) * hn + col] = head_b ? __fadd_rn(acc[r], hb) : acc[r];
    }
}
#undef TD_SUB
#undef TD_ADD
#undef TD_MUL

}

td_status wino_input_launch(const float* x, int B, int H, int W, int C, float* V, const int* m_dyn, int m_mul, long long t0,
                            int Ts, hipStream_t s) {
    TD_REQUIRE(x && V && B >= 1 && H >= 1 && W >= 1 && C >= 4 && (C & 3) == 0 && Ts >= 1 && t0 >= 0, "winograd input transform: bad arguments");
    const long long threads = (long long)Ts * (C / 4);
    hipLaunchKernelGGL(wino_input_kernel, dim3((unsigned)((threads + 255) / 256)), dim3(256), 0, s, x, B, H, W, C, V, m_dyn, m_mul, t0, Ts);
    TD_KERNEL_CHECK();
    return TD_OK;
}

td_status wino_output_launch(const float* Mb, int B, int H, int W, int N, const float* scale, const float* bias, int relu,
                             float* y, const int* m_dyn, int m_mul, long long t0, int Ts, hipStream_t s) {
    TD_REQUIRE(Mb && y && B >= 1 && H >= 1 && W >= 1 && N >= 4 && (N & 3) == 0 && Ts >= 1 && t0 >= 0, "winograd output transform: bad arguments");
    const long long threads = (long long)Ts * (N / 4);
    hipLaunchKernelGGL(wino_output_kernel, dim3((unsigned)((threads + 255) / 256)), dim3(256), 0, s, Mb, B, H, W, N, scale, bias,
                       relu, y, m_dyn, m_mul, t0, Ts);
    TD_KERNEL_CHECK();
    return TD_OK;
}

void wino_filter_transform(const float* w, int N, int C, float* U) {
    static const double G[4][3] = {{1, 0, 0}, {0.5, 0.5, 0.5}, {0.5, -0.5, 0.5}, {0, 0, 1}};
    for (int n = 0; n < N; ++n)
        for (int c = 0; c < C; ++c) {
            double g[3][3], t[4][3];
            for (int a = 0; a < 3; ++a)
                for (int b = 0; b < 3; ++b) g[a][b] = w[(((size_t)n * 3 + a) * 3 + b) * C + c];
            for (int i = 0; i < 4; ++i)
                for (int b = 0; b < 3; ++b) t[i][b] = G[i][0] * g[0][b] + G[i][1] * g[1][b] + G[i][2] * g[2][b];
            for (int i = 0; i < 4; ++i)
                for (int j = 0; j < 4; ++j)
                    U[((size_t)(4 * i + j) * N + n) * C + c] = (float)(t[i][0] * G[j][0] + t[i][1] * G[j][1] + t[i][2] * G[j][2]);
        }
}

td_status wino43_input_launch(const float* x, int B, int H, int W, int C, float* V, const int* m_dyn, hipStream_t s) {
    TD_REQUIRE(x && V && B >= 1 && H >= 1 && W >= 1 && C >= 4 && (C & 3) == 0, "winograd F(4x4) input transform: bad arguments");
    const long long T = (long long)B * ((H + 3) / 4) * ((W + 3) / 4);
    const long long threads = T * (C / 4);
    TD_REQUIRE(threads < (1ll << 31), "winograd F(4x4) input transform: grid too large");
    hipLaunchKernelGGL(wino43_input_kernel, dim3((unsigned)((threads + 255) / 256)), dim3(256), 0, s, x, B, H, W, C, V, T, m_dyn);
    TD_KERNEL_CHECK();
    return TD_OK;
}

td_status wino43_output_launch(const float* Mb, int B, int H, int W, int N, const float* scale, const float* bias, int relu,
                               float* y, const int* m_dyn, hipStream_t s) {
    TD_REQUIRE(Mb && y && B >= 1 && H >= 1 && W >= 1 && N >= 4 && (N & 3) == 0, "winograd F(4x4) output transform: bad arguments");
    const long long T = (long long)B * ((H + 3) / 4) * ((W + 3) / 4);
    const long long threads = T * (N / 4);
    TD_REQUIRE(threads < (1ll << 31), "winograd F(4x4) output transform: grid too large");
    hipLaunchKernelGGL(wino43_output_kernel, dim3((unsigned)((threads + 255) / 256)), dim3(256), 0, s, Mb, B, H, W, N, scale, bias,
                       relu, y, T, m_dyn);
    TD_KERNEL_CHECK();
    return TD_OK;
}

td_status wino43_output_head_launch(const float* Mb, int B, int H, int W, int N, const float* scale, const float* bias, int relu,
                                    const float* head_w, const float* head_b, float* head_y, int head_n, hipStream_t s) {
    TD_REQUIRE(Mb && head_w && head_y && B >= 1 && H >= 1 && W >= 1, "winograd F(4x4) output transform + head: bad arguments");
    TD_REQUIRE(N == 256 && head_n >= 1 && head_n <= 32, "winograd F(4x4) output transform + head: 256 channels, at most 32 head rows (got %d, %d)", N, head_n);
    const long long T = (long long)B * ((H + 3) / 4) * ((W + 3) / 4);
    TD_REQUIRE((T + 3) / 4 < (1ll << 31), "winograd F(4x4) output transform + head: grid too large");
    hipLaunchKernelGGL(wino43_output_head_kernel, dim3((unsigned)((T + 3) / 4)), dim3(256), 0, s, Mb, B, H, W, scale, bias, relu, T,
                       head_w, head_b, head_y, head_n);
    TD_KERNEL_CHECK();
    return TD_OK;
}

void wino43_filter_transform(const float* w, int N, int C, float* U) {
    static const double G[6][3] = {{1.0 / 4, 0, 0},           {-1.0 / 6, -1.0 / 6, -1.0 / 6}, {-1.0 / 6, 1.0 / 6, -1.0 / 6},
                                   {1.0 / 24, 1.0 / 12, 1.0 / 6}, {1.0 / 24, -1.0 / 12, 1.0 / 6}, {0, 0, 1}};
    for (int n = 0; n < N; ++n)
        for (int c = 0; c < C; ++c) {
            double g[3][3], t[6][3];
            for (int a = 0; a < 3; ++a)
                for (int b = 0; b < 3; ++b) g[a][b] = w[(((size_t)n * 3 + a) * 3 + b) * C + c];
            for (int i = 0; i < 6; ++i)
                for (int b = 0; b < 3; ++b) t[i][b] = G[i][0] * g[0][b] + G[i][1] * g[1][b] + G[i][2] * g[2][b];
            for (int i = 0; i < 6; ++i)
                for (int j = 0; j < 6; ++j)
                    U[((size_t)(6 * i + j) * N + n) * C + c] = (float)(t[i][0] * G[j][0] + t[i][1] * G[j][1] + t[i][2] * G[j][2]);
        }
}
```

Baseline: 676.9.

## Group FPN/RPN Winograd F(4x4) convolutions across pyramid levels into single launches

Adds a multi-level Winograd F(4x4) path that concatenates the tile axes of several FPN levels, padded to 64-tile boundaries. One input-transform launch and one fused contraction launch then cover all levels, each block picking its level's pointers from a small per-level table. The goal is fewer launches and better GPU fill on the small, low-occupancy coarse levels in the FP32 path. RPN head buffers are also made contiguous across levels, and when grouping does not fit the convs fall back to the fold path. The cost is a larger V scratch buffer, padding waste, and level lookup inside the kernels.

```diff
diff --git a/include/treedet.h b/include/treedet.h
--- a/include/treedet.h
+++ b/include/treedet.h
@@ -112,6 +112,10 @@
                                   int H, int W, int Cin, int Cout, int relu, void* stream);
 td_status td_conv2d_winograd_head_nhwc(const float* x, const float* w, const float* bias, const float* head_w, const float* head_b,
                                        float* head_y, int B, int H, int W, int Cin, int head_n, void* stream);
+td_status td_wino43_input_nhwc(const float* x, float* v, int B, int H, int W, int C, void* stream);
+td_status td_conv2d_winograd_group_nhwc(const float* const* x, const float* const* w, const float* const* scale, const float* const* bias,
+                                        float* const* y, const int* H, const int* W, int nlev, int B, int Cin, int Cout, int relu,
+                                        float* v, int64_t* tile_first, void* stream);
 td_status td_nms(const float* boxes, const float* scores, int n, float iou_thresh, int32_t* keep_idx,
                  int32_t* keep_count, void* stream);
 td_status td_roi_align(const void* feat, int H, int W, int C, const float* rois, int R, float spatial_scale,
diff --git a/treedetection_amd/_lib.py b/treedetection_amd/_lib.py
--- a/treedetection_amd/_lib.py
+++ b/treedetection_amd/_lib.py
@@ -62,12 +62,14 @@
                                      C.c_int, C.c_int64, C.c_void_p, C.c_void_p]),
     "td_bottleneck_tail_nhwc": (C.c_int, [C.c_void_p] * 9 + [C.c_int] * 6 + [C.c_void_p]),
     "td_resize_bilinear_f64": (C.c_int, [C.c_void_p, C.c_int, C.c_int, C.c_int, C.c_void_p, C.c_int, C.c_int, C.c_int, C.c_int64, C.c_void_p]),
+    "td_wino43_input_nhwc": (C.c_int, [C.c_void_p] * 2 + [C.c_int] * 4 + [C.c_void_p]),
     "td_windows_u16_to_input": (C.c_int, [C.c_void_p, C.c_int, C.c_int, C.c_int, C.c_void_p, C.c_int, C.c_void_p, C.c_void_p, C.c_int, C.c_int,
                                           C.c_int, C.c_int64, C.c_int64, C.c_void_p]),
     "td_resize_shape": (None, [C.c_int, C.c_int, C.c_int, C.c_int, C.POINTER(C.c_int), C.POINTER(C.c_int)]),
     "td_conv2d_nhwc": (C.c_int, [C.c_void_p, C.c_void_p, C.c_void_p, C.c_void_p, C.c_void_p, C.c_int, C.c_void_p]
                        + [C.c_int] * 11 + [C.c_void_p]),
     "td_conv2d_head_nhwc": (C.c_int, [C.c_void_p] * 6 + [C.c_int] * 9 + [C.c_void_p]),
+    "td_conv2d_winograd_group_nhwc": (C.c_int, [C.c_void_p] * 7 + [C.c_int] * 5 + [C.c_void_p] * 3),
     "td_conv2d_winograd_head_nhwc": (C.c_int, [C.c_void_p] * 6 + [C.c_int] * 5 + [C.c_void_p]),
     "td_conv2d_winograd_nhwc": (C.c_int, [C.c_void_p] * 5 + [C.c_int] * 6 + [C.c_void_p]),
     "td_nms": (C.c_int, [C.c_void_p, C.c_void_p, C.c_int, C.c_float, C.c_void_p, C.c_void_p, C.c_void_p]),
diff --git a/treedetection_amd/csrc/api.cpp b/treedetection_amd/csrc/api.cpp
--- a/treedetection_amd/csrc/api.cpp
+++ b/treedetection_amd/csrc/api.cpp
@@ -168,6 +168,60 @@
     return TD_OK;
 }
 
+td_status td_wino43_input_nhwc(const float* x, float* v, int B, int H, int W, int C, void* stream) {
+    return wino43_input_launch(x, B, H, W, C, v, nullptr, static_cast<hipStream_t>(stream));
+}
+
+td_status td_conv2d_winograd_group_nhwc(const float* const* x, const float* const* w, const float* const* scale, const float* const* bias,
+                                        float* const* y, const int* H, const int* W, int nlev, int B, int Cin, int Cout, int relu,
+                                        float* v, int64_t* tile_first, void* stream) {
+    TD_REQUIRE(x && w && y && H && W && nlev >= 1 && nlev <= 5 && B >= 1, "td_conv2d_winograd_group_nhwc: bad arguments");
+    hipStream_t s = static_cast<hipStream_t>(stream);
+    WinoGroup g{};
+    g.nlev = nlev; g.B = B; g.C = Cin; g.N = Cout; g.relu = relu;
+    for (int l = 0; l < nlev; ++l) {
+        TD_REQUIRE(x[l] && w[l] && y[l], "td_conv2d_winograd_group_nhwc: level %d has a null tensor", l);
+        g.lev[l].x = x[l]; g.lev[l].y = y[l]; g.lev[l].H = H[l]; g.lev[l].W = W[l];
+        g.lev[l].scale = scale ? scale[l] : nullptr; g.lev[l].bias = bias ? bias[l] : nullptr;
+    }
+    TD_REQUIRE(wino43_group_layout(g), "td_conv2d_winograd_group_nhwc: needs Cin = 128, 256 or 512, Cout %% 64 == 0 and planes below 4 GB");
+    if (tile_first) {
+        for (int l = 0; l < nlev; ++l) tile_first[l] = g.lev[l].first;
+        tile_first[nlev] = g.T;
+    }
+    std::vector<void*> banks(nlev, nullptr);
+    void* V = v;
+    td_status st = TD_OK;
+    const size_t wn = (size_t)Cout * 9 * Cin, un = (size_t)36 * Cout * Cin;
+    std::vector<float> wh(wn), uh(un);
+    for (int l = 0; l < nlev && st == TD_OK; ++l) {
+        for (int k = 0; k < l; ++k)
+            if (w[k] == w[l]) banks[l] = banks[k];
+        if (!banks[l]) {
+            if (hipMemcpy(wh.data(), w[l], wn * 4, hipMemcpyDeviceToHost) != hipSuccess) { st = TD_ERR_HIP; td_set_error("td_conv2d_winograd_group_nhwc: filter copy failed"); break; }
+            wino43_filter_transform(wh.data(), Cout, Cin, uh.data());
+            if ((st = scratch(&banks[l], un * 4)) == TD_OK && hipMemcpy(banks[l], uh.data(), un * 4, hipMemcpyHostToDevice) != hipSuccess) {
+                st = TD_ERR_HIP;
+                td_set_error("td_conv2d_winograd_group_nhwc: filter upload failed");
+            }
+        }
+        g.lev[l].U = static_cast<const float*>(banks[l]);
+    }
+    if (st == TD_OK && !V) st = scratch(&V, (size_t)36 * g.T * Cin * 4);
+    if (st == TD_OK) st = wino43_input_group_launch(g, static_cast<float*>(V), s);
+    if (st == TD_OK) st = wino43_fused_group_launch(g, static_cast<const float*>(V), s);
+    hipError_t herr = hipStreamSynchronize(s);
+    for (int l = 0; l < nlev; ++l) {
+        bool dup = false;
+        for (int k = 0; k < l; ++k) dup = dup || banks[k] == banks[l];
+        if (!dup) (void)hipFree(banks[l]);
+    }
+    if (V != v) (void)hipFree(V);
+    if (st < 0) return st;
+    TD_HIP_CHECK(herr);
+    return TD_OK;
+}
+
 td_status td_resize_tile_u8(const uint8_t* src, int h, int w, int c, uint8_t* dst, int out_h, int out_w,
                             int dst_pitch_px, void* tmp_dev, void* stream) {
     return resize_tile_u8_launch(src, h, w, c, dst, out_h, out_w, dst_pitch_px, tmp_dev, static_cast<hipStream_t>(stream));
diff --git a/treedetection_amd/csrc/common.h b/treedetection_amd/csrc/common.h
--- a/treedetection_amd/csrc/common.h
+++ b/treedetection_amd/csrc/common.h
@@ -156,6 +156,22 @@
 bool wino43_fused_ok(int B, int H, int W, int C, int N);
 td_status wino43_fused_launch(const float* V, const float* U, int B, int H, int W, int C, int N, const float* scale, const float* bias,
                               int relu, float* y, const int* m_dyn, hipStream_t s);
+struct WinoGroup {
+    int nlev, B, C, N, relu;
+    struct Level {
+        const float* x;
+        const float* U;
+        const float* scale;
+        const float* bias;
+        float* y;
+        int H, W;
+        long long first;
+    } lev[5];
+    long long T;
+};
+bool wino43_group_layout(WinoGroup& g);
+td_status wino43_input_group_launch(const WinoGroup& g, float* V, hipStream_t s);
+td_status wino43_fused_group_launch(const WinoGroup& g, const float* V, hipStream_t s);
 td_status wino43_output_launch(const float* Mb, int B, int H, int W, int N, const float* scale, const float* bias, int relu,
                                float* y, const int* m_dyn, hipStream_t s);
 td_status wino43_output_head_launch(const float* Mb, int B, int H, int W, int N, const float* scale, const float* bias, int relu,
diff --git a/treedetection_amd/csrc/engine.cpp b/treedetection_amd/csrc/engine.cpp
--- a/treedetection_amd/csrc/engine.cpp
+++ b/treedetection_amd/csrc/engine.cpp
@@ -78,6 +78,7 @@
     void *inner[4] = {}, *pfeat[5] = {};
     void* rpn_t = nullptr;
     float* rpn_headbuf[5] = {};
+    float* rpn_head_all = nullptr;
     uint32_t* key_ws = nullptr;
     float *cand_boxes = nullptr, *cand_scores = nullptr;
     int *cand_valid = nullptr, *cand_idx = nullptr;
@@ -107,6 +108,7 @@
     float *wino_v = nullptr, *wino_m = nullptr;
     size_t wino_elems = 0;
     bool group_levels = true;
+    int group_f32 = 3;
     bool fuse_head = true;
     bool fuse_tail = true;
     bool fuse_tail_fp16 = false;
@@ -424,7 +426,11 @@
     if (const char* ws = getenv("TD_WINO_SLAB")) e->wino_slab = atoi(ws);
     if (const char* wf = getenv("TD_WINO_FUSED")) e->wino_fused = atoi(wf) != 0;
     if (const char* fh = getenv("TD_FUSE_HEAD")) e->fuse_head = atoi(fh) != 0;
-    if (const char* gl = getenv("TD_GROUP_LEVELS")) e->group_levels = atoi(gl) != 0;
+    if (const char* gl = getenv("TD_GROUP_LEVELS")) {
+        const int v = atoi(gl);
+        e->group_levels = v != 0;
+        e->group_f32 = v == 1 ? 3 : ((v & 2) ? 1 : 0) | ((v & 4) ? 2 : 0);
+    }
     if (const char* ft = getenv("TD_FUSE_TAIL")) { e->fuse_tail = atoi(ft) != 0; e->fuse_tail_fp16 = atoi(ft) == 2; }
     if (const char* w4 = getenv("TD_WINO43_MIN")) e->wino43_min = atoi(w4);
     if (const char* wf2 = getenv("TD_WINO_FOLD")) e->wino_fold = atoi(wf2);
@@ -668,14 +674,19 @@
         if ((st = AA(&e->xtmp[s], px * co)) < 0) return st;
         if ((st = AA(&e->inner[s], px * e->fpn_c)) < 0) return st;
     }
-    size_t total_anchors = 0;
+    size_t total_anchors = 0, px_all = 0;
+    const bool f32 = e->desc.precision == TD_PRECISION_FP32;
+    for (int l = 0; l < 5; ++l) px_all += b * hs[l] * wsz[l];
+    e->rpn_head_all = nullptr;
+    if (f32 && (st = A(&e->rpn_head_all, px_all * RPN_HEAD_C)) < 0) return st;
     for (int l = 0; l < 5; ++l) {
         const size_t px = b * hs[l] * wsz[l];
         if ((st = AA(&e->pfeat[l], px * e->fpn_c)) < 0) return st;
-        if ((st = A(&e->rpn_headbuf[l], px * RPN_HEAD_C)) < 0) return st;
+        if (f32) e->rpn_headbuf[l] = nullptr;
+        else if ((st = A(&e->rpn_headbuf[l], px * RPN_HEAD_C)) < 0) return st;
         total_anchors += (size_t)hs[l] * wsz[l] * RPN_A;
     }
-    if ((st = AA(&e->rpn_t, b * hs[0] * wsz[0] * e->fpn_c)) < 0) return st;
+    if ((st = AA(&e->rpn_t, (f32 ? px_all : b * hs[0] * wsz[0]) * e->fpn_c)) < 0) return st;
     if ((st = A(&e->key_ws, rpn_topk_ws_elems((int)b, (int)total_anchors))) < 0) return st;
     const size_t nc = b * RPN_LEVELS * RPN_CAND;
     if ((st = A(&e->cand_boxes, nc * 4)) < 0) return st;
@@ -725,6 +736,13 @@
         for (int s = 0; s < 4; ++s) need = std::max(need, b * tiles(hs[s], wsz[s]) * (size_t)e->stages[s][0].c2.cout);
         need = std::max(need, mrows * tiles(14, 14) * (size_t)e->fpn_c);
         e->wino_elems = 16 * need;
+        WinoGroup g{};
+        g.B = B; g.C = g.N = e->fpn_c;
+        for (int l = 0; l < 5 && e->wino43_min > 0 && hs[l] >= e->wino43_min && wsz[l] >= e->wino43_min; ++l) {
+            g.lev[l].H = hs[l]; g.lev[l].W = wsz[l];
+            g.nlev = l + 1;
+        }
+        if (g.nlev >= 2 && wino43_group_layout(g)) e->wino_elems = std::max(e->wino_elems, (size_t)36 * (size_t)g.T * (size_t)e->fpn_c);
         if ((st = A(&e->wino_v, e->wino_elems)) < 0) return st;
         if ((st = A(&e->wino_m, e->wino_elems)) < 0) return st;
     }
@@ -929,6 +947,7 @@
         ClassScope cs(e, s_, dyn ? TD_CLS_MASK_HEAD : TD_CLS_WINO_XFORM, 0.0, dyn ? 0.0 : mb + yb);
         return wino43_output_launch(e->wino_m, B_, H_, W_, L.cout, L.scale, L.bias, relu ? 1 : 0, static_cast<float*>(y_), m_dyn, s_);
     };
+    bool fold_family = false;
     auto run_conv = [&](const ConvLayer& L, const void* x_, int B_, int H_, int W_, int stride, int pad, bool relu,
                         void* y_, const void* res_, int res_shift, hipStream_t s_, int prec_,
                         const int* m_dyn = nullptr, int m_mul = 1, int out_mode = 0,
@@ -963,8 +982,8 @@
                 use_43 = use_wino && L.wino_u43 && e->wino43_min > 0 && H_ >= e->wino43_min && W_ >= e->wino43_min &&
                          (size_t)36 * T43 * (size_t)std::max(L.cin, L.cout) <= e->wino_elems && T43 * std::max(L.cin, L.cout) < (1ll << 31);
                 const int hw_ = H_ * W_, wf_ = e->wino_fold;
-                use_fold = use_43 && wf_ > 0 && wino43_fused_ok(m_dyn ? B_ : 1, H_, W_, L.cin, L.cout) &&
-                           (((wf_ & 1) && !m_dyn && (!head || (wf_ & 32)) && ((L.cin == 256 && hw_ >= 160 * 160) || (L.cin == 128 && hw_ >= 80 * 80))) ||
+                use_fold = use_43 && wf_ > 0 && wino43_fused_ok(m_dyn ? B_ : 1, H_, W_, L.cin, L.cout) && (
+                           (fold_family && !m_dyn && !head) || ((wf_ & 1) && !m_dyn && (!head || (wf_ & 32)) && ((L.cin == 256 && hw_ >= 160 * 160) || (L.cin == 128 && hw_ >= 80 * 80))) ||
                             ((wf_ & 2) && m_dyn && !head) || ((wf_ & 4) && !m_dyn && !head && L.cin == 256 && hw_ >= 80 * 80) ||
                             ((wf_ & 8) && !m_dyn && !head && hw_ >= 40 * 40) || ((wf_ & 16) && !m_dyn && !head));
                 if (use_43 && !use_fold) {
@@ -1038,6 +1057,47 @@
         ClassScope cs(e, s_, TD_CLS_CONV3X3, flops, bytes);
         return conv_pp8_grouped_launch(a, s_);
     };
+    auto wino43_family = [&](const ConvLayer& L) {
+        return prec == TD_PRECISION_FP32 && e->autotune && e->wino_fold > 0 && e->wino_v && e->wino43_min > 0 && L.wino_u43 && L.kh == 3 && L.kw == 3 &&
+               L.cin == 256 && L.cin >= e->wino_minc && L.cout >= e->wino_minc && L.cout % 64 == 0;
+    };
+    auto run_wino43_group = [&](const ConvLayer* const* Ls, const void* const* xs, void* const* ys, int nl, const int* Hs, const int* Ws,
+                                bool relu, hipStream_t s_) -> td_status {
+        WinoGroup g{};
+        g.nlev = nl; g.B = B; g.C = Ls[0]->cin; g.N = Ls[0]->cout; g.relu = relu ? 1 : 0;
+        for (int l = 0; l < nl; ++l) {
+            g.lev[l].x = static_cast<const float*>(xs[l]); g.lev[l].U = static_cast<const float*>(Ls[l]->wino_u43);
+            g.lev[l].scale = Ls[l]->scale; g.lev[l].bias = Ls[l]->bias; g.lev[l].y = static_cast<float*>(ys[l]);
+            g.lev[l].H = Hs[l]; g.lev[l].W = Ws[l];
+        }
+        td_status st2 = TD_OK;
+        if (nl < 2 || !wino43_group_layout(g) || (size_t)36 * g.T * (size_t)std::max(g.C, g.N) > e->wino_elems) {
+            fold_family = true;
+            for (int l = 0; l < nl; ++l)
+                if ((st2 = run_conv(*Ls[l], xs[l], B, Hs[l], Ws[l], 1, 1, relu, ys[l], nullptr, 0, s_, prec)) < 0) break;
+            fold_family = false;
+            return st2;
+        }
+        double flops = 0.0, bytes = 0.0, exec = 0.0, xvb = 0.0, vyub = 0.0;
+        for (int l = 0; l < nl; ++l) {
+            const double M = (double)B * Hs[l] * Ws[l], K = 9.0 * g.C, T = (double)B * ((Hs[l] + 3) / 4) * ((Ws[l] + 3) / 4);
+            flops += 2.0 * M * g.N * K;
+            bytes += 4.0 * (M * g.C + M * g.N + g.N * K);
+            exec += 2.0 * 36 * T * (double)g.C * g.N;
+            xvb += 4.0 * M * g.C + 4.0 * 36 * T * g.C;
+            vyub += 4.0 * 36 * T * g.C + 4.0 * M * g.N + 4.0 * 36 * g.N * g.C;
+        }
+        ProfScope ps(e, s_, 0, flops, bytes);
+        if (e->prof) {
+            e->prof_launches[0] += nl - 1;
+            e->prof_flops[8] += exec;
+            e->prof_launches[8] += nl;
+        }
+        { ClassScope cs(e, s_, TD_CLS_WINO_XFORM, 0.0, xvb);
+        if ((st2 = wino43_input_group_launch(g, e->wino_v, s_)) < 0) return st2; }
+        ClassScope cs(e, s_, TD_CLS_WINO_GEMM, exec, vyub);
+        return wino43_fused_group_launch(g, e->wino_v, s_);
+    };
     auto run_tail = [&](const Block& blk, const void* t1_, int B_, int H_, int W_, void* y_, const void* shortcut_, hipStream_t s_) -> td_status {
         TailArgs a{};
         a.x = t1_; a.w2 = blk.c2.w; a.scale2 = blk.c2.scale; a.bias2 = blk.c2.bias;
@@ -1064,6 +1124,13 @@
     wsz[4] = (wsz[3] - 1) / 2 + 1;
     const size_t esz = prec == TD_PRECISION_FP16 ? 2 : 4;
     auto off = [&](void* p, size_t elems) -> void* { return static_cast<char*>(p) + elems * esz; };
+    if (e->rpn_head_all) {
+        size_t px0 = 0;
+        for (int l = 0; l < 5; ++l) {
+            e->rpn_headbuf[l] = e->rpn_head_all + px0 * RPN_HEAD_C;
+            px0 += (size_t)B * hs[l] * wsz[l];
+        }
+    }
     int sb = e->backbone_subbatch > 0 ? e->backbone_subbatch : B;
     if (sb > B) sb = B;
     const bool do_stem = PH(6) || (PH(0) && !e->stem_done);
@@ -1134,10 +1201,20 @@
     ProfScope fpn_group(e, s, 0, 0.0, 0.0, true);
     const bool group_fpn = prec == TD_PRECISION_FP16 && e->group_levels && groupable(e->fpn_out[0]) && groupable(e->fpn_out[1]) &&
                            groupable(e->fpn_out[2]) && groupable(e->fpn_out[3]);
+    const bool group_fpn32 = (e->group_f32 & 1) && wino43_family(e->fpn_out[0]) && wino43_family(e->fpn_out[1]) && wino43_family(e->fpn_out[2]) &&
+                             wino43_family(e->fpn_out[3]);
+    int ng_fpn = 0;
+    while (group_fpn32 && ng_fpn < 4 && hs[ng_fpn] >= e->wino43_min && wsz[ng_fpn] >= e->wino43_min) ++ng_fpn;
     for (int l = 3; l >= 0; --l) {
         const void* td_res = l == 3 ? nullptr : e->inner[l + 1];
         if ((st = run_conv(e->lateral[l], e->res[l], B, hs[l], wsz[l], 1, 0, false, e->inner[l], td_res, td_res ? 1 : 0, s, prec)) < 0) return st;
-        if (!group_fpn && (st = run_conv(e->fpn_out[l], e->inner[l], B, hs[l], wsz[l], 1, 1, false, e->pfeat[l], nullptr, 0, s, prec)) < 0) return st;
+        if (!group_fpn && l >= ng_fpn && (st = run_conv(e->fpn_out[l], e->inner[l], B, hs[l], wsz[l], 1, 1, false, e->pfeat[l], nullptr, 0, s, prec)) < 0) return st;
+    }
+    if (ng_fpn > 0) {
+        const ConvLayer* Ls[4] = {&e->fpn_out[0], &e->fpn_out[1], &e->fpn_out[2], &e->fpn_out[3]};
+        const void* xs[4] = {e->inner[0], e->inner[1], e->inner[2], e->inner[3]};
+        void* ys[4] = {e->pfeat[0], e->pfeat[1], e->pfeat[2], e->pfeat[3]};
+        if ((st = run_wino43_group(Ls, xs, ys, ng_fpn, hs, wsz, false, s)) < 0) return st;
     }
     if (group_fpn) {
         const ConvLayer* Ls[4] = {&e->fpn_out[0], &e->fpn_out[1], &e->fpn_out[2], &e->fpn_out[3]};
@@ -1162,8 +1239,31 @@
             float* hy[5] = {e->rpn_headbuf[0], e->rpn_headbuf[1], e->rpn_headbuf[2], e->rpn_headbuf[3], e->rpn_headbuf[4]};
             if ((st = run_grouped(Ls, xs, nullptr, hy, 5, hs, wsz, true, &e->rpn_head, s)) < 0) return st;
         }
+        const bool group_rpn32 = (e->group_f32 & 2) && wino43_family(e->rpn_conv) && e->rpn_conv.cout == e->fpn_c && e->rpn_head.kh == 1 &&
+                                 e->rpn_head.kw == 1 && e->rpn_head.cin == e->rpn_conv.cout && hs[0] >= e->wino43_min && wsz[0] >= e->wino43_min;
+        if (group_rpn32) {
+            int ng = 0;
+            while (ng < 5 && hs[ng] >= e->wino43_min && wsz[ng] >= e->wino43_min) ++ng;
+            const ConvLayer* Ls[5] = {&e->rpn_conv, &e->rpn_conv, &e->rpn_conv, &e->rpn_conv, &e->rpn_conv};
+            const void* xs[5] = {e->pfeat[0], e->pfeat[1], e->pfeat[2], e->pfeat[3], e->pfeat[4]};
+            void* ts[5];
+            size_t px0 = 0;
+            for (int l = 0; l < 5; ++l) {
+                ts[l] = off(e->rpn_t, px0 * e->fpn_c);
+                px0 += (size_t)B * hs[l] * wsz[l];
+            }
+            TD_REQUIRE(px0 < (1ull << 31), "forward: too many RPN pixels for one head launch");
+            if ((st = run_wino43_group(Ls, xs, ts, ng, hs, wsz, true, s)) < 0) return st;
+            for (int l = ng; l < 5; ++l)
+                if ((st = run_conv(e->rpn_conv, e->pfeat[l], B, hs[l], wsz[l], 1, 1, true, ts[l], nullptr, 0, s, prec)) < 0) return st;
+            if ((st = run_conv(e->rpn_head, e->rpn_t, 1, 1, (int)px0, 1, 0, false, e->rpn_headbuf[0], nullptr, 0, s, prec)) < 0) return st;
+            if (e->prof) {
+                e->prof_launches[0] += 4;
+                e->prof_bytes[0] += 4.0 * 4.0 * e->rpn_head.cout * e->rpn_head.cin;
+            }
+        }
         for (int l = 0; l < 5; ++l) {
-            if (group_rpn) {
+            if (group_rpn || group_rpn32) {
                 const std::string nm = "rpn_head" + std::to_string(l + 2);
                 set_named(e, nm.c_str(), e->rpn_headbuf[l], B, hs[l], wsz[l], RPN_HEAD_C);
                 continue;
diff --git a/treedetection_amd/csrc/wino_fused.hip b/treedetection_amd/csrc/wino_fused.hip
--- a/treedetection_amd/csrc/wino_fused.hip
+++ b/treedetection_amd/csrc/wino_fused.hip
@@ -4,15 +4,24 @@
 
 namespace {
 
-struct WinoFusedArgs {
-    const float* V;
+struct WinoFusedLevel {
     const float* U;
     const float* scale;
     const float* bias;
     float* y;
+    int H, W;
+    unsigned first;
+    unsigned pad_;
+};
+constexpr int WF_MAXLEV = 5;
+
+struct WinoFusedArgs {
+    const float* V;
     const int* m_dyn;
-    int B, H, W, C, N, relu;
+    int B, C, N, relu, nlev;
     long long T;
+    long long Tend;
+    WinoFusedLevel lev[WF_MAXLEV];
 };
 
 constexpr int WF_BN = 64;
@@ -39,19 +48,27 @@
     static_assert((NWT == 2 || NWT == 4) && (NS == 4 || NS == 8) && KREP >= 1 && NS * WF_STAGE <= 160 * 1024 && DROWS == WF_BT, "geometry");
     __shared__ __attribute__((aligned(16))) char lds[NS * WF_STAGE];
 
-    const int TH = (a.H + 3) >> 2, TW = (a.W + 3) >> 2;
-    long long live = a.T;
+    long long tend = a.Tend;
     if (a.m_dyn) {
-        const long long n = (long long)*a.m_dyn * TH * TW;
-        live = n < live ? n : live;
-    }
-    const int tb_n = (int)((live + WF_BT - 1) / WF_BT), nb_n = a.N / WF_BN;
+        const long long n = (long long)*a.m_dyn * ((a.lev[0].H + 3) >> 2) * ((a.lev[0].W + 3) >> 2);
+        tend = n < tend ? n : tend;
+    }
+    const int tb_n = (int)((tend + WF_BT - 1) / WF_BT), nb_n = a.N / WF_BN;
     const int nblk = tb_n * nb_n;
     if ((int)blockIdx.x >= nblk) return;
     const int pid = xcd_remap(blockIdx.x, nblk);
     const int tb = pid / nb_n, nb = pid - tb * nb_n;
     const long long t0 = (long long)tb * WF_BT;
     const int n0 = nb * WF_BN;
+    WinoFusedLevel L = a.lev[0];
+#pragma unroll
+    for (int l = 1; l < WF_MAXLEV; ++l)
+        if (l < a.nlev && t0 >= (long long)a.lev[l].first) L = a.lev[l];
+    const int TH = (L.H + 3) >> 2, TW = (L.W + 3) >> 2;
+    const long long tl0 = t0 - (long long)L.first;
+    long long live = (long long)a.B * TH * TW;
+    live = tend - (long long)L.first < live ? tend - (long long)L.first : live;
+    if (tl0 >= live) return;
 
     const int tid = threadIdx.x, lane = tid & 63;
     const int wave = __builtin_amdgcn_readfirstlane(tid >> 6);
@@ -62,10 +79,10 @@
     const unsigned row_bytes = (unsigned)a.C * 4u;
     const unsigned planeV = (unsigned)((unsigned long long)a.T * row_bytes), planeU = (unsigned)a.N * row_bytes;
     const __amdgpu_buffer_rsrc_t vrsrc = __builtin_amdgcn_make_buffer_rsrc(const_cast<float*>(a.V), 0, (int)(36u * planeV), 0x00020000);
-    const __amdgpu_buffer_rsrc_t ursrc = __builtin_amdgcn_make_buffer_rsrc(const_cast<float*>(a.U), 0, (int)(36u * planeU), 0x00020000);
+    const __amdgpu_buffer_rsrc_t ursrc = __builtin_amdgcn_make_buffer_rsrc(const_cast<float*>(L.U), 0, (int)(36u * planeU), 0x00020000);
     const int ld_c = tid & 7, ld_r = tid >> 3;
     const unsigned src_piece = (unsigned)(ld_c ^ ((ld_r >> 1) & 7)) * 16u;
-    const bool v_ok = t0 + ld_r < live;
+    const bool v_ok = tl0 + ld_r < live;
     const unsigned v_off = (unsigned)(t0 + ld_r) * row_bytes + src_piece;
     const unsigned u_off = (unsigned)(n0 + ld_r) * row_bytes + src_piece;
     typedef __attribute__((address_space(3))) void lds_void;
@@ -213,37 +230,37 @@
     r0 = WF_AT[0][5]; r1 = WF_AT[1][5]; r2 = WF_AT[2][5]; r3 = WF_AT[3][5];
     wf_static_for<8>([&](auto sl_c) __attribute__((always_inline)) { fold_y(sl_c); });
 
-    const long long t = t0 + wt * 16 + (int)r16;
+    const long long t = tl0 + wt * 16 + (int)r16;
     const bool tlive = t < live;
     const unsigned tt = tlive ? (unsigned)t : 0u;
     const unsigned tyx = tt % (unsigned)(TW * TH);
     const unsigned b = tt / (unsigned)(TW * TH);
     const unsigned ty = tyx / (unsigned)TW, tx = tyx - ty * (unsigned)TW;
-    const __amdgpu_buffer_rsrc_t yrsrc = __builtin_amdgcn_make_buffer_rsrc(a.y, 0, (int)((unsigned)a.B * a.H * a.W * a.N * 4u), 0x00020000);
+    const __amdgpu_buffer_rsrc_t yrsrc = __builtin_amdgcn_make_buffer_rsrc(L.y, 0, (int)((unsigned)a.B * L.H * L.W * a.N * 4u), 0x00020000);
     f32x4 sc[2], bi[2];
 #pragma unroll
     for (int blk = 0; blk < 2; ++blk) {
         const int n = n0 + wc * 32 + blk * 16 + 4 * (int)q;
-        sc[blk] = a.scale ? *reinterpret_cast<const f32x4*>(a.scale + n) : f32x4{1.f, 1.f, 1.f, 1.f};
-        bi[blk] = a.bias ? *reinterpret_cast<const f32x4*>(a.bias + n) : f32x4{0.f, 0.f, 0.f, 0.f};
-    }
-    const unsigned pix0 = (b * (unsigned)a.H + 4u * ty) * (unsigned)a.W + 4u * tx;
+        sc[blk] = L.scale ? *reinterpret_cast<const f32x4*>(L.scale + n) : f32x4{1.f, 1.f, 1.f, 1.f};
+        bi[blk] = L.bias ? *reinterpret_cast<const f32x4*>(L.bias + n) : f32x4{0.f, 0.f, 0.f, 0.f};
+    }
+    const unsigned pix0 = (b * (unsigned)L.H + 4u * ty) * (unsigned)L.W + 4u * tx;
     const unsigned nbytes = (unsigned)a.N * 4u;
 #pragma unroll
     for (int i = 0; i < 4; ++i) {
-        const bool rok = tlive && (int)(4u * ty) + i < a.H;
+        const bool rok = tlive && (int)(4u * ty) + i < L.H;
 #pragma unroll
         for (int j = 0; j < 4; ++j) {
-            const bool ok = rok && (int)(4u * tx) + j < a.W;
-            const unsigned pbase = (pix0 + (unsigned)(i * a.W + j)) * nbytes;
+            const bool ok = rok && (int)(4u * tx) + j < L.W;
+            const unsigned pbase = (pix0 + (unsigned)(i * L.W + j)) * nbytes;
 #pragma unroll
             for (int blk = 0; blk < 2; ++blk) {
                 f32x4 v = Y[4 * i + j][blk];
 #pragma unroll
                 for (int e = 0; e < 4; ++e) {
                     float o = v[e];
-                    if (a.scale) o = __fmul_rn(o, sc[blk][e]);
-                    if (a.bias) o = __fadd_rn(o, bi[blk][e]);
+                    if (L.scale) o = __fmul_rn(o, sc[blk][e]);
+                    if (L.bias) o = __fadd_rn(o, bi[blk][e]);
                     if (a.relu) o = o > 0.f ? o : 0.f;
                     v[e] = o;
                 }
@@ -262,26 +279,35 @@
            36ull * (unsigned long long)N * C * 4 < 0xfffffff0ull - (1u << 20) && (unsigned long long)B * H * W * N * 4 < 0xfffffff0ull - (1u << 20);
 }
 
-td_status wino43_fused_launch(const float* V, const float* U, int B, int H, int W, int C, int N, const float* scale, const float* bias,
-                              int relu, float* y, const int* m_dyn, hipStream_t s) {
-    TD_REQUIRE(V && U && y && B >= 1 && H >= 1 && W >= 1, "winograd F(4x4) fused contraction: bad arguments");
-    TD_REQUIRE(wino43_fused_ok(B, H, W, C, N), "winograd F(4x4) fused contraction: needs C = 128, 256 or 512, N %% 64 == 0 and planes below 4 GB (C %d, N %d)", C, N);
-    WinoFusedArgs a{};
-    a.V = V; a.U = U; a.scale = scale; a.bias = bias; a.y = y; a.m_dyn = m_dyn;
-    a.B = B; a.H = H; a.W = W; a.C = C; a.N = N; a.relu = relu;
-    a.T = (long long)B * ((H + 3) / 4) * ((W + 3) / 4);
+bool wino43_group_layout(WinoGroup& g) {
+    if (g.nlev < 1 || g.nlev > WF_MAXLEV || g.B < 1) return false;
+    long long first = 0;
+    for (int l = 0; l < g.nlev; ++l) {
+        if (g.lev[l].H < 1 || g.lev[l].W < 1 || !wino43_fused_ok(g.B, g.lev[l].H, g.lev[l].W, g.C, g.N)) return false;
+        const long long live = (long long)g.B * ((g.lev[l].H + 3) / 4) * ((g.lev[l].W + 3) / 4);
+        g.lev[l].first = first;
+        first += (live + 63) / 64 * 64;
+    }
+    g.T = first;
+    return 36ull * (unsigned long long)g.T * g.C * 4 < 0xfffffff0ull - (1u << 20) && g.T * (g.C / 4) < (1ll << 31);
+}
+
+namespace {
+
+td_status wf_launch(const WinoFusedArgs& a, hipStream_t s) {
+    const int C = a.C, N = a.N;
     static const int num_cu = [] {
         int dev = 0, n = 0;
         if (hipGetDevice(&dev) != hipSuccess || hipDeviceGetAttribute(&n, hipDeviceAttributeMultiprocessorCount, dev) != hipSuccess || n < 64) n = 256;
         return n;
     }();
-    const long long blocks64 = ((a.T + 63) / 64) * (N / WF_BN);
-    int nwt = (C == 512 || (blocks64 < num_cu && !m_dyn)) ? 2 : 4;
+    const long long blocks64 = ((a.Tend + 63) / 64) * (N / WF_BN);
+    int nwt = (C == 512 || (blocks64 < num_cu && !a.m_dyn)) ? 2 : 4;
     if (const char* f = getenv("TD_WF_NWT")) {
         const int v = atoi(f);
         if ((v == 2 || v == 4) && !(v == 4 && C == 512)) nwt = v;
     }
-    const long long blocks = ((a.T + 16 * nwt - 1) / (16 * nwt)) * (N / WF_BN);
+    const long long blocks = ((a.Tend + 16 * nwt - 1) / (16 * nwt)) * (N / WF_BN);
     TD_REQUIRE(blocks < (1ll << 31), "winograd F(4x4) fused contraction: grid too large");
 #define TD_WF_LAUNCH(NSV, KREPV, NWTV, VARV) hipLaunchKernelGGL((wino43_fused_kernel<NSV, KREPV, NWTV, VARV>), dim3((unsigned)blocks), dim3(128 * NWTV), 0, s, a)
 #if defined(TD_WF_DIAG)
@@ -311,3 +337,34 @@
     TD_KERNEL_CHECK();
     return TD_OK;
 }
+
+}
+
+td_status wino43_fused_launch(const float* V, const float* U, int B, int H, int W, int C, int N, const float* scale, const float* bias,
+                              int relu, float* y, const int* m_dyn, hipStream_t s) {
+    TD_REQUIRE(V && U && y && B >= 1 && H >= 1 && W >= 1, "winograd F(4x4) fused contraction: bad arguments");
+    TD_REQUIRE(wino43_fused_ok(B, H, W, C, N), "winograd F(4x4) fused contraction: needs C = 128, 256 or 512, N %% 64 == 0 and planes below 4 GB (C %d, N %d)", C, N);
+    WinoFusedArgs a{};
+    a.V = V; a.m_dyn = m_dyn;
+    a.B = B; a.C = C; a.N = N; a.relu = relu; a.nlev = 1;
+    a.T = a.Tend = (long long)B * ((H + 3) / 4) * ((W + 3) / 4);
+    a.lev[0].U = U; a.lev[0].scale = scale; a.lev[0].bias = bias; a.lev[0].y = y; a.lev[0].H = H; a.lev[0].W = W;
+    return wf_launch(a, s);
+}
+
+td_status wino43_fused_group_launch(const WinoGroup& g, const float* V, hipStream_t s) {
+    TD_REQUIRE(V && g.nlev >= 1 && g.nlev <= WF_MAXLEV && g.B >= 1, "winograd F(4x4) fused group: bad arguments");
+    WinoGroup chk = g;
+    TD_REQUIRE(wino43_group_layout(chk) && chk.T == g.T, "winograd F(4x4) fused group: needs C = 128, 256 or 512, N %% 64 == 0, planes below 4 GB and the tile axis of wino43_group_layout");
+    WinoFusedArgs a{};
+    a.V = V;
+    a.B = g.B; a.C = g.C; a.N = g.N; a.relu = g.relu; a.nlev = g.nlev;
+    a.T = g.T;
+    for (int l = 0; l < g.nlev; ++l) {
+        TD_REQUIRE(g.lev[l].U && g.lev[l].y && g.lev[l].first == chk.lev[l].first, "winograd F(4x4) fused group: level %d incomplete", l);
+        a.lev[l].U = g.lev[l].U; a.lev[l].scale = g.lev[l].scale; a.lev[l].bias = g.lev[l].bias; a.lev[l].y = g.lev[l].y;
+        a.lev[l].H = g.lev[l].H; a.lev[l].W = g.lev[l].W; a.lev[l].first = (unsigned)g.lev[l].first;
+        a.Tend = g.lev[l].first + (long long)g.B * ((g.lev[l].H + 3) / 4) * ((g.lev[l].W + 3) / 4);
+    }
+    return wf_launch(a, s);
+}
diff --git a/treedetection_amd/csrc/winograd.hip b/treedetection_amd/csrc/winograd.hip
--- a/treedetection_amd/csrc/winograd.hip
+++ b/treedetection_amd/csrc/winograd.hip
@@ -132,21 +132,38 @@
     t[5] = TD_ADD(TD_SUB(TD_MUL(4.f, d[1]), TD_MUL(5.f, d[3])), d[5]);
 }
 
-__global__ __launch_bounds__(256) void wino43_input_kernel(const float* __restrict__ x, int B, int H, int W, int C,
-                                                           float* __restrict__ V, long long T, const int* __restrict__ m_dyn) {
-    const int TH = (H + 3) >> 2, TW = (W + 3) >> 2;
-    const int c4n = C >> 2;
+struct Wino43InputArgs {
+    float* V;
+    const int* m_dyn;
+    int B, C, nlev;
+    long long T;
+    struct Level { const float* x; int H, W; unsigned first, pad_; } lev[5];
+};
+
+__global__ __launch_bounds__(256) void wino43_input_kernel(const Wino43InputArgs a) {
+    const int C = a.C, c4n = C >> 2;
+    float* __restrict__ V = a.V;
+    const long long T = a.T;
     const unsigned idx = blockIdx.x * blockDim.x + threadIdx.x;
     const unsigned t = idx / (unsigned)c4n;
     const int c = (int)(idx - t * (unsigned)c4n) * 4;
-    long long live = T;
-    if (m_dyn) {
-        const long long n = (long long)*m_dyn * TH * TW;
-        live = n < T ? n : T;
-    }
-    if ((long long)t >= live) return;
-    const unsigned tyx = t % (unsigned)(TW * TH);
-    const int b = (int)(t / (unsigned)(TW * TH));
+    const unsigned tblk = (blockIdx.x * blockDim.x) / (unsigned)c4n;
+    Wino43InputArgs::Level L = a.lev[0];
+#pragma unroll
+    for (int l = 1; l < 5; ++l)
+        if (l < a.nlev && tblk >= a.lev[l].first) L = a.lev[l];
+    const float* __restrict__ x = L.x;
+    const int H = L.H, W = L.W;
+    const int TH = (H + 3) >> 2, TW = (W + 3) >> 2;
+    long long live = (long long)a.B * TH * TW;
+    if (a.m_dyn) {
+        const long long n = (long long)*a.m_dyn * TH * TW;
+        live = n < live ? n : live;
+    }
+    const unsigned tl = t - L.first;
+    if ((long long)tl >= live) return;
+    const unsigned tyx = tl % (unsigned)(TW * TH);
+    const int b = (int)(tl / (unsigned)(TW * TH));
     const int ty = (int)(tyx / (unsigned)TW);
     const int tx = (int)(tyx - (unsigned)ty * (unsigned)TW);
     const int y0 = 4 * ty - 1, x0 = 4 * tx - 1;
@@ -377,7 +394,29 @@
     const long long T = (long long)B * ((H + 3) / 4) * ((W + 3) / 4);
     const long long threads = T * (C / 4);
     TD_REQUIRE(threads < (1ll << 31), "winograd F(4x4) input transform: grid too large");
-    hipLaunchKernelGGL(wino43_input_kernel, dim3((unsigned)((threads + 255) / 256)), dim3(256), 0, s, x, B, H, W, C, V, T, m_dyn);
+    Wino43InputArgs a{};
+    a.V = V; a.m_dyn = m_dyn; a.B = B; a.C = C; a.nlev = 1; a.T = T;
+    a.lev[0].x = x; a.lev[0].H = H; a.lev[0].W = W;
+    hipLaunchKernelGGL(wino43_input_kernel, dim3((unsigned)((threads + 255) / 256)), dim3(256), 0, s, a);
+    TD_KERNEL_CHECK();
+    return TD_OK;
+}
+
+td_status wino43_input_group_launch(const WinoGroup& g, float* V, hipStream_t s) {
+    TD_REQUIRE(V && g.nlev >= 1 && g.nlev <= 5 && g.B >= 1 && g.C >= 4 && 256 % (g.C / 4) == 0 && 64 % (256 / (g.C / 4)) == 0,
+               "winograd F(4x4) input transform of a group: bad arguments");
+    WinoGroup chk = g;
+    TD_REQUIRE(wino43_group_layout(chk) && chk.T == g.T, "winograd F(4x4) input transform of a group: not the tile axis of wino43_group_layout");
+    Wino43InputArgs a{};
+    a.V = V; a.B = g.B; a.C = g.C; a.nlev = g.nlev; a.T = g.T;
+    long long end = 0;
+    for (int l = 0; l < g.nlev; ++l) {
+        TD_REQUIRE(g.lev[l].x && g.lev[l].first == chk.lev[l].first, "winograd F(4x4) input transform of a group: level %d incomplete", l);
+        a.lev[l].x = g.lev[l].x; a.lev[l].H = g.lev[l].H; a.lev[l].W = g.lev[l].W; a.lev[l].first = (unsigned)g.lev[l].first;
+        end = g.lev[l].first + (long long)g.B * ((g.lev[l].H + 3) / 4) * ((g.lev[l].W + 3) / 4);
+    }
+    const long long threads = end * (g.C / 4);
+    hipLaunchKernelGGL(wino43_input_kernel, dim3((unsigned)((threads + 255) / 256)), dim3(256), 0, s, a);
     TD_KERNEL_CHECK();
     return TD_OK;
 }
```

Result: no change. 679.9 (median of 4 runs) (+0.4%).
